# ntnu-yjyjames/nano-vectordb

Measured on AMD Instinct MI355X. Metric: QPS + effective HBM GB/s, flat-scan top-10 d=768, higher is better.
Workload: dtype f16

## Files before the change

nano-vectordb_amd/csrc/kernels_corpus.h:

```cpp
#pragma once
#include <hip/hip_runtime.h>

#include "kernels_exact.h"
#include "nvdb_common.h"

namespace nvdbhip {

template <int DT>
__global__ __launch_bounds__(256) void gen_rows_kernel(uint64_t seed, uint64_t row_base, uint64_t n, uint32_t dim,
                                                       void* __restrict__ rows, float* __restrict__ scales) {
  const int lane = threadIdx.x & 63;
  const uint64_t r = static_cast<uint64_t>(blockIdx.x) * 4 + (threadIdx.x >> 6);
  if (r >= n) return;
  const uint32_t key = synth_row_key(seed, row_base + r);
  unsigned long long ss = 0;
  for (uint32_t c = lane; c < dim; c += 64) { const long long v = synth_raw(key, c); ss += static_cast<unsigned long long>(v * v); }
  for (int o = 32; o > 0; o >>= 1) ss += __shfl_xor(ss, o);
  const double inv = synth_inv_norm(ss);
  if constexpr (DT == DT_F32) {
    float* out = static_cast<float*>(rows) + r * dim;
    for (uint32_t c = lane; c < dim; c += 64) out[c] = synth_elem(synth_raw(key, c), inv);
  } else if constexpr (DT == DT_F16) {
    _Float16* out = static_cast<_Float16*>(rows) + r * dim;
    for (uint32_t c = lane; c < dim; c += 64) out[c] = static_cast<_Float16>(synth_elem(synth_raw(key, c), inv));
  } else {
    float mx = 0.f;
    for (uint32_t c = lane; c < dim; c += 64) mx = fmaxf(mx, fabsf(synth_elem(synth_raw(key, c), inv)));
    for (int o = 32; o > 0; o >>= 1) mx = fmaxf(mx, __shfl_xor(mx, o));
    const float scale = mx > 0.f ? mx / 127.f : 1.f;
    const float is = 1.0f / scale;
    signed char* out = static_cast<signed char*>(rows) + r * dim;
    for (uint32_t c = lane; c < dim; c += 64) {
      float qv = rintf(synth_elem(synth_raw(key, c), inv) * is);
      qv = fminf(fmaxf(qv, -127.f), 127.f);
      out[c] = static_cast<signed char>(static_cast<int>(qv));
    }
    if (lane == 0) scales[r] = scale;
  }
}

template <typename SrcT>
__global__ __launch_bounds__(256) void shadow_f16_kernel(const SrcT* __restrict__ src, _Float16* __restrict__ dst, size_t n,
                                                         uint32_t dim, uint32_t sdim, uint32_t* __restrict__ maxabs_bits) {
  float mx = 0.f;
  const size_t count = n * sdim;
  for (size_t i = static_cast<size_t>(blockIdx.x) * 256 + threadIdx.x; i < count; i += static_cast<size_t>(gridDim.x) * 256) {
    const size_t r = i / sdim;
    const uint32_t c = static_cast<uint32_t>(i - r * sdim);
    const float v = c < dim ? static_cast<float>(src[r * dim + c]) : 0.f;
    dst[i] = static_cast<_Float16>(v);
    mx = fmaxf(mx, fabsf(v));
  }
  for (int o = 32; o > 0; o >>= 1) mx = fmaxf(mx, __shfl_xor(mx, o));
  if ((threadIdx.x & 63) == 0 && mx > 0.f) atomicMax(maxabs_bits, __builtin_bit_cast(uint32_t, mx));
}

static __global__ __launch_bounds__(256) void shadow_i8_kernel(const signed char* __restrict__ src, signed char* __restrict__ dst, size_t n,
                                                        uint32_t dim, uint32_t sdim) {
  const size_t count = n * sdim;
  for (size_t i = static_cast<size_t>(blockIdx.x) * 256 + threadIdx.x; i < count; i += static_cast<size_t>(gridDim.x) * 256) {
    const size_t r = i / sdim;
    const uint32_t c = static_cast<uint32_t>(i - r * sdim);
    dst[i] = c < dim ? src[r * dim + c] : static_cast<signed char>(0);
  }
}

template <typename SrcT>
__global__ __launch_bounds__(256) void shadow_q8_kernel(const SrcT* __restrict__ src, signed char* __restrict__ dst, float* __restrict__ dst_scales,
                                                        uint64_t n, uint32_t dim, uint32_t sdim, uint32_t* __restrict__ out_bits) {
  const int lane = threadIdx.x & 63;
  float wres = 0.f;
  bool bad = false;
  for (uint64_t r = static_cast<uint64_t>(blockIdx.x) * 4 + (threadIdx.x >> 6); r < n; r += static_cast<uint64_t>(gridDim.x) * 4) {
    const SrcT* row = src + r * dim;
    float mx = 0.f;
    for (uint32_t c = lane; c < dim; c += 64) mx = fmaxf(mx, fabsf(static_cast<float>(row[c])));
    for (int o = 32; o > 0; o >>= 1) mx = fmaxf(mx, __shfl_xor(mx, o));
    if (!(mx < 3.0e38f)) bad = true;
    const float scale = mx > 0.f ? mx / 127.f : 1.f;
    const float inv = 1.0f / scale;
    float ss = 0.f;
    signed char* out = dst + r * sdim;
    for (uint32_t c = lane; c < sdim; c += 64) {
      float qv = 0.f, x = 0.f;
      if (c < dim) { x = static_cast<float>(row[c]); qv = fminf(fmaxf(rintf(x * inv), -127.f), 127.f); }
      out[c] = static_cast<signed char>(static_cast<int>(qv));
      const float d = x - qv * scale;
      ss = __builtin_fmaf(d, d, ss);
    }
    for (int o = 32; o > 0; o >>= 1) ss += __shfl_xor(ss, o);
    if (!(ss == ss)) bad = true;
    if (lane == 0) dst_scales[r] = scale;
    wres = fmaxf(wres, sqrtf(ss) * 1.0001f);
  }
  if (lane == 0 && wres > 0.f) atomicMax(out_bits, __builtin_bit_cast(uint32_t, wres));
  if (lane == 0 && (bad || !(wres < 3.0e38f))) out_bits[1] = 1u;
}

template <int DT>
__global__ __launch_bounds__(256) void row_norm_max_kernel(const void* __restrict__ rows, const float* __restrict__ scales,
                                                           uint64_t n, uint32_t dim, uint32_t* __restrict__ out_bits) {
  const int lane = threadIdx.x & 63;
  float wmax = 0.f;
  for (uint64_t r = static_cast<uint64_t>(blockIdx.x) * 4 + (threadIdx.x >> 6); r < n; r += static_cast<uint64_t>(gridDim.x) * 4) {
    const void* rp = row_ptr<DT>(rows, r, dim);
    float ss = 0.f;
    for (uint32_t c = lane; c < dim; c += 64) { const float v = load1<DT>(rp, c); ss = __builtin_fmaf(v, v, ss); }
    for (int o = 32; o > 0; o >>= 1) ss += __shfl_xor(ss, o);
    float nrm = sqrtf(ss) * 1.0001f;
    if constexpr (DT == DT_I8) {
      const float sc = scales[r];
      nrm *= fabsf(sc);
      if (!(sc >= 0.f && sc < 1e30f) && lane == 0) out_bits[1] = 1u;
    }
    wmax = fmaxf(wmax, nrm);
  }
  if (lane == 0 && wmax > 0.f) atomicMax(out_bits, __builtin_bit_cast(uint32_t, wmax));
}

}
```

nano-vectordb_amd/csrc/kernels_filter.h:

```cpp
#pragma once
#include <hip/hip_runtime.h>

#include "kernels_exact.h"

namespace nvdbhip {

typedef _Float16 half8_t __attribute__((ext_vector_type(8)));
typedef float floatx16 __attribute__((ext_vector_type(16)));
typedef int intx16 __attribute__((ext_vector_type(16)));
typedef int int4_t __attribute__((ext_vector_type(4)));

#define NVDB_GPTR(p) ((const __attribute__((address_space(1))) void*)(p))
#define NVDB_LPTR(p) ((__attribute__((address_space(3))) void*)(p))

constexpr int FILTER_ROWS = 32;
constexpr int FILTER_STAGES = 3;
constexpr int FILTER_STAGES_I8 = 5;

struct PrepInit {
  uint32_t* cnt;
  float* thr;
  uint32_t* misc;
  uint32_t* prog;
  uint32_t prog_words;
  uint32_t* tickets;
  const float* q_src;
  float* q32_copy;
};
constexpr uint32_t FUSE_TICKETS = 1;

__device__ __forceinline__ const float* prep_init(const PrepInit& pi, const float* q32, uint32_t q, uint32_t tid, uint32_t nq, uint32_t dim, uint32_t* overflow) {
  if (pi.cnt != nullptr) {
    if (tid == 0) { pi.cnt[q] = 0; overflow[q] = 0; pi.thr[q] = NEG_INF; }
    if (q == 0 && tid < 8) pi.misc[tid] = 0;
    if (q == 0 && tid >= 64 && tid < 64 + FUSE_TICKETS) pi.tickets[tid - 64] = 0;
    for (uint32_t j = q * 256 + tid; j < pi.prog_words; j += gridDim.x * 256) pi.prog[j] = 0xFFFFFFFFu;
  }
  if (pi.q_src != nullptr && q < nq) {
    float* dst = pi.q32_copy + static_cast<uint64_t>(q) * dim;
    const float* srch = pi.q_src + static_cast<uint64_t>(q) * dim;
    for (uint32_t i = tid; i < dim; i += 256) dst[i] = srch[i];
    return dst;
  }
  return q32 + static_cast<uint64_t>(q) * dim;
}

static __global__ __launch_bounds__(256) void prep_q16_kernel(const float* __restrict__ q32, uint32_t nq, uint32_t dim, uint32_t sdim,
                                                       float max_row_norm, float rel, float abs_per_norm, uint32_t* __restrict__ overflow, _Float16* __restrict__ q16,
                                                       float* __restrict__ qscale, float* __restrict__ qinv,
                                                       float* __restrict__ ebound, float* __restrict__ slack, PrepInit pi) {
  __shared__ float red_max[4], red_ss[4];
  const uint32_t q = blockIdx.x, tid = threadIdx.x;
  const float* src = prep_init(pi, q32, q, tid, nq, dim, overflow);
  if (q >= nq) {
    for (uint32_t i = tid; i < sdim; i += 256) q16[static_cast<uint64_t>(q) * sdim + i] = static_cast<_Float16>(0.f);
    if (tid == 0) { qscale[q] = 1.f; qinv[q] = 1.f; ebound[q] = 0.f; slack[q] = 0.f; }
    return;
  }
  float mx = 0.f, ss = 0.f;
  for (uint32_t i = tid; i < dim; i += 256) { const float v = src[i]; mx = fmaxf(mx, fabsf(v)); ss = __builtin_fmaf(v, v, ss); }
  for (int o = 32; o > 0; o >>= 1) { mx = fmaxf(mx, __shfl_xor(mx, o)); ss += __shfl_xor(ss, o); }
  if ((tid & 63) == 0) { red_max[tid >> 6] = mx; red_ss[tid >> 6] = ss; }
  __syncthreads();
  mx = fmaxf(fmaxf(red_max[0], red_max[1]), fmaxf(red_max[2], red_max[3]));
  ss = (red_ss[0] + red_ss[1]) + (red_ss[2] + red_ss[3]);
  int e = 0;
  if (mx > 0.f && mx < 3.0e38f) {
    int ex; (void)frexpf(mx, &ex);
    e = 15 - ex;
    e = e > 100 ? 100 : (e < -100 ? -100 : e);
  }
  const float sc = ldexpf(1.f, e);
  for (uint32_t i = tid; i < sdim; i += 256) q16[static_cast<uint64_t>(q) * sdim + i] = static_cast<_Float16>(i < dim ? src[i] * sc : 0.f);
  if (tid == 0) {
    const float nrm = sqrtf(ss) * 1.0001f;
    const float eb = rel * nrm * max_row_norm + abs_per_norm * nrm + 1e-30f;
    qscale[q] = sc; qinv[q] = ldexpf(1.f, -e); ebound[q] = eb; slack[q] = 2.f * eb;
    if (!(ss < 3.0e38f)) { overflow[q] = 1u; ebound[q] = -1.f; }
  }
}

typedef float float4_t __attribute__((ext_vector_type(4)));
typedef float float2_t __attribute__((ext_vector_type(2)));

#define NVDB_MFMA_F16_ZERO_A(acc, a, b) asm volatile("v_mfma_f32_32x32x16_f16 %0, %1, %2, 0" : "=&v"(acc) : "v"(a), "a"(b))
#define NVDB_MFMA_F16_ZERO_V(acc, a, b) asm volatile("v_mfma_f32_32x32x16_f16 %0, %1, %2, 0" : "=&v"(acc) : "v"(a), "v"(b))
#define NVDB_MFMA_F16_ACC_A(acc, a, b) asm volatile("v_mfma_f32_32x32x16_f16 %0, %1, %2, %0" : "+v"(acc) : "v"(a), "a"(b))
#define NVDB_MFMA_F16_ACC_V(acc, a, b) asm volatile("v_mfma_f32_32x32x16_f16 %0, %1, %2, %0" : "+v"(acc) : "v"(a), "v"(b))

__device__ __forceinline__ void glds16(uint32_t voff, const void* sbase, uint32_t lds_off) {
  uint32_t keep;
  asm volatile("s_mov_b32 %0, m0\n\ts_mov_b32 m0, %2\n\ts_nop 0\n\tglobal_load_lds_dwordx4 %1, %3\n\ts_mov_b32 m0, %0"
               : "=&s"(keep) : "v"(voff), "s"(lds_off), "s"(sbase) : "memory");
}

__device__ __forceinline__ float vmax3(float a, float b, float c) {
  float r;
  asm("v_max3_f32 %0, %1, %2, %3" : "=v"(r) : "v"(a), "v"(b), "v"(c));
  return r;
}

struct Hit { float score; uint32_t row; uint32_t qid; uint32_t pad; };
constexpr uint32_t I8_HI_L1_MAX = 65500;
constexpr int I8_ACC_BIAS = 0x4B000000;
__device__ __forceinline__ int shl_i32(int v, uint32_t bits) { return static_cast<int>(static_cast<uint32_t>(v) << bits); }
constexpr uint32_t FILTER_LOGCAP = 4096;

struct ScatterArgs {
  Cand* cand;
  uint32_t* cnt;
  uint32_t* overflow;
  uint32_t* log_overflow;
  uint32_t cap;
  uint32_t n_rows;
  uint32_t perm_mul, perm_mask, perm_T;
  float* xcdw;
  uint32_t lo_bits;
};

__device__ __forceinline__ void stream_tile_range(uint32_t T, uint32_t S, uint32_t stream, bool xcd_map, const float* xcdw, uint32_t& lo, uint32_t& hi) {
  if (!xcd_map || xcdw == nullptr || (S & 7u) != 0) {
    lo = static_cast<uint32_t>(static_cast<uint64_t>(T) * stream / S);
    hi = static_cast<uint32_t>(static_cast<uint64_t>(T) * (stream + 1) / S);
    return;
  }
  double pre[9];
  pre[0] = 0.0;
#pragma unroll
  for (int x = 0; x < 8; ++x) pre[x + 1] = pre[x] + static_cast<double>(xcdw[x]);
  const double total = pre[8] * static_cast<double>(S >> 3);
  auto f = [&](uint32_t s) -> uint32_t {
    if (s >= S) return T;
    double part = 0.0;
#pragma unroll
    for (int x = 0; x < 8; ++x) part = (static_cast<uint32_t>(x) == (s & 7u)) ? pre[x] : part;
    const double cum = pre[8] * static_cast<double>(s >> 3) + part;
    const uint32_t v = static_cast<uint32_t>(static_cast<double>(T) * (cum / total));
    return v > T ? T : v;
  };
  lo = f(stream);
  hi = f(stream + 1);
}

__device__ __forceinline__ void record_xcd_speed(float* xcdw, bool xcd_map, uint32_t label, uint32_t ntiles, uint32_t ticks_100mhz) {
  if (xcdw == nullptr || !xcd_map || ntiles < 128) return;
  atomicAdd(xcdw + 8 + label, static_cast<float>(ticks_100mhz) * 0.01f);
  atomicAdd(xcdw + 16 + label, static_cast<float>(ntiles));
}

__host__ __device__ __forceinline__ uint32_t perm_tile_raw(uint32_t g, uint32_t mul, uint32_t mask, uint32_t T) {
  if (mask == 0) return g;
  uint32_t x = g;
  do { x = (x * mul + 0x9E3779B1u) & mask; } while (x >= T);
  return x;
}
__device__ __forceinline__ uint32_t perm_tile(uint32_t g, const ScatterArgs& a) { return perm_tile_raw(g, a.perm_mul, a.perm_mask, a.perm_T); }

__host__ __device__ __forceinline__ void perm_params(uint32_t T, uint32_t& mul, uint32_t& mask) {
  mul = 1u; mask = 0u;
  if (T < 64) return;
  uint32_t m = 1;
  while (m < T) m <<= 1;
  mask = m - 1;
  mul = (static_cast<uint32_t>(0.6180339887 * m) | 1u) & mask;
}

__device__ __forceinline__ void scatter_own_log(const Hit* mylog, uint32_t wcnt, const ScatterArgs& a, int lane) {
  asm volatile("s_waitcnt vmcnt(0)" ::: "memory");
  uint32_t n = wcnt;
  if (n > FILTER_LOGCAP) { if (lane == 0) *a.log_overflow = 1u; n = FILTER_LOGCAP; }
  for (uint32_t i = lane; i < n; i += 64) {
    const uint32_t* w = reinterpret_cast<const uint32_t*>(mylog + i);
    const uint32_t sbits = __hip_atomic_load(w + 0, __ATOMIC_RELAXED, __HIP_MEMORY_SCOPE_AGENT);
    const uint32_t row = __hip_atomic_load(w + 1, __ATOMIC_RELAXED, __HIP_MEMORY_SCOPE_AGENT);
    const uint32_t qid = __hip_atomic_load(w + 2, __ATOMIC_RELAXED, __HIP_MEMORY_SCOPE_AGENT);
    if (row >= a.n_rows) continue;
    const uint32_t slot = atomicAdd(&a.cnt[qid], 1u);
    if (slot < a.cap) a.cand[static_cast<uint64_t>(qid) * a.cap + slot] = Cand{__builtin_bit_cast(float, sbits), row};
    else a.overflow[qid] = 1u;
  }
}

__device__ __forceinline__ void glds16_v(const void* gptr, uint32_t lds_off) {
  uint32_t keep;
  asm volatile("s_mov_b32 %0, m0\n\ts_mov_b32 m0, %2\n\ts_nop 0\n\tglobal_load_lds_dwordx4 %1, off\n\ts_mov_b32 m0, %0"
               : "=&s"(keep) : "v"(gptr), "s"(lds_off) : "memory");
}

template <int DIM> constexpr size_t filter_f16_lds_bytes() { return static_cast<size_t>(FILTER_STAGES) * FILTER_ROWS * DIM * 2; }
// ... 504 lines not shown
  const char* gbase = reinterpret_cast<const char*>(rows);
  const uint32_t lds_base = static_cast<uint32_t>(reinterpret_cast<uintptr_t>(NVDB_LPTR(smem)));
  const uint32_t g_lo = row_lo / TROWS + t_lo;
  auto tile_phys = [&](uint32_t t_rel) -> uint32_t { return perm_tile(g_lo + (t_rel < NT ? t_rel : NT - 1), sa); };
  auto stage_ptr = [&](uint32_t t_rel, int kh) -> const char* {
    return gbase + static_cast<uint64_t>(tile_phys(t_rel)) * TROWS * ROW_BYTES + kh * SROW;
  };
  auto issue_piece = [&](const char* src, uint32_t buf, int i) {
    glds16(src_off[i], src, lds_base + buf * STAGE_BYTES + (wave * PPW + i) * 1024);
  };
#pragma unroll
  for (int i = 0; i < PPW; ++i) issue_piece(stage_ptr(0, 0), 0, i);
#pragma unroll
  for (int i = 0; i < PPW; ++i) issue_piece(stage_ptr(0, 1), 1, i);

  constexpr int PIECE_EVERY = KS / PPW;
  uint32_t wcnt = 0;
  Hit* mylog = hitlog + static_cast<uint64_t>(wave_gid) * FILTER_LOGCAP;
  uint32_t* myprog = prog + static_cast<uint64_t>(stream) * 8;
  uint32_t sync_strikes = 0;
  const uint32_t xw_t0 = static_cast<uint32_t>(__builtin_amdgcn_s_memrealtime());
  for (uint32_t t = 0; t < NT; ++t) {
    if constexpr (SYNC) {
      if (wave == 0 && (t & sync_mask) == 0) sibling_rendezvous(myprog, qt, t, sync_lead, sync_strikes, lane);
    }
    float4_t acc;
#pragma unroll
    for (int kh = 0; kh < 2; ++kh) {
      const uint32_t st = 2 * t + kh;
      asm volatile("s_waitcnt vmcnt(%0)" ::"n"(PPW) : "memory");
      __builtin_amdgcn_s_barrier();
      const char* next_src = stage_ptr(t + 1, kh);
      const uint32_t next_buf = (st + 2) % FILTER_STAGES;
      const char* stage = smem + (st % FILTER_STAGES) * STAGE_BYTES;
      if (!wave_has_queries) {
#pragma unroll
        for (int i = 0; i < PPW; ++i) issue_piece(next_src, next_buf, i);
        continue;
      }
      auto read_a = [&](int s) -> float4_t {
        return *reinterpret_cast<const float4_t*>(stage + (a16 ^ ((s & 3) << 6)) + (s >> 2) * 256);
      };
      float4_t ar[RING];
#pragma unroll
      for (int s = 0; s < RING - 1; ++s) ar[s] = read_a(s);
#pragma unroll
      for (int s = 0; s < KS; ++s) {
        if (s + RING - 1 < KS) ar[(s + RING - 1) % RING] = read_a(s + RING - 1);
        const float4_t a = ar[s % RING];
        const int f = kh * KS + s;
        if (f == 0) NVDB_MFMA16_ZERO_A(acc, a, bqa[0]);
        else if (f < NFRAG_A) NVDB_MFMA16_ACC_A(acc, a, bqa[f < NFRAG_A ? f : 0]);
        else NVDB_MFMA16_ACC_V(acc, a, bqv[f >= NFRAG_A ? f - NFRAG_A : 0]);
        if (s % PIECE_EVERY == PIECE_EVERY - 1) issue_piece(next_src, next_buf, s / PIECE_EVERY);
      }
    }
    if (!wave_has_queries) continue;
    asm volatile("s_nop 15\n\ts_nop 15" : "+v"(acc));
    const float m = vmax3(vmax3(acc[0], acc[1], acc[2]), acc[3], acc[3]);
    if (__builtin_amdgcn_ballot_w64(m - thr_s >= 0.f)) {
      const uint32_t row0 = tile_phys(t) * TROWS;
#pragma unroll
      for (int r = 0; r < 4; ++r) {
        const float v = acc[r];
        const bool hit = v >= thr_s;
        const unsigned long long mm = __builtin_amdgcn_ballot_w64(hit);
        if (mm) {
          const uint32_t idx = wcnt + static_cast<uint32_t>(__builtin_popcountll(mm & ((1ull << lane) - 1ull)));
          if (hit && idx < FILTER_LOGCAP) mylog[idx] = Hit{v * inv_s, row0 + 4 * g4 + r, qid, 0u};
          wcnt += static_cast<uint32_t>(__builtin_popcountll(mm));
        }
      }
    }
  }
  if constexpr (SYNC) { if (wave == 0 && lane == 0) __hip_atomic_store(myprog + qt, 0xFFFFFFFFu, __ATOMIC_RELAXED, __HIP_MEMORY_SCOPE_AGENT); }
  if (wave == 0 && lane == 0) record_xcd_speed(sa.xcdw, xcd_map, stream & 7u, NT, static_cast<uint32_t>(__builtin_amdgcn_s_memrealtime()) - xw_t0);
  scatter_own_log(mylog, wcnt, sa, lane);
}

static __global__ __launch_bounds__(256) void prep_q8_kernel(const float* __restrict__ q32, uint32_t nq, uint32_t dim, uint32_t sdim,
                                                      float max_row_norm, float corpus_resid, signed char* __restrict__ qhi,
                                                      signed char* __restrict__ qlo, float* __restrict__ qscale,
                                                      float* __restrict__ qinv, float* __restrict__ ebound,
                                                      float* __restrict__ slack, float* __restrict__ qdelta, uint32_t* __restrict__ overflow, uint32_t lo_bits, PrepInit pi) {
  __shared__ float red_max[4], red_ss[4];
  __shared__ uint32_t red_lo[4];
  const uint32_t q = blockIdx.x, tid = threadIdx.x;
  const float* src = prep_init(pi, q32, q, tid, nq, dim, overflow);
  if (q >= nq) {
    for (uint32_t i = tid; i < sdim; i += 256) { qhi[static_cast<uint64_t>(q) * sdim + i] = 0; qlo[static_cast<uint64_t>(q) * sdim + i] = 0; }
    if (tid == 0) { qscale[q] = 1.f; qinv[q] = 1.f; ebound[q] = 0.f; slack[q] = 0.f; qdelta[q] = 0.f; }
    return;
  }
  float mx = 0.f, ss = 0.f;
  for (uint32_t i = tid; i < dim; i += 256) { const float v = src[i]; mx = fmaxf(mx, fabsf(v)); ss = __builtin_fmaf(v, v, ss); }
  for (int o = 32; o > 0; o >>= 1) { mx = fmaxf(mx, __shfl_xor(mx, o)); ss += __shfl_xor(ss, o); }
  if ((tid & 63) == 0) { red_max[tid >> 6] = mx; red_ss[tid >> 6] = ss; }
  __syncthreads();
  mx = fmaxf(fmaxf(red_max[0], red_max[1]), fmaxf(red_max[2], red_max[3]));
  ss = (red_ss[0] + red_ss[1]) + (red_ss[2] + red_ss[3]);
  const int tmax = 127 << lo_bits, half = 1 << (lo_bits - 1);
  const float sq0 = (mx > 0.f && mx < 3.0e38f) ? mx / static_cast<float>(tmax) : 1.f;
  const float isq0 = 1.0f / sq0;
  float sq_adj = 1.f;
  if (static_cast<uint64_t>(dim) * 127u > I8_HI_L1_MAX) {
    __shared__ uint32_t red_l1[4];
    uint32_t l1 = 0;
    for (uint32_t i = tid; i < dim; i += 256) {
      int t = static_cast<int>(rintf(src[i] * isq0));
      t = t > tmax ? tmax : (t < -tmax ? -tmax : t);
      const int hi = (t + half) >> lo_bits;
      l1 += static_cast<uint32_t>(hi < 0 ? -hi : hi);
    }
    for (int o = 32; o > 0; o >>= 1) l1 += __shfl_xor(l1, o);
    if ((tid & 63) == 0) red_l1[tid >> 6] = l1;
    __syncthreads();
    l1 = (red_l1[0] + red_l1[1]) + (red_l1[2] + red_l1[3]);
    if (l1 > I8_HI_L1_MAX - dim) {
      const float shrink = static_cast<float>(l1) / static_cast<float>(I8_HI_L1_MAX - dim) * 1.001f;
      sq_adj = shrink;
    }
  }
  const float sq = sq0 * sq_adj;
  const float isq = 1.0f / sq;
  uint32_t lo2 = 0;
  for (uint32_t i = tid; i < dim; i += 256) {
    int t = static_cast<int>(rintf(src[i] * isq));
    t = t > tmax ? tmax : (t < -tmax ? -tmax : t);
    const int hi = (t + half) >> lo_bits;
    const int lo = t - (hi << lo_bits);
    qhi[static_cast<uint64_t>(q) * sdim + i] = static_cast<signed char>(hi);
    qlo[static_cast<uint64_t>(q) * sdim + i] = static_cast<signed char>(lo);
    lo2 += static_cast<uint32_t>(lo * lo);
  }
  for (uint32_t i = dim + tid; i < sdim; i += 256) { qhi[static_cast<uint64_t>(q) * sdim + i] = 0; qlo[static_cast<uint64_t>(q) * sdim + i] = 0; }
  for (int o = 32; o > 0; o >>= 1) lo2 += __shfl_xor(lo2, o);
  if ((tid & 63) == 0) red_lo[tid >> 6] = lo2;
  __syncthreads();
  if (tid == 0) {
    qdelta[q] = sqrtf(static_cast<float>(red_lo[0] + red_lo[1] + red_lo[2] + red_lo[3])) * max_row_norm * 1.0001f;

    const float nrm = sqrtf(ss) * 1.0001f;
    const float eb = (0.5005f * sqrtf(static_cast<float>(dim)) * sq + 1.0e-5f * nrm) * max_row_norm * 1.001f + nrm * corpus_resid * 1.001f + 1e-30f;
    qscale[q] = isq; qinv[q] = sq; ebound[q] = eb; slack[q] = 2.f * eb;
    if (!(ss < 3.0e38f)) { overflow[q] = 1u; ebound[q] = -1.f; }
  }
}

template <int ROW_BYTES> __device__ constexpr bool swz16() { return (ROW_BYTES / 16) % 16 == 0; }
template <int ROW_BYTES> __device__ inline uint32_t swz_chunk(uint32_t c, uint32_t r) {
  static_assert(ROW_BYTES % 128 == 0, "int8 row stride: a multiple of 128 bytes");
  return swz16<ROW_BYTES>() ? c ^ (r & 15u) : c ^ ((r >> 1) & 7u);
}
template <int ROW_BYTES> __device__ inline uint32_t a_base_i8(uint32_t r31, uint32_t hsel) { return r31 * ROW_BYTES + (swz_chunk<ROW_BYTES>(hsel, r31) << 4); }
template <int ROW_BYTES> __device__ inline uint32_t a_addr_i8(uint32_t a_base, int s) {
  return swz16<ROW_BYTES>() ? (a_base ^ ((s & 7) << 5)) + (s >> 3) * 256 : (a_base ^ ((s & 3) << 5)) + (s >> 2) * 128;
}

#define NVDB_MFMA_I8_ZERO(acc, a, b) asm volatile("v_mfma_i32_32x32x32_i8 %0, %1, %2, 0" : "=&v"(acc) : "v"(a), "a"(b))
#define NVDB_MFMA_I8_ACC(acc, a, b) asm volatile("v_mfma_i32_32x32x32_i8 %0, %1, %2, %0" : "+v"(acc) : "v"(a), "a"(b))
#define NVDB_MFMA_I8_FROM(acc, a, b, c0) asm volatile("v_mfma_i32_32x32x32_i8 %0, %1, %2, %3" : "=&v"(acc) : "v"(a), "a"(b), "v"(c0))

template <int DIM> constexpr size_t filter_i8_lds_bytes() { return static_cast<size_t>(FILTER_STAGES_I8) * (FILTER_ROWS * DIM + 4 * 1024); }
template <int DIM, bool BOOT = false, int RING = 6, bool SYNC = false>
__global__ __launch_bounds__(256, 1) void filter_i8_kernel(
    const signed char* __restrict__ rows, const float* __restrict__ scales, uint32_t row_lo, uint32_t row_hi,
    const signed char* __restrict__ qhi, const signed char* __restrict__ qlo, uint32_t nq, uint32_t QT,
    const float* __restrict__ thr, const float* __restrict__ qscale, const float* __restrict__ qinv,
    Hit* __restrict__ hitlog, ScatterArgs sa, uint32_t aux, uint32_t* __restrict__ prog, uint32_t sync_mask, uint32_t sync_lead) {
  constexpr int KSTEPS = DIM / 32;
  constexpr int ROW_BYTES = DIM;
  constexpr int DATA_BYTES = FILTER_ROWS * ROW_BYTES;
  constexpr int STAGE_BYTES = DATA_BYTES + 4 * 1024;
  constexpr int PIECES = DATA_BYTES / 1024;
  constexpr int PPW = PIECES / 4;
  constexpr int CHUNKS_PER_ROW = ROW_BYTES / 16;
  static_assert(DIM % 128 == 0, "int8 row stride: a multiple of 128 bytes (swz_chunk)");
  static_assert(PIECES % 4 == 0 && KSTEPS % PPW == 0 && 2 * KSTEPS <= 64, "shape");
  static_assert(FILTER_STAGES_I8 * STAGE_BYTES == filter_i8_lds_bytes<DIM>(), "the launchers size the dynamic LDS with filter_i8_lds_bytes");

  extern __shared__ __attribute__((aligned(16))) char smem[];
  const int tid = threadIdx.x, lane = tid & 63, wave = __builtin_amdgcn_readfirstlane(tid >> 6);
  const int r31 = lane & 31, hsel = lane >> 5;
  const uint32_t wave_gid = blockIdx.x * 4 + wave;

  const uint32_t nwg = gridDim.x, b = blockIdx.x;
  const uint32_t S = nwg / QT;
  uint32_t stream, qt;
  if ((nwg & 7u) == 0 && ((nwg >> 3) % QT) == 0) { const uint32_t xcd = b & 7u, i = b >> 3; qt = i % QT; stream = (i / QT) * 8u + xcd; }
  else { qt = b % QT; stream = b / QT; }
  const uint32_t tiles_total = (row_hi - row_lo) / FILTER_ROWS;
  const bool xcd_map = (nwg & 7u) == 0 && ((nwg >> 3) % QT) == 0;
  uint32_t t_lo, t_hi;
  stream_tile_range(tiles_total, S, stream, xcd_map, sa.xcdw, t_lo, t_hi);
  const uint32_t NT = t_hi - t_lo;
  if (NT == 0) return;

  const uint32_t qbase = qt * 128u + wave * 32u;
  float4_t bq[2 * KSTEPS];
#pragma unroll
  for (int f = 0; f < 2 * KSTEPS; ++f) {
    const signed char* plane = (f < KSTEPS) ? qhi : qlo;
    const int s = f % KSTEPS;
    bq[f] = *reinterpret_cast<const float4_t*>(plane + static_cast<uint64_t>(qbase + r31) * DIM + 32 * s + 16 * hsel);
  }
#pragma unroll
  for (int f = 0; f < 2 * KSTEPS; ++f) asm volatile("" ::"a"(bq[f]));
  const uint32_t qid = qbase + r31;
  const bool real = qid < nq;
  float thr_s = real ? thr[qid] * qscale[qid] : __builtin_huge_valf();
  float inv_s = real ? qinv[qid] : 0.f;
  asm volatile("" ::"v"(thr_s), "v"(inv_s));
  const bool wave_has_queries = qbase < nq;

  uint32_t src_off[PPW];
#pragma unroll
  for (int i = 0; i < PPW; ++i) {
    const uint32_t P = static_cast<uint32_t>((wave * PPW + i) * 64 + lane);
    const uint32_t r = P / CHUNKS_PER_ROW, cpos = P % CHUNKS_PER_ROW;
    src_off[i] = r * ROW_BYTES + (swz_chunk<ROW_BYTES>(cpos, r) << 4);
  }
  const uint32_t sc_off = (lane & 7) * 16;
  const uint32_t a_base = a_base_i8<ROW_BYTES>(static_cast<uint32_t>(r31), static_cast<uint32_t>(hsel));

  const char* gbase = reinterpret_cast<const char*>(rows);
  const uint32_t lds_base = static_cast<uint32_t>(reinterpret_cast<uintptr_t>(NVDB_LPTR(smem)));
  const uint32_t g_lo = row_lo / FILTER_ROWS + t_lo;
  auto tile_row0 = [&](uint32_t t_rel) -> uint32_t { return perm_tile(g_lo + (t_rel < NT ? t_rel : NT - 1), sa) * FILTER_ROWS; };
// ... 324 lines not shown
    if constexpr (VAR == 1) continue;
    const uint32_t row0 = tile_row0(t);
    if constexpr (DEFER) {
      uint32_t nflag = 0;
#pragma unroll
      for (int mb = 0; mb < MB; ++mb)
#pragma unroll
        for (int nb = 0; nb < NB; ++nb) {
          if (!__builtin_amdgcn_ballot_w64(d1[mb][nb] >= 0.f)) continue;
#pragma unroll
          for (int r = 0; r < 16; ++r) {
            const unsigned long long m = __builtin_amdgcn_ballot_w64(static_cast<float>(acc[mb][nb][r]) * scv[mb][r] >= t1q[nb]);
            if (m) {
              nflag += static_cast<uint32_t>(__builtin_popcountll(m));
              const int L = __builtin_ctzll(m);
              pend_H = __builtin_amdgcn_readlane(acc[mb][nb][r], L);
              pend_scale = readlane_f(scv[mb][r], L);
              pend_thr = readlane_f(thr_s[nb], L);
              pend_inv = readlane_f(inv_s[nb], L);
              pend_qid = readlane_u(qid[nb], L);
              pend_row = 32u * mb + (r & 3) + 8u * (r >> 2) + 4u * (static_cast<uint32_t>(L) >> 5);
            }
          }
        }
      if (nflag == 1) {
        if (lane < DIM / 16) pend_x = *reinterpret_cast<const uint4*>(stage + pend_row * ROW_BYTES + (swz_chunk<ROW_BYTES>(static_cast<uint32_t>(lane), pend_row) << 4));
        if (lane < DIM / 16) glds16(static_cast<uint32_t>(lane) * 16u, qlo + static_cast<uint64_t>(pend_qid) * DIM, lds_scratch);
        pend_row += row0;
        pend = true;
        continue;
      }
    }
#pragma unroll
    for (int mb = 0; mb < MB; ++mb)
#pragma unroll
      for (int nb = 0; nb < NB; ++nb) {
        if (!__builtin_amdgcn_ballot_w64(d1[mb][nb] >= 0.f)) continue;
        ++n_stage2;
        const signed char* ql = qlo + static_cast<uint64_t>(qbase + nb * 32 + r31) * DIM + 16 * hsel;
        intx16 lo;
        constexpr int HALF = KSTEPS / 2;
#pragma unroll
        for (int h = 0; h < 2; ++h) {
          float4_t bl[HALF];
#pragma unroll
          for (int s = 0; s < HALF; ++s) bl[s] = *reinterpret_cast<const float4_t*>(ql + 32 * (h * HALF + s));
#pragma unroll
          for (int s = 0; s < RING - 1; ++s) ar[s] = read_a(MB * (h * HALF + s) + mb);
#pragma unroll
          for (int s = 0; s < HALF; ++s) {
            if (s + RING - 1 < HALF) ar[(s + RING - 1) % RING] = read_a(MB * (h * HALF + s + RING - 1) + mb);
            const float4_t a = ar[s % RING];
            if (h == 0 && s == 0) NVDB_MFMA_I8_ZERO_V(lo, a, bl[s]); else NVDB_MFMA_I8_ACC_V(lo, a, bl[s]);
          }
        }
        asm volatile("s_nop 15\n\ts_nop 15" : "+v"(lo));
#pragma unroll
        for (int r = 0; r < 16; ++r) {
          const float fv = static_cast<float>(shl_i32(acc[mb][nb][r], sa.lo_bits) + lo[r]) * scv[mb][r];
          const bool hit = fv >= thr_s[nb];
          const unsigned long long m = __builtin_amdgcn_ballot_w64(hit);
          if (m) {
            const uint32_t idx = wcnt + static_cast<uint32_t>(__builtin_popcountll(m & ((1ull << lane) - 1ull)));
            if (hit && idx < FILTER_LOGCAP) mylog[idx] = Hit{fv * inv_s[nb], row0 + 32 * mb + (r & 3) + 8 * (r >> 2) + 4 * hsel, qid[nb], 0u};
            wcnt += static_cast<uint32_t>(__builtin_popcountll(m));
          }
        }
      }
  }
  if constexpr (DEFER) { if (pend) consume_pending(0); }
  if constexpr (STAMP) {
    const uint64_t dc = __builtin_amdgcn_s_memtime() - stamp_c, dr = __builtin_amdgcn_s_memrealtime() - stamp_r;
    if (wave == 0 && lane == 0) {
      uint64_t* out = reinterpret_cast<uint64_t*>(prog + static_cast<uint64_t>(gridDim.x) * 8) + static_cast<uint64_t>(blockIdx.x) * 2;
      out[0] = dc; out[1] = dr;
    }
  }
  if constexpr (SYNC) { if (wave == 0 && lane == 0) __hip_atomic_store(prog + static_cast<uint64_t>(stream) * 8 + qt, 0xFFFFFFFFu, __ATOMIC_RELAXED, __HIP_MEMORY_SCOPE_AGENT); }
  if (stage_counts && lane == 0 && (n_stage1 | n_stage2)) { atomicAdd(stage_counts, n_stage1); atomicAdd(stage_counts + 1, n_stage2); }
  if (wave == 0 && lane == 0) record_xcd_speed(sa.xcdw, xcd_map, stream & 7u, NT, static_cast<uint32_t>(__builtin_amdgcn_s_memrealtime()) - xw_t0);
  scatter_own_log(mylog, wcnt, sa, lane);
}

template <int DIM>
__device__ __forceinline__ void verify_and_scatter_i8(const Hit* mylog, uint32_t wcnt, const ScatterArgs& a, int lane, const signed char* __restrict__ rows,
                                                      const signed char* __restrict__ qlo, const float* __restrict__ thr, const float* __restrict__ qscale,
                                                      const float* __restrict__ qinv) {
  asm volatile("s_waitcnt vmcnt(0)" ::: "memory");
  uint32_t n = wcnt;
  if (n > FILTER_LOGCAP) { if (lane == 0) *a.log_overflow = 1u; n = FILTER_LOGCAP; }
  constexpr int CPL = DIM / 64;
  constexpr int NE = 2;
  const int part4 = lane & 3;
  for (uint32_t base = 0; base < n; base += 16 * NE) {
    uint32_t sbits[NE], row[NE], qid[NE];
    int H[NE], part[NE];
    bool valid[NE];
#pragma unroll
    for (int j = 0; j < NE; ++j) {
      const uint32_t e = base + 16u * j + (static_cast<uint32_t>(lane) >> 2);
      valid[j] = e < n;
      const uint32_t* w = reinterpret_cast<const uint32_t*>(mylog + (valid[j] ? e : 0u));
      sbits[j] = __hip_atomic_load(w + 0, __ATOMIC_RELAXED, __HIP_MEMORY_SCOPE_AGENT);
      row[j] = __hip_atomic_load(w + 1, __ATOMIC_RELAXED, __HIP_MEMORY_SCOPE_AGENT);
      qid[j] = __hip_atomic_load(w + 2, __ATOMIC_RELAXED, __HIP_MEMORY_SCOPE_AGENT);
      H[j] = static_cast<int>(__hip_atomic_load(w + 3, __ATOMIC_RELAXED, __HIP_MEMORY_SCOPE_AGENT));
    }
    uint4 x[NE][CPL], y[NE][CPL];
#pragma unroll
    for (int j = 0; j < NE; ++j) {
      valid[j] = valid[j] && row[j] < a.n_rows;
      const uint4* xr = reinterpret_cast<const uint4*>(rows + static_cast<uint64_t>(valid[j] ? row[j] : 0u) * DIM);
      const uint4* qr = reinterpret_cast<const uint4*>(qlo + static_cast<uint64_t>(valid[j] ? qid[j] : 0u) * DIM);
#pragma unroll
      for (int c = 0; c < CPL; ++c) { x[j][c] = xr[part4 + 4 * c]; y[j][c] = qr[part4 + 4 * c]; }
    }
#pragma unroll
    for (int j = 0; j < NE; ++j) {
      part[j] = 0;
#pragma unroll
      for (int c = 0; c < CPL; ++c) {
        part[j] = __builtin_amdgcn_sdot4(static_cast<int>(x[j][c].x), static_cast<int>(y[j][c].x), part[j], false);
        part[j] = __builtin_amdgcn_sdot4(static_cast<int>(x[j][c].y), static_cast<int>(y[j][c].y), part[j], false);
        part[j] = __builtin_amdgcn_sdot4(static_cast<int>(x[j][c].z), static_cast<int>(y[j][c].z), part[j], false);
        part[j] = __builtin_amdgcn_sdot4(static_cast<int>(x[j][c].w), static_cast<int>(y[j][c].w), part[j], false);
      }
      part[j] += __builtin_amdgcn_update_dpp(0, part[j], 0xB1, 0xF, 0xF, true);
      part[j] += __builtin_amdgcn_update_dpp(0, part[j], 0x4E, 0xF, 0xF, true);
      if (valid[j] && part4 == 0) {
        const float fv = static_cast<float>(shl_i32(H[j], a.lo_bits) + part[j]) * __builtin_bit_cast(float, sbits[j]);
        if (fv >= thr[qid[j]] * qscale[qid[j]]) {
          const uint32_t slot = atomicAdd(&a.cnt[qid[j]], 1u);
          if (slot < a.cap) a.cand[static_cast<uint64_t>(qid[j]) * a.cap + slot] = Cand{fv * qinv[qid[j]], row[j]};
          else a.overflow[qid[j]] = 1u;
        }
      }
    }
  }
}

template <int DIM, int WPB = 4, bool DEFER = true> constexpr size_t filter_i8p_lds_bytes() {
  return static_cast<size_t>(3) * (2 * FILTER_ROWS * DIM + (WPB == 4 ? 4 : 1) * 256) + (DEFER ? WPB * (16 / WPB) * DIM : 0);
}
template <int DIM, bool SYNC = false, bool STAMP = false, int RING = 6, int VAR = 0, int WPB = 4, bool DEFER = true>
__global__ __launch_bounds__(64 * WPB, 1) void filter_i8p_kernel(
    const signed char* __restrict__ rows, const float* __restrict__ scales, uint32_t row_lo, uint32_t row_hi,
    const signed char* __restrict__ qhi, const signed char* __restrict__ qlo, uint32_t nq, uint32_t QT,
    const float* __restrict__ thr, const float* __restrict__ qscale, const float* __restrict__ qinv,
    const float* __restrict__ qdelta, Hit* __restrict__ hitlog, ScatterArgs sa, uint32_t* __restrict__ prog,
    uint32_t sync_mask, uint32_t sync_lead, uint32_t* __restrict__ stage_counts) {
  static_assert(WPB == 4 || WPB == 8, "4 waves x 64 queries or 8 waves x 32 queries");
  constexpr int NB = 8 / WPB, MB = 2;
  constexpr int NV = 16 * NB;
  constexpr int KSTEPS = DIM / 32;
  constexpr int ROW_BYTES = DIM;
  constexpr int TROWS = FILTER_ROWS * MB;
  constexpr int NSTAGE = 3;
  constexpr int DATA_BYTES = TROWS * ROW_BYTES;
  constexpr int SC_COPIES = WPB == 4 ? 4 : 1;
  constexpr int STAGE_BYTES = DATA_BYTES + SC_COPIES * 256;
  constexpr int NSLOT_DEFER = 16 / WPB, SCRATCH_BYTES = DEFER ? NSLOT_DEFER * DIM : 0;
  constexpr int PIECES = DATA_BYTES / 1024;
  constexpr int PPW = PIECES / WPB;
  constexpr int CHUNKS_PER_ROW = ROW_BYTES / 16;
  static_assert(DIM % 128 == 0 && DIM <= 768, "row stride multiple of 128 bytes (swz_chunk); int32 range of 128*H + L");
  static_assert(PIECES % WPB == 0 && KSTEPS % PPW == 0 && KSTEPS % 2 == 0 && KSTEPS >= 8, "shape");
  static_assert(NSTAGE * STAGE_BYTES + WPB * SCRATCH_BYTES <= 160 * 1024 && PPW + 1 < 64 && DIM % 16 == 0 && DIM / 16 <= 64, "LDS / vmcnt range");
  static_assert(NSTAGE * STAGE_BYTES + WPB * SCRATCH_BYTES == filter_i8p_lds_bytes<DIM, WPB, DEFER>(), "the launchers size the dynamic LDS with filter_i8p_lds_bytes");

  extern __shared__ __attribute__((aligned(16))) char smem[];
  const int tid = threadIdx.x, lane = tid & 63, wave = __builtin_amdgcn_readfirstlane(tid >> 6);
  const int r31 = lane & 31, hsel = lane >> 5;
  const uint32_t wave_gid = blockIdx.x * WPB + wave;

  const uint32_t nwg = gridDim.x, b = blockIdx.x;
  const uint32_t S = nwg / QT;
  uint32_t stream, qt;
  if ((nwg & 7u) == 0 && ((nwg >> 3) % QT) == 0) { const uint32_t xcd = b & 7u, i = b >> 3; qt = i % QT; stream = (i / QT) * 8u + xcd; }
  else { qt = b % QT; stream = b / QT; }
  const uint32_t tiles_total = (row_hi - row_lo) / TROWS;
  const bool xcd_map = (nwg & 7u) == 0 && ((nwg >> 3) % QT) == 0;
  uint32_t t_lo, t_hi;
  stream_tile_range(tiles_total, S, stream, xcd_map, sa.xcdw, t_lo, t_hi);
  const uint32_t NT = t_hi - t_lo;
  if (NT == 0) return;

  const uint32_t qbase = qt * 256u + wave * (32u * NB);
  float4_t bq[NB * KSTEPS];
#pragma unroll
  for (int f = 0; f < NB * KSTEPS; ++f) {
    const int nb = f / KSTEPS, s = f % KSTEPS;
    bq[f] = *reinterpret_cast<const float4_t*>(qhi + static_cast<uint64_t>(qbase + nb * 32 + r31) * DIM + 32 * s + 16 * hsel);
  }
#pragma unroll
  for (int f = 0; f < NB * KSTEPS; ++f) asm volatile("" ::"a"(bq[f]));
  constexpr bool BIASED = !DEFER;
  intx16 bias0;
#pragma unroll
  for (int r = 0; r < 16; ++r) bias0[r] = I8_ACC_BIAS;
  if constexpr (BIASED) asm volatile("" : "+v"(bias0));
  auto hval = [&](int bits) -> int { return BIASED ? bits - I8_ACC_BIAS : bits; };
  uint32_t qid[NB];
  float thr_s[NB], t1q[NB], inv_s[NB];
  const float lo_unit = __builtin_bit_cast(float, (127u - sa.lo_bits) << 23);
#pragma unroll
  for (int nb = 0; nb < NB; ++nb) {
    qid[nb] = qbase + nb * 32 + r31;
    const bool real = qid[nb] < nq;
    thr_s[nb] = real ? thr[qid[nb]] * qscale[qid[nb]] : __builtin_huge_valf();
    inv_s[nb] = real ? qinv[qid[nb]] : 0.f;
    const float T = thr_s[nb];
    t1q[nb] = real ? (T - (1.001f * qdelta[qid[nb]] + 2e-6f * fabsf(T) + 1e-5f)) * lo_unit : __builtin_huge_valf();
    asm volatile("" ::"v"(thr_s[nb]), "v"(inv_s[nb]), "v"(t1q[nb]));
  }
// ... 392 lines not shown
```

nano-vectordb_amd/csrc/kernels_filter_i8s.h:

```cpp
#pragma once
#include "kernels_filter.h"

namespace nvdbhip {

typedef int intx4_t __attribute__((ext_vector_type(4)));

#define NVDB_MFMA_I8S_FROM(acc, a, b, c0) asm volatile("v_mfma_i32_16x16x64_i8 %0, %1, %2, %3" : "=&v"(acc) : "v"(a), "a"(b), "v"(c0))
#define NVDB_MFMA_I8S_ACC(acc, a, b) asm volatile("v_mfma_i32_16x16x64_i8 %0, %1, %2, %0" : "+v"(acc) : "v"(a), "a"(b))

template <int DIM, int WPB = 4> constexpr size_t filter_i8s_lds_bytes() { return static_cast<size_t>(3) * (2 * FILTER_ROWS * DIM + WPB * 256); }
template <int DIM, bool SYNC = false, bool STAMP = false, int RING = 6, int VAR = 0, int WPB = 4>
__global__ __launch_bounds__(64 * WPB, 1) void filter_i8s_kernel(
    const signed char* __restrict__ rows, const float* __restrict__ scales, uint32_t row_lo, uint32_t row_hi,
    const signed char* __restrict__ qhi, const signed char* __restrict__ qlo, uint32_t nq, uint32_t QT,
    const float* __restrict__ thr, const float* __restrict__ qscale, const float* __restrict__ qinv,
    const float* __restrict__ qdelta, Hit* __restrict__ hitlog, ScatterArgs sa, uint32_t* __restrict__ prog,
    uint32_t sync_mask, uint32_t sync_lead, uint32_t* __restrict__ stage_counts) {
  static_assert(WPB == 4 || WPB == 8, "4 waves x 64 queries or 8 waves x 32 queries");
  constexpr bool NOTEST = VAR == 1 || VAR == 3 || VAR == 4;
  constexpr int NB = 16 / WPB, MB = 2;
  constexpr int NV = 8 * NB;
  constexpr int KS = DIM / 64;
  constexpr int ROW_BYTES = DIM;
  constexpr int TROWS = FILTER_ROWS * MB;
  constexpr int NSTAGE = 3;
  constexpr int DATA_BYTES = TROWS * ROW_BYTES;
  constexpr int STAGE_BYTES = DATA_BYTES + WPB * 256;
  constexpr int PIECES = DATA_BYTES / 1024, PPW = PIECES / WPB;
  constexpr int CHUNKS_PER_ROW = ROW_BYTES / 16;
  constexpr int NSLOT = 2 * NB * KS;
  constexpr int NFRAG = 2 * KS;
  static_assert(DIM % 128 == 0 && DIM <= 768, "row stride multiple of 128 bytes (swz_chunk); 64 queries x DIM bytes = 192 AGPRs at most");
  static_assert(PIECES % WPB == 0 && PPW % 2 == 0 && NSTAGE * STAGE_BYTES <= 160 * 1024 && PPW + 1 < 64 && NFRAG >= RING, "shape / LDS / vmcnt range");
  static_assert(NSTAGE * STAGE_BYTES == filter_i8s_lds_bytes<DIM, WPB>(), "the launchers size the dynamic LDS with filter_i8s_lds_bytes");

  extern __shared__ __attribute__((aligned(16))) char smem[];
  const int tid = threadIdx.x, lane = tid & 63, wave = __builtin_amdgcn_readfirstlane(tid >> 6);
  const int x15 = lane & 15, g4 = lane >> 4;
  const uint32_t wave_gid = blockIdx.x * WPB + wave;

  const uint32_t nwg = gridDim.x, b = blockIdx.x;
  const uint32_t S = nwg / QT;
  uint32_t stream, qt;
  if ((nwg & 7u) == 0 && ((nwg >> 3) % QT) == 0) { const uint32_t xcd = b & 7u, i = b >> 3; qt = i % QT; stream = (i / QT) * 8u + xcd; }
  else { qt = b % QT; stream = b / QT; }
  const uint32_t tiles_total = (row_hi - row_lo) / TROWS;
  const bool xcd_map = (nwg & 7u) == 0 && ((nwg >> 3) % QT) == 0;
  uint32_t t_lo, t_hi;
  stream_tile_range(tiles_total, S, stream, xcd_map, sa.xcdw, t_lo, t_hi);
  const uint32_t NT = t_hi - t_lo;
  if (NT == 0) return;

  const uint32_t qbase = qt * 256u + wave * (16u * NB);
  float4_t bq[NB * KS];
#pragma unroll
  for (int f = 0; f < NB * KS; ++f) {
    const int nb = f / KS, s = f % KS;
    bq[f] = *reinterpret_cast<const float4_t*>(qhi + static_cast<uint64_t>(qbase + nb * 16 + x15) * DIM + 64 * s + 16 * g4);
  }
#pragma unroll
  for (int f = 0; f < NB * KS; ++f) asm volatile("" ::"a"(bq[f]));
  intx4_t bias0;
#pragma unroll
  for (int r = 0; r < 4; ++r) bias0[r] = I8_ACC_BIAS;
  asm volatile("" : "+v"(bias0));
  uint32_t qid[NB];
  float t1q[NB];
  const float lo_unit = __builtin_bit_cast(float, (127u - sa.lo_bits) << 23);
#pragma unroll
  for (int nb = 0; nb < NB; ++nb) {
    qid[nb] = qbase + nb * 16 + x15;
    const bool real = qid[nb] < nq;
    const float T = real ? thr[qid[nb]] * qscale[qid[nb]] : __builtin_huge_valf();
    t1q[nb] = real ? (T - (1.001f * qdelta[qid[nb]] + 2e-6f * fabsf(T) + 1e-5f)) * lo_unit : __builtin_huge_valf();
    asm volatile("" ::"v"(t1q[nb]));
  }
  const bool wave_has_queries = qbase < nq;

  uint32_t src_off[PPW];
#pragma unroll
  for (int i = 0; i < PPW; ++i) {
    const uint32_t P = static_cast<uint32_t>((wave * PPW + i) * 64 + lane);
    const uint32_t r = P / CHUNKS_PER_ROW, cpos = P % CHUNKS_PER_ROW;
    src_off[i] = r * ROW_BYTES + (swz_chunk<ROW_BYTES>(cpos, r) << 4);
  }
  const uint32_t sc_off = (lane & (8 * MB - 1)) * 16;
  const uint32_t a16 = static_cast<uint32_t>(x15) * ROW_BYTES + (swz_chunk<ROW_BYTES>(static_cast<uint32_t>(g4), static_cast<uint32_t>(x15)) << 4);

  const char* gbase = reinterpret_cast<const char*>(rows);
  const uint32_t lds_base = static_cast<uint32_t>(reinterpret_cast<uintptr_t>(NVDB_LPTR(smem)));
  const uint32_t g_lo = row_lo / TROWS + t_lo;
  auto tile_row0 = [&](uint32_t t_rel) -> uint32_t { return perm_tile(g_lo + (t_rel < NT ? t_rel : NT - 1), sa) * TROWS; };
  auto issue_piece = [&](uint32_t row0, uint32_t buf, int i) {
    glds16(src_off[i], gbase + static_cast<uint64_t>(row0) * ROW_BYTES, lds_base + buf * STAGE_BYTES + (wave * PPW + i) * 1024);
  };
  auto issue_scales = [&](uint32_t row0, uint32_t buf) {
    if (lane < 8 * MB) glds16(sc_off, reinterpret_cast<const char*>(scales + row0), lds_base + buf * STAGE_BYTES + DATA_BYTES + wave * 256);
  };
  auto loop_piece = [&](uint32_t row0, uint32_t buf, int i) { if constexpr (VAR != 3) issue_piece(row0, buf, i); };
  auto loop_scales = [&](uint32_t row0, uint32_t buf) { if constexpr (VAR != 3) issue_scales(row0, buf); };
#pragma unroll
  for (int st = 0; st < NSTAGE - 1; ++st) {
#pragma unroll
    for (int i = 0; i < PPW; ++i) issue_piece(tile_row0(st), st, i);
    issue_scales(tile_row0(st), st);
  }

  uint32_t wcnt = 0, n_stage1 = 0;
  Hit* mylog = hitlog + static_cast<uint64_t>(wave_gid) * FILTER_LOGCAP;

  intx4_t acc0[2][NB], acc1[2][NB];
  float scv[2][8], scc[2][8];
#pragma unroll
  for (int i = 0; i < 8; ++i) { scv[0][i] = scv[1][i] = 0.f; scc[0][i] = scc[1][i] = 0.f; }
#pragma unroll
  for (int h = 0; h < 2; ++h)
#pragma unroll
    for (int nb = 0; nb < NB; ++nb) acc1[h][nb] = bias0;
  float mx[NB][2];
  float4_t ar[RING];

  auto read_a = [&](const char* stage, int u, int mb) -> float4_t {
    const int s = u >> 1, h = u & 1;
    if constexpr (VAR == 4) { float4_t z = {0.f, 1.f, 2.f, 3.f}; asm volatile("" : "+v"(z)); return z; }
    const uint32_t off = swz16<ROW_BYTES>() ? (a16 ^ ((s & 3) << 6)) + (s >> 2) * 256 : (a16 ^ ((s & 1) << 6)) + (s >> 1) * 128;
    return *reinterpret_cast<const float4_t*>(stage + off + (2 * mb + h) * 16 * ROW_BYTES);
  };
  constexpr int SW0 = NSLOT >= 64 ? 8 : 4;
  auto scale_step = [&](const char* stage, int mb, int set, int w) {
    if constexpr (NOTEST) return;
    if (w == 0) {
      const float* sc_lds = reinterpret_cast<const float*>(stage + DATA_BYTES + wave * 256);
#pragma unroll
      for (int h = 0; h < 2; ++h) {
        const float4 v = *reinterpret_cast<const float4*>(sc_lds + 32 * mb + 16 * h + 4 * g4);
        scv[set][4 * h] = v.x; scv[set][4 * h + 1] = v.y; scv[set][4 * h + 2] = v.z; scv[set][4 * h + 3] = v.w;
      }
    }
    const int i = w - SW0;
    if (i >= 0 && i < 8) scc[set][i] = scv[set][i] * -8388608.f;
  };
  float tm[NV];
  constexpr int W0 = SW0 + 10;
  constexpr int SPU = (NSLOT - W0 - 4) / NV >= 2 ? 2 : 1;
  static_assert(W0 + NV * SPU + 2 <= NSLOT, "the test ends before the half's last MFMA");
  auto test_step = [&](const intx4_t (&a)[2][NB], const float (&sc)[8], const float (&sccs)[8], int w) {
    if constexpr (NOTEST) return;
    const int rel = w - W0;
    if (rel < 0 || rel % SPU != 0) return;
    const int v = rel / SPU;
    if (v < NV) {
      const int nb = v >> 3, h = (v >> 2) & 1, j = v & 3;
      const int b0 = a[h][nb][j];
      tm[v] = __builtin_fmaf(__builtin_bit_cast(float, b0), sc[4 * h + j], sccs[4 * h + j]);
    }
    const int p = v - 1;
    if (p >= 0 && p < NV && (p & 1)) mx[p >> 3][(p >> 2) & 1] = vmax3(mx[p >> 3][(p >> 2) & 1], tm[p - 1], tm[p]);
  };
  auto reset_max = [&]() {
#pragma unroll
    for (int nb = 0; nb < NB; ++nb) { mx[nb][0] = -__builtin_huge_valf(); mx[nb][1] = -__builtin_huge_valf(); }
  };
  float flagv = -1.f;
  auto combine_flags = [&]() {
    if constexpr (NOTEST) return;
    float m[NB];
#pragma unroll
    for (int nb = 0; nb < NB; ++nb) m[nb] = vmax3(mx[nb][0], mx[nb][1], mx[nb][1]) - t1q[nb];
    flagv = NB == 4 ? vmax3(vmax3(m[0], m[1], m[NB / 2]), m[NB - 1], m[NB - 1]) : vmax3(m[0], m[NB - 1], m[NB - 1]);
  };
  auto any_flag = [&]() -> bool { return __builtin_amdgcn_ballot_w64(flagv >= 0.f) != 0; };
  auto rare_log = [&](const intx4_t (&a)[2][NB], const float (&sc)[8], uint32_t row0, int mb) {
    ++n_stage1;
#pragma unroll
    for (int nb = 0; nb < NB; ++nb)
#pragma unroll
      for (int h = 0; h < 2; ++h) {
        if (!__builtin_amdgcn_ballot_w64(mx[nb][h] >= t1q[nb])) continue;
#pragma unroll
        for (int j = 0; j < 4; ++j) {
          const int H = a[h][nb][j] - I8_ACC_BIAS;
          const bool hit = static_cast<float>(H) * sc[4 * h + j] >= t1q[nb];
          const unsigned long long m = __builtin_amdgcn_ballot_w64(hit);
          if (m) {
            const uint32_t idx = wcnt + static_cast<uint32_t>(__builtin_popcountll(m & ((1ull << lane) - 1ull)));
            if (hit && idx < FILTER_LOGCAP)
              mylog[idx] = Hit{sc[4 * h + j], row0 + 32u * mb + 16u * h + 4u * g4 + j, qid[nb], static_cast<uint32_t>(H)};
            wcnt += static_cast<uint32_t>(__builtin_popcountll(m));
          }
        }
      }
  };

  uint32_t sync_strikes = 0;
  uint64_t stamp_c = 0, stamp_r = 0;
  if constexpr (STAMP) { stamp_c = __builtin_amdgcn_s_memtime(); stamp_r = __builtin_amdgcn_s_memrealtime(); }
  const uint32_t xw_t0 = static_cast<uint32_t>(__builtin_amdgcn_s_memrealtime());
  constexpr int HP = PPW / 2, HP0 = HP < 3 ? HP : 3;
  constexpr int D1 = (HP - HP0) > 0 ? (HP - HP0) : 1;
  constexpr int EV1 = NFRAG / D1, EV2 = NFRAG / (PPW - HP);
  static_assert((HP == HP0 || NFRAG % (HP - HP0) == 0) && NFRAG % (PPW - HP) == 0, "pieces spread evenly over the A fragments of both halves");
  for (uint32_t t = 0; t < NT; ++t) {
    if constexpr (SYNC) {
      if (wave == 0 && (t & sync_mask) == 0) sibling_rendezvous(prog + static_cast<uint64_t>(stream) * 8, qt, t, sync_lead, sync_strikes, lane);
    }
    asm volatile("s_waitcnt vmcnt(%0)" ::"n"(PPW + 1) : "memory");
    __builtin_amdgcn_s_barrier();
    const uint32_t next_row0 = tile_row0(t + 2), next_buf = (t + 2) % NSTAGE;
    const char* stage = smem + (t % NSTAGE) * STAGE_BYTES;
    if (!wave_has_queries) {
#pragma unroll
      for (int i = 0; i < PPW; ++i) issue_piece(next_row0, next_buf, i);
      issue_scales(next_row0, next_buf);
      continue;
    }
    reset_max();
#pragma unroll
    for (int u = 0; u < RING - 1; ++u) ar[u] = read_a(stage, u, 0);
#pragma unroll
    for (int i = 0; i < HP0; ++i) loop_piece(next_row0, next_buf, i);
    __builtin_amdgcn_sched_barrier(0);
#pragma unroll
    for (int u = 0; u < NFRAG; ++u) {
      if (u + RING - 1 < NFRAG) ar[(u + RING - 1) % RING] = read_a(stage, u + RING - 1, 0);
      else ar[(u + RING - 1) % RING] = read_a(stage, u + RING - 1 - NFRAG, 1);
      const float4_t av = ar[u % RING];
      const int s = u >> 1, h = u & 1;
#pragma unroll
      for (int nb = 0; nb < NB; ++nb) {
        if (s == 0) NVDB_MFMA_I8S_FROM(acc0[h][nb], av, bq[nb * KS], bias0);
        else NVDB_MFMA_I8S_ACC(acc0[h][nb], av, bq[nb * KS + s]);
        const int w = NB * u + nb;
        scale_step(stage, 0, 0, w);
        test_step(acc1, scv[1], scc[1], w);
        if (w == NSLOT - 1) combine_flags();
        __builtin_amdgcn_sched_barrier(0);
      }
      if constexpr (HP > HP0) {
        if (u % EV1 == EV1 - 1) loop_piece(next_row0, next_buf, HP0 + u / EV1);
        __builtin_amdgcn_sched_barrier(0);
      }
    }
    if (VAR == 0 && t > 0 && any_flag()) rare_log(acc1, scv[1], tile_row0(t - 1), 1);
    if constexpr (VAR != 0) { asm volatile("" ::"v"(flagv)); }
    reset_max();
    constexpr int R0 = NFRAG % RING;
#pragma unroll
    for (int u = 0; u < NFRAG; ++u) {
      if (u + RING - 1 < NFRAG) ar[(R0 + u + RING - 1) % RING] = read_a(stage, u + RING - 1, 1);
      const float4_t av = ar[(R0 + u) % RING];
      const int s = u >> 1, h = u & 1;
#pragma unroll
      for (int nb = 0; nb < NB; ++nb) {
        if (s == 0) NVDB_MFMA_I8S_FROM(acc1[h][nb], av, bq[nb * KS], bias0);
        else NVDB_MFMA_I8S_ACC(acc1[h][nb], av, bq[nb * KS + s]);
        const int w = NB * u + nb;
        scale_step(stage, 1, 1, w);
        test_step(acc0, scv[0], scc[0], w);
        if (w == NSLOT - 1) combine_flags();
        __builtin_amdgcn_sched_barrier(0);
      }
      if (u % EV2 == EV2 - 1) loop_piece(next_row0, next_buf, HP + u / EV2);
      if (u == 0) loop_scales(next_row0, next_buf);
      __builtin_amdgcn_sched_barrier(0);
    }
    if (VAR == 0 && any_flag()) rare_log(acc0, scv[0], tile_row0(t), 0);
    if constexpr (VAR != 0) { asm volatile("" ::"v"(flagv)); }
  }
  if (wave_has_queries) {
    asm volatile("s_nop 15\n\ts_nop 15" ::: "memory");
    reset_max();
#pragma unroll
    for (int w = W0; w < W0 + (NV + 1) * SPU; ++w) test_step(acc1, scv[1], scc[1], w);
    combine_flags();
    if (VAR == 0 && any_flag()) rare_log(acc1, scv[1], tile_row0(NT - 1), 1);
  }
  if constexpr (STAMP) {
    const uint64_t dc = __builtin_amdgcn_s_memtime() - stamp_c, dr = __builtin_amdgcn_s_memrealtime() - stamp_r;
    if (wave == 0 && lane == 0) {
      uint64_t* out = reinterpret_cast<uint64_t*>(prog + static_cast<uint64_t>(gridDim.x) * 8) + static_cast<uint64_t>(blockIdx.x) * 2;
      out[0] = dc; out[1] = dr;
    }
  }
  if constexpr (SYNC) { if (wave == 0 && lane == 0) __hip_atomic_store(prog + static_cast<uint64_t>(stream) * 8 + qt, 0xFFFFFFFFu, __ATOMIC_RELAXED, __HIP_MEMORY_SCOPE_AGENT); }
  if (stage_counts && lane == 0 && n_stage1) atomicAdd(stage_counts, n_stage1);
  if (wave == 0 && lane == 0) record_xcd_speed(sa.xcdw, xcd_map, stream & 7u, NT, static_cast<uint32_t>(__builtin_amdgcn_s_memrealtime()) - xw_t0);
  verify_and_scatter_i8<DIM>(mylog, wcnt, sa, lane, rows, qlo, thr, qscale, qinv);
}

}
```

nano-vectordb_amd/csrc/nvdb_corpus.cpp:

```cpp
#include "nvdb_ctx.h"
#include "kernels_corpus.h"

namespace {

std::string g_create_err;

void free_corpus(nvdb_hip_ctx* c) {
  if (c->owned) {
    if (c->rows) (void)hipFree(c->rows);
    if (c->scales) (void)hipFree(c->scales);
  }
  if (c->shadow16) { (void)hipFree(c->shadow16); c->shadow16 = nullptr; }
  if (c->shadow8) { (void)hipFree(c->shadow8); c->shadow8 = nullptr; }
  if (c->shadow8_scales) { (void)hipFree(c->shadow8_scales); c->shadow8_scales = nullptr; }
  c->rows = nullptr; c->scales = nullptr; c->owned = false; c->n = 0; c->dim = 0; c->fdim = 0; c->dtype = 0; c->max_norm = 0.f;
  c->cap_hint = 0;
  c->q8shadow = false; c->resid_max = 0.f; c->filter_max_norm = 0.f;
  c->shadow_demoted = false; c->last_filter_kind = 0;
  c->range_valid = false; c->range_total = 0;
  parts_drop(c);
  c->nmasks = 0;
}

nvdb_status compute_max_norm(nvdb_hip_ctx* c) {
  nvdb_status st = ensure(c, c->misc, 64);
  if (st) return st;
  HIPCHK(c, hipMemsetAsync(c->misc.p, 0, 64, c->stream));
  uint32_t* bits = static_cast<uint32_t*>(c->misc.p) + 8;
  const unsigned grid = static_cast<unsigned>(std::min<uint64_t>((c->n + 3) / 4, 4096));
  if (c->dtype == NVDB_DTYPE_F32) row_norm_max_kernel<DT_F32><<<grid, 256, 0, c->stream>>>(c->rows, c->scales, c->n, c->dim, bits);
  else if (c->dtype == NVDB_DTYPE_F16) row_norm_max_kernel<DT_F16><<<grid, 256, 0, c->stream>>>(c->rows, c->scales, c->n, c->dim, bits);
  else row_norm_max_kernel<DT_I8><<<grid, 256, 0, c->stream>>>(c->rows, c->scales, c->n, c->dim, bits);
  HIPCHK(c, hipGetLastError());
  uint32_t h = 0, hb[2] = {0, 0};
  HIPCHK(c, hipMemcpyAsync(hb, bits, 8, hipMemcpyDeviceToHost, c->stream));
  HIPCHK(c, hipStreamSynchronize(c->stream));
  h = hb[0];
  std::memcpy(&c->max_norm, &h, 4);
  c->i8_scales_signed = hb[1] != 0;
  c->fdim = c->dim;
  c->filter_max_norm = c->max_norm;
  c->q8shadow = false; c->resid_max = 0.f;
  size_t free_hbm = 0, total_hbm = 0;
  const bool automatic = c->opt_q8_shadow < 0;
  if (automatic && hipMemGetInfo(&free_hbm, &total_hbm) != hipSuccess) { (void)hipGetLastError(); free_hbm = 0; }
  if (q8_shadow_wanted(c, free_hbm)) {
    const uint32_t sdim = c->dim;
    const size_t count = static_cast<size_t>(c->n) * sdim, pad = static_cast<size_t>(PAD_ROWS) * sdim + 4096;
    const size_t n_pad = (static_cast<size_t>(c->n) + PAD_ROWS - 1) / PAD_ROWS * PAD_ROWS + PAD_ROWS;
    hipError_t e = hipMalloc(reinterpret_cast<void**>(&c->shadow8), count + pad);
    if (e == hipSuccess) e = hipMalloc(reinterpret_cast<void**>(&c->shadow8_scales), n_pad * 4);
    if (e != hipSuccess) {
      if (c->shadow8) (void)hipFree(c->shadow8);
      c->shadow8 = nullptr; c->shadow8_scales = nullptr;
      (void)hipGetLastError();
      if (!automatic) return fail(c, NVDB_ERR_HIP, std::string("q8_shadow allocation: ") + hipGetErrorString(e));
    }
  }
  if (c->shadow8) {
    const uint32_t sdim = c->dim;
    const size_t count = static_cast<size_t>(c->n) * sdim, pad = static_cast<size_t>(PAD_ROWS) * sdim + 4096;
    const size_t n_pad = (static_cast<size_t>(c->n) + PAD_ROWS - 1) / PAD_ROWS * PAD_ROWS + PAD_ROWS;
    HIPCHK(c, hipMemsetAsync(c->shadow8 + count, 0, pad, c->stream));
    HIPCHK(c, hipMemsetAsync(c->shadow8_scales, 0, n_pad * 4, c->stream));
    HIPCHK(c, hipMemsetAsync(bits, 0, 8, c->stream));
    if (c->dtype == NVDB_DTYPE_F32) shadow_q8_kernel<float><<<grid, 256, 0, c->stream>>>(static_cast<const float*>(c->rows), c->shadow8, c->shadow8_scales, c->n, c->dim, sdim, bits);
    else shadow_q8_kernel<_Float16><<<grid, 256, 0, c->stream>>>(static_cast<const _Float16*>(c->rows), c->shadow8, c->shadow8_scales, c->n, c->dim, sdim, bits);
    HIPCHK(c, hipGetLastError());
    HIPCHK(c, hipMemcpyAsync(hb, bits, 8, hipMemcpyDeviceToHost, c->stream));
    HIPCHK(c, hipStreamSynchronize(c->stream));
    if (hb[1] == 0) {
      std::memcpy(&c->resid_max, &hb[0], 4);
      HIPCHK(c, hipMemsetAsync(bits, 0, 8, c->stream));
      row_norm_max_kernel<DT_I8><<<grid, 256, 0, c->stream>>>(c->shadow8, c->shadow8_scales, c->n, sdim, bits);
      HIPCHK(c, hipGetLastError());
      HIPCHK(c, hipMemcpyAsync(hb, bits, 8, hipMemcpyDeviceToHost, c->stream));
      HIPCHK(c, hipStreamSynchronize(c->stream));
      std::memcpy(&c->filter_max_norm, &hb[0], 4);
      c->q8shadow = true;
      c->i8_scales_signed = false;
      return NVDB_OK;
    }
    (void)hipFree(c->shadow8); c->shadow8 = nullptr;
    (void)hipFree(c->shadow8_scales); c->shadow8_scales = nullptr;
  }
  if (c->dtype != NVDB_DTYPE_I8 && c->dim <= F16_FILTER_MAX_DIM && !(c->dtype == NVDB_DTYPE_F16 && f16_filter_dim(c->dim)) && c->opt_f32_shadow) {
    uint32_t sdim = 128;
    while (!f16_filter_dim(sdim) || sdim < c->dim) sdim += 128;
    const size_t count = static_cast<size_t>(c->n) * sdim;
    const size_t pad = static_cast<size_t>(PAD_ROWS) * sdim * 2 + 4096;
    HIPCHK(c, hipMalloc(reinterpret_cast<void**>(&c->shadow16), count * 2 + pad));
    HIPCHK(c, hipMemsetAsync(reinterpret_cast<char*>(c->shadow16) + count * 2, 0, pad, c->stream));
    HIPCHK(c, hipMemsetAsync(bits, 0, 4, c->stream));
    if (c->dtype == NVDB_DTYPE_F32) shadow_f16_kernel<float><<<4096, 256, 0, c->stream>>>(static_cast<const float*>(c->rows), c->shadow16, c->n, c->dim, sdim, bits);
    else shadow_f16_kernel<_Float16><<<4096, 256, 0, c->stream>>>(static_cast<const _Float16*>(c->rows), c->shadow16, c->n, c->dim, sdim, bits);
    HIPCHK(c, hipGetLastError());
    HIPCHK(c, hipMemcpyAsync(&h, bits, 4, hipMemcpyDeviceToHost, c->stream));
    HIPCHK(c, hipStreamSynchronize(c->stream));
    float maxabs; std::memcpy(&maxabs, &h, 4);
    if (!(maxabs < 60000.f)) { (void)hipFree(c->shadow16); c->shadow16 = nullptr; }
    else c->fdim = sdim;
  }
  if (c->dtype == NVDB_DTYPE_I8 && c->dim <= I8_FILTER_MAX_DIM && !i8_filter_dim(c->dim) && c->opt_f32_shadow) {
    uint32_t sdim = 256;
    while (!i8_filter_dim(sdim) || sdim < c->dim) sdim += 128;
    const size_t count = static_cast<size_t>(c->n) * sdim, pad = static_cast<size_t>(PAD_ROWS) * sdim + 4096;
    const size_t n_pad = (static_cast<size_t>(c->n) + PAD_ROWS - 1) / PAD_ROWS * PAD_ROWS + PAD_ROWS;
    HIPCHK(c, hipMalloc(reinterpret_cast<void**>(&c->shadow8), count + pad));
    HIPCHK(c, hipMalloc(reinterpret_cast<void**>(&c->shadow8_scales), n_pad * 4));
    HIPCHK(c, hipMemsetAsync(c->shadow8 + count, 0, pad, c->stream));
    HIPCHK(c, hipMemsetAsync(c->shadow8_scales, 0, n_pad * 4, c->stream));
    HIPCHK(c, hipMemcpyAsync(c->shadow8_scales, c->scales, static_cast<size_t>(c->n) * 4, hipMemcpyDeviceToDevice, c->stream));
    shadow_i8_kernel<<<4096, 256, 0, c->stream>>>(static_cast<const signed char*>(c->rows), c->shadow8, c->n, c->dim, sdim);
    HIPCHK(c, hipGetLastError());
    HIPCHK(c, hipStreamSynchronize(c->stream));
    c->fdim = sdim;
  }
  return NVDB_OK;
}

nvdb_status upload_rows(nvdb_hip_ctx* c, void* dst, const void* src, size_t bytes) {
  unsigned T = std::min(6u, std::max(2u, std::thread::hardware_concurrency() / 2));
  if (const char* e = std::getenv("NVDB_UPLOAD_THREADS")) T = static_cast<unsigned>(std::max(1, std::atoi(e)));
  constexpr size_t CH = size_t(8) << 20;
  const size_t nch = (bytes + CH - 1) / CH;
  if (T <= 1 || nch < 4 * static_cast<size_t>(T)) {
    const size_t chunk = size_t(256) << 20;
    for (size_t off = 0; off < bytes; off += chunk) {
      const size_t take = std::min(chunk, bytes - off);
      HIPCHK(c, hipMemcpy(static_cast<char*>(dst) + off, static_cast<const char*>(src) + off, take, hipMemcpyHostToDevice));
    }
    return NVDB_OK;
  }
  std::vector<std::string> errs(T);
  std::atomic<size_t> next{0};
  auto worker = [&](unsigned t) {
    hipStream_t st = nullptr;
    void* pin[2] = {nullptr, nullptr};
    hipEvent_t ev[2] = {nullptr, nullptr};
    bool used[2] = {false, false};
    auto chk = [&](hipError_t e, const char* what) { if (e != hipSuccess && errs[t].empty()) errs[t] = std::string(what) + ": " + hipGetErrorString(e); return e == hipSuccess; };
    bool ok = chk(hipSetDevice(c->device), "hipSetDevice") && chk(hipStreamCreateWithFlags(&st, hipStreamNonBlocking), "hipStreamCreate");
    const auto tp0 = std::chrono::steady_clock::now();
    for (int b = 0; b < 2 && ok; ++b)
      ok = chk(hipHostMalloc(&pin[b], CH, hipHostMallocDefault), "hipHostMalloc") && chk(hipEventCreateWithFlags(&ev[b], hipEventDisableTiming), "hipEventCreate");
    if (t == 0 && std::getenv("NVDB_UPLOAD_DEBUG")) std::fprintf(stderr, "[nvdb upload] thread 0: stream + 2 pinned buffers of %zu MB in %.1f ms\n", CH >> 20, std::chrono::duration<double, std::milli>(std::chrono::steady_clock::now() - tp0).count());
    for (int b = 0; ok; b ^= 1) {
      const size_t i = next.fetch_add(1);
      if (i >= nch) break;
      const size_t off = i * CH, take = std::min(CH, bytes - off);
      if (used[b]) ok = chk(hipEventSynchronize(ev[b]), "hipEventSynchronize");
      if (!ok) break;
      std::memcpy(pin[b], static_cast<const char*>(src) + off, take);
      ok = chk(hipMemcpyAsync(static_cast<char*>(dst) + off, pin[b], take, hipMemcpyHostToDevice, st), "hipMemcpyAsync") && chk(hipEventRecord(ev[b], st), "hipEventRecord");
      used[b] = true;
    }
    if (st) (void)hipStreamSynchronize(st);
    for (int b = 0; b < 2; ++b) { if (ev[b]) (void)hipEventDestroy(ev[b]); if (pin[b]) (void)hipHostFree(pin[b]); }
    if (st) (void)hipStreamDestroy(st);
  };
  std::vector<std::thread> th;
  for (unsigned t = 0; t < T; ++t) th.emplace_back(worker, t);
  for (auto& x : th) x.join();
  for (const auto& e : errs) if (!e.empty()) return fail(c, NVDB_ERR_HIP, "upload: " + e);
  return NVDB_OK;
}

// ... 15 lines not shown
  const size_t pad = static_cast<size_t>(PAD_ROWS) * dim * bpe_of(dtype) + 4096;
  HIPCHK(c, hipMalloc(rows, bytes + pad));
  hipError_t e = hipMemset(static_cast<char*>(*rows) + bytes, 0, pad);
  if (e == hipSuccess && dtype == NVDB_DTYPE_I8) {
    e = hipMalloc(reinterpret_cast<void**>(scales), (n + PAD_ROWS) * sizeof(float));
    if (e == hipSuccess) e = hipMemset(*scales + n, 0, PAD_ROWS * sizeof(float));
  }
  if (e != hipSuccess) {
    (void)hipFree(*rows); *rows = nullptr;
    if (*scales) { (void)hipFree(*scales); *scales = nullptr; }
    return fail(c, NVDB_ERR_HIP, std::string("corpus allocation: ") + hipGetErrorString(e));
  }
  return NVDB_OK;
}

nvdb_status corpus_take_ownership(nvdb_hip_ctx* c, void* dev_rows, float* dev_scales, uint64_t n, uint32_t dim, uint32_t dtype,
                                  uint64_t global_row_base) {
  free_corpus(c);
  c->rows = dev_rows; c->scales = dev_scales; c->owned = true;
  nvdb_status st = check_corpus_args(c, n, dim, dtype);
  if (!st && (!dev_rows || (dtype == NVDB_DTYPE_I8 && !dev_scales))) st = fail(c, NVDB_ERR_INVALID, "take_ownership: null buffer");
  if (st) { free_corpus(c); return st; }
  HIPCHK(c, hipSetDevice(c->device));
  c->n = n; c->dim = dim; c->dtype = dtype; c->row_base = global_row_base;
  return compute_max_norm(c);
}

}

extern "C" {

int nvdb_hip_abi_version(void) { return NVDB_HIP_ABI_VERSION; }

int nvdb_hip_device_count(void) {
  int n = 0;
  if (hipGetDeviceCount(&n) != hipSuccess) return -1;
  return n;
}

nvdb_status nvdb_hip_create(int device_ordinal, nvdb_hip_ctx** out_ctx) {
  if (!out_ctx) return NVDB_ERR_INVALID;
  *out_ctx = nullptr;
  int ndev = 0;
  hipError_t e = hipGetDeviceCount(&ndev);
  if (e != hipSuccess || ndev <= 0) {
    g_create_err = std::string("no HIP device available: ") + (e != hipSuccess ? hipGetErrorString(e) : "device count is 0");
    return NVDB_ERR_HIP;
  }
  if (device_ordinal < 0 || device_ordinal >= ndev) { g_create_err = "device ordinal out of range"; return NVDB_ERR_INVALID; }
  if ((e = hipSetDevice(device_ordinal)) != hipSuccess) { g_create_err = hipGetErrorString(e); return NVDB_ERR_HIP; }
  auto* c = new nvdb_hip_ctx();
  c->device = device_ordinal;
  hipDeviceProp_t prop;
  if (hipGetDeviceProperties(&prop, device_ordinal) == hipSuccess) c->num_cu = prop.multiProcessorCount;
  if ((e = hipStreamCreateWithFlags(&c->stream, hipStreamNonBlocking)) != hipSuccess) {
    g_create_err = hipGetErrorString(e);
    delete c;
    return NVDB_ERR_HIP;
  }
  {
    float w0[24];
    for (int i = 0; i < 24; ++i) w0[i] = i < 8 ? 1.f : 0.f;
    if ((e = hipMalloc(&c->xcdw.p, sizeof(w0))) != hipSuccess || (e = hipMemcpy(c->xcdw.p, w0, sizeof(w0), hipMemcpyHostToDevice)) != hipSuccess) {
      g_create_err = hipGetErrorString(e);
      if (c->xcdw.p) (void)hipFree(c->xcdw.p);
      (void)hipStreamDestroy(c->stream);
      delete c;
      return NVDB_ERR_HIP;
    }
    c->xcdw.bytes = sizeof(w0);
  }
  *out_ctx = c;
  return NVDB_OK;
}

void nvdb_hip_destroy(nvdb_hip_ctx* c) {
  if (!c) return;
  (void)hipSetDevice(c->device);
  (void)hipStreamSynchronize(c->stream);
  free_corpus(c);
  parts_destroy(c);
  if (c->hostblock.p) c->misc.p = nullptr;
  for (DevBuf* b : {&c->q32, &c->q16, &c->qscale, &c->qinv, &c->ebound, &c->slack, &c->thr, &c->cnt, &c->overflow, &c->cand,
                    &c->out_ids, &c->out_scores, &c->misc, &c->hostblock, &c->hitlog, &c->prog, &c->qdelta, &c->rq, &c->rcand, &c->rout_ids, &c->rout_dist, &c->rdbg, &c->lk_scores, &c->lk_sel, &c->lk_hist, &c->lk_state, &c->xcdw, &c->tickets,
                    &c->rg_radius, &c->rg_kept, &c->rg_off, &c->rg_idx, &c->rg_q, &c->rg_desc, &c->rg_taken, &c->rg_slab, &c->rg_pcnt, &c->rg_maskof, &c->rg_ids, &c->rg_scores, &c->row_masks, &c->mask_rows})
    if (b->p) (void)hipFree(b->p);
  for (hipEvent_t e : c->ev_pool) (void)hipEventDestroy(e);
  for (auto& k : c->klaunch) { (void)hipEventDestroy(k.e0); (void)hipEventDestroy(k.e1); }
  for (hipEvent_t e : c->kl_pool) (void)hipEventDestroy(e);
  if (c->pinned) (void)hipHostFree(c->pinned);
  if (c->rpinned) (void)hipHostFree(c->rpinned);
  (void)hipStreamDestroy(c->stream);
  delete c;
}

const char* nvdb_hip_last_error(const nvdb_hip_ctx* c) { return c ? c->err.c_str() : g_create_err.c_str(); }

nvdb_status nvdb_hip_upload_corpus(nvdb_hip_ctx* c, const void* rows, const float* scales, uint64_t n, uint32_t dim,
                                   uint32_t dtype, uint64_t global_row_base) {
  nvdb_status st = check_corpus_args(c, n, dim, dtype);
  if (st) return st;
  if (!rows) return fail(c, NVDB_ERR_INVALID, "upload_corpus: null rows");
  if (dtype == NVDB_DTYPE_I8 && !scales) return fail(c, NVDB_ERR_INVALID, "upload_corpus: int8 corpus needs per-row scales");
  HIPCHK(c, hipSetDevice(c->device));
  free_corpus(c);
  const size_t bytes = static_cast<size_t>(n) * dim * bpe_of(dtype);
  const bool dbg = std::getenv("NVDB_UPLOAD_DEBUG") != nullptr;
  const auto t0 = std::chrono::steady_clock::now();
  auto since = [&]() { return std::chrono::duration<double, std::milli>(std::chrono::steady_clock::now() - t0).count(); };
  if ((st = corpus_alloc_padded(c, n, dim, dtype, &c->rows, &c->scales))) return st;
  c->owned = true;
  const double t_alloc = since();
  if ((st = upload_rows(c, c->rows, rows, bytes))) return st;
  const double t_rows = since();
  if (dtype == NVDB_DTYPE_I8) HIPCHK(c, hipMemcpy(c->scales, scales, n * sizeof(float), hipMemcpyHostToDevice));
  c->n = n; c->dim = dim; c->dtype = dtype; c->row_base = global_row_base;
  st = compute_max_norm(c);
  if (dbg) std::fprintf(stderr, "[nvdb upload] %.2f GB: device allocation %.1f ms, rows %.1f ms (%.1f GB/s), scales + row-norm pass (+ shadow copy) %.1f ms\n",
                        bytes / 1e9, t_alloc, t_rows - t_alloc, bytes / 1e6 / (t_rows - t_alloc), since() - t_rows);
  return st;
}

nvdb_status nvdb_hip_adopt_corpus(nvdb_hip_ctx* c, void* dev_rows, float* dev_scales, uint64_t n, uint32_t dim, uint32_t dtype,
                                  uint64_t global_row_base) {
  nvdb_status st = check_corpus_args(c, n, dim, dtype);
  if (st) return st;
  if (!dev_rows) return fail(c, NVDB_ERR_INVALID, "adopt_corpus: null rows");
  if (dtype == NVDB_DTYPE_I8 && !dev_scales) return fail(c, NVDB_ERR_INVALID, "adopt_corpus: int8 corpus needs per-row scales");
  HIPCHK(c, hipSetDevice(c->device));
  free_corpus(c);
  c->rows = dev_rows; c->scales = dev_scales; c->owned = false;
  c->n = n; c->dim = dim; c->dtype = dtype; c->row_base = global_row_base;
  return compute_max_norm(c);
}

nvdb_status nvdb_hip_generate_corpus(nvdb_hip_ctx* c, uint64_t seed, uint64_t n, uint32_t dim, uint32_t dtype,
                                     uint64_t global_row_base) {
  nvdb_status st = check_corpus_args(c, n, dim, dtype);
  if (st) return st;
  HIPCHK(c, hipSetDevice(c->device));
  free_corpus(c);
  if ((st = corpus_alloc_padded(c, n, dim, dtype, &c->rows, &c->scales))) return st;
  c->owned = true;
  c->n = n; c->dim = dim; c->dtype = dtype; c->row_base = global_row_base;
  const uint64_t slab = 1ull << 24;
  for (uint64_t r0 = 0; r0 < n; r0 += slab) {
    const uint64_t cntr = std::min(slab, n - r0);
    const unsigned grid = static_cast<unsigned>((cntr + 3) / 4);
    char* rp = static_cast<char*>(c->rows) + r0 * dim * bpe_of(dtype);
    if (dtype == NVDB_DTYPE_F32) gen_rows_kernel<DT_F32><<<grid, 256, 0, c->stream>>>(seed, global_row_base + r0, cntr, dim, rp, nullptr);
    else if (dtype == NVDB_DTYPE_F16) gen_rows_kernel<DT_F16><<<grid, 256, 0, c->stream>>>(seed, global_row_base + r0, cntr, dim, rp, nullptr);
    else gen_rows_kernel<DT_I8><<<grid, 256, 0, c->stream>>>(seed, global_row_base + r0, cntr, dim, rp, c->scales + r0);
    HIPCHK(c, hipGetLastError());
  }
  return compute_max_norm(c);
}

nvdb_status nvdb_hip_corpus_info(const nvdb_hip_ctx* c, uint64_t* n, uint32_t* dim, uint32_t* dtype, uint64_t* base, float* mx) {
  if (!c) return NVDB_ERR_INVALID;
  if (n) *n = c->n;
  if (dim) *dim = c->dim;
  if (dtype) *dtype = c->dtype;
  if (base) *base = c->row_base;
  if (mx) *mx = c->max_norm;
  return c->rows ? NVDB_OK : NVDB_ERR_NO_CORPUS;
}

nvdb_status nvdb_hip_download_rows(nvdb_hip_ctx* c, uint64_t row0, uint64_t nrows, void* rows_out, float* scales_out) {
  if (!c) return NVDB_ERR_INVALID;
  if (!c->rows) return fail(c, NVDB_ERR_NO_CORPUS, "Empty base");
  if (row0 + nrows > c->n || !rows_out) return fail(c, NVDB_ERR_INVALID, "download_rows: range out of bounds");
  HIPCHK(c, hipSetDevice(c->device));
  HIPCHK(c, hipStreamSynchronize(c->stream));
  const size_t rb = static_cast<size_t>(c->dim) * bpe_of(c->dtype);
  HIPCHK(c, hipMemcpy(rows_out, static_cast<const char*>(c->rows) + row0 * rb, nrows * rb, hipMemcpyDeviceToHost));
  if (scales_out && c->scales) HIPCHK(c, hipMemcpy(scales_out, c->scales + row0, nrows * sizeof(float), hipMemcpyDeviceToHost));
  return NVDB_OK;
}

nvdb_status nvdb_hip_set_option(nvdb_hip_ctx* c, const char* key, int64_t value) {
  if (!c || !key) return NVDB_ERR_INVALID;
  const std::string k(key);
  if (k == "path") { if (value < 0 || value > 2) return fail(c, NVDB_ERR_INVALID, "path must be 0,1,2"); c->opt_path = value; }
  else if (k == "chunk0_rows") { if (value < 256) return fail(c, NVDB_ERR_INVALID, "chunk0_rows must be >= 256"); c->opt_chunk0 = value; }
  else if (k == "cand_cap") { if (value < 0 || value > SELECT_MAX_CAP) return fail(c, NVDB_ERR_INVALID, "cand_cap out of range"); c->opt_cap = value; }
  else if (k == "time_kernels") { c->opt_time_kernels = value ? 1 : 0; }
  else if (k == "sync_every") { if (value < 1 || (value & (value - 1))) return fail(c, NVDB_ERR_INVALID, "sync_every must be a power of two"); c->opt_sync_every = value; }
  else if (k == "sync_lead") { if (value < 1) return fail(c, NVDB_ERR_INVALID, "sync_lead must be >= 1"); c->opt_sync_lead = value; }
  else if (k == "sibling_sync") { c->opt_sibling_sync = value ? 1 : 0; }
  else if (k == "f32_shadow") { c->opt_f32_shadow = value ? 1 : 0; }
  else if (k == "q8_shadow") { c->opt_q8_shadow = value < 0 ? -1 : value ? 1 : 0; }
  else if (k == "q8_auto_min_rows") { if (value < 1) return fail(c, NVDB_ERR_INVALID, "q8_auto_min_rows must be >= 1"); c->opt_q8_auto_min_rows = value; }
  else if (k == "q8_auto_max_mb") { if (value < 0 || value > (int64_t(1) << 30)) return fail(c, NVDB_ERR_INVALID, "q8_auto_max_mb out of range"); c->opt_q8_auto_max_mb = value; }
#ifdef NVDB_HIP_DEV
  else if (k == "mfma16") { c->opt_mfma16 = value ? 1 : 0; }
  else if (k == "i8_wide") { c->opt_i8_wide = value ? 1 : 0; }
  else if (k == "i8_pipe") { c->opt_i8_pipe = value ? 1 : 0; }
  else if (k == "i8_waves8") { c->opt_i8_waves8 = value ? 1 : 0; }
  else if (k == "i8_mfma16") { c->opt_i8_mfma16 = value ? 1 : 0; }
  else if (k == "i8_small8") { c->opt_i8_small8 = value ? 1 : 0; }
#else
  else if (k == "mfma16" || k == "i8_wide" || k == "i8_pipe" || k == "i8_mfma16" || k == "i8_small8") { if (!value) return fail(c, NVDB_ERR_UNSUPPORTED, k + " = 0 selects a developer-build kernel variant (libnvdb_hip_dev.so)"); }
  else if (k == "i8_waves8") { if (value) return fail(c, NVDB_ERR_UNSUPPORTED, "i8_waves8 = 1 selects a developer-build kernel variant (libnvdb_hip_dev.so)"); }
#endif

  else if (k == "i8_defer") { c->opt_i8_defer = value ? 1 : 0; }
  else if (k == "xcd_balance") { c->opt_xcd_balance = value ? 1 : 0; }
  else if (k == "i8_lo_bits") { if (value < 2 || value > 7) return fail(c, NVDB_ERR_INVALID, "i8_lo_bits must be in [2,7]"); c->opt_i8_lo_bits = value; }
  else if (k == "boot_tiles") { if (value < 0 || value > SELECT_MAX_CAP) return fail(c, NVDB_ERR_INVALID, "boot_tiles out of range"); c->opt_boot_tiles = value; }
#ifdef NVDB_HIP_DEV
  else if (k == "debug_rows") { c->dbg_rows = value < 0 ? 0 : value; }
#endif
  else if (k == "waves8") { c->opt_waves8 = value ? 1 : 0; }
  else if (k == "fuse") { c->opt_fuse = value ? 1 : 0; }
  else if (k == "zero_copy") { c->opt_zero_copy = value ? 1 : 0; }
  else if (k == "shadow_exact_thr") { c->opt_shadow_exact_thr = value ? 1 : 0; }
  else if (k == "exact_mfma") { c->opt_exact_mfma = value ? 1 : 0; }
  else if (k == "exact_img") { c->opt_exact_img = value ? 1 : 0; }
  else if (k == "exact_prescan") { c->opt_exact_prescan = value ? 1 : 0; }
  else if (k == "exact_wgs") { if (value < 1 || value > 16) return fail(c, NVDB_ERR_INVALID, "exact_wgs must be in [1,16]"); c->opt_exact_wgs = value; }
  else if (k == "exact_lds") { if (value < 0 || value > 2) return fail(c, NVDB_ERR_INVALID, "exact_lds must be 0, 1 or 2"); c->opt_exact_lds = value; }
  else if (k == "time_launches") { c->opt_time_launches = value ? 1 : 0; }
  else if (k == "tile_permute") { c->opt_tile_permute = value ? 1 : 0; }
  else if (k == "rescore8") { c->opt_rescore8 = value < 0 ? 0 : (value > 2 ? 2 : value); }
  else if (k == "mfma_boot") { c->opt_mfma_boot = value ? 1 : 0; }
  else if (k == "refine_v2") { c->opt_refine_v2 = value < 0 ? 0 : (value > 2 ? 2 : value); }
  else if (k == "refine_pinned") { c->opt_refine_pinned = value ? 1 : 0; }
  else if (k == "refine_dbg_q") { if (value < 0) return fail(c, NVDB_ERR_INVALID, "refine_dbg_q must be >= 0"); c->opt_refine_dbg_q = value; }
  else if (k == "largek_budget_mb") { if (value < 1) return fail(c, NVDB_ERR_INVALID, "largek_budget_mb must be >= 1"); c->opt_largek_budget_mb = value; }
  else if (k == "range_max_mb") { if (value < 1) return fail(c, NVDB_ERR_INVALID, "range_max_mb must be >= 1"); c->opt_range_max_mb = value; }
  else if (k == "chunk_growth") { if (value != 0 && (value < 2 || value > 64)) return fail(c, NVDB_ERR_INVALID, "chunk_growth must be 0 (automatic) or in [2,64]"); c->opt_growth = value; }
  else if (k == "min_filter_batch") { if (value < 1) return fail(c, NVDB_ERR_INVALID, "min_filter_batch must be >= 1"); c->opt_min_filter_batch = value; }
  else return fail(c, NVDB_ERR_INVALID, "unknown option: " + k);
  return NVDB_OK;
}

nvdb_status nvdb_hip_shadow_info(const nvdb_hip_ctx* c, uint64_t* out4) {
  if (!c || !out4) return NVDB_ERR_INVALID;
  out4[0] = c->q8shadow ? 1u : 0u;
  out4[1] = c->q8shadow ? q8_shadow_bytes(c->n, c->dim) : 0u;
  out4[2] = c->shadow_demoted ? 1u : 0u;
  out4[3] = c->last_filter_kind;
  return NVDB_OK;
}

nvdb_status nvdb_hip_get_stats(nvdb_hip_ctx* c, nvdb_hip_scan_stats* stats) {
  if (!c || !stats) return NVDB_ERR_INVALID;
  if (c->stats_lazy) {
    c->stats_lazy = false;
    unsigned long long tot = 0;
    HIPCHK(c, hipSetDevice(c->device));
    if (nvdb_status st = sum_candidates(c, &tot)) return st;
    c->stats.candidates = tot;
  }
  *stats = c->stats;
  return NVDB_OK;
}

#ifdef NVDB_HIP_DEV
uint32_t nvdb_permuted_tile(uint32_t g, uint32_t n_tiles) {
  uint32_t mul, mask;
  perm_params(n_tiles, mul, mask);
  return perm_tile_raw(g, mul, mask, n_tiles);
}
#endif

void nvdb_synth_rows_f32(uint64_t seed, uint64_t row0, uint64_t nrows, uint32_t dim, float* out) {
  std::vector<int32_t> raw(dim);
  for (uint64_t r = 0; r < nrows; ++r) {
    const uint32_t key = synth_row_key(seed, row0 + r);
    uint64_t ss = 0;
    for (uint32_t c = 0; c < dim; ++c) { raw[c] = synth_raw(key, c); ss += static_cast<uint64_t>(static_cast<int64_t>(raw[c]) * raw[c]); }
    const double inv = synth_inv_norm(ss);
    for (uint32_t c = 0; c < dim; ++c) out[r * dim + c] = synth_elem(raw[c], inv);
  }
}

void nvdb_f32_to_f16(const float* src, uint16_t* dst, uint64_t n) {
  for (uint64_t i = 0; i < n; ++i) dst[i] = f32_to_f16_rne(src[i]);
}

void nvdb_quantize_i8_rows(const float* rows, uint64_t nrows, uint32_t dim, int8_t* out, float* scales) {
  for (uint64_t r = 0; r < nrows; ++r) scales[r] = quantize_i8_row(rows + r * dim, dim, out + r * dim);
}

}
```

nano-vectordb_amd/csrc/nvdb_ctx.h:

```cpp
#pragma once
#pragma GCC visibility push(default)
#include "../../include/nvdb_hip.h"
#ifdef NVDB_HIP_DEV
#include "../../include/nvdb_hip_dev.h"
#endif
#pragma GCC visibility pop

#include <hip/hip_runtime.h>
#include <hip/hip_ext.h>

#include <algorithm>
#include <atomic>
#include <chrono>
#include <cmath>
#include <cstdio>
#include <cstdlib>
#include <cstring>
#include <set>
#include <string>
#include <thread>
#include <type_traits>
#include <vector>

#include "kernels_exact.h"
#include "kernels_filter.h"
#include "nvdb_common.h"

using namespace nvdbhip;

namespace nvdbhip {

constexpr uint32_t SELECT_MAX_CAP = 8192;
constexpr uint32_t WAVE_KMAX = 64;
constexpr uint32_t FILTER_KMAX = 1024;
constexpr float FILTER_REL_F16 = 7.5e-4f;
constexpr uint32_t PROG_SLOTS = 16;
constexpr uint32_t F16_FILTER_MAX_DIM = 3072;
constexpr uint32_t I8W_TILE_ROWS = 64;
constexpr uint32_t PAD_ROWS = 64;
constexpr uint32_t I8_FILTER_MAX_DIM = 1536;

struct DevBuf {
  void* p = nullptr;
  size_t bytes = 0;
};

struct PartState;

}

struct nvdb_hip_ctx {
  int device = 0;
  int num_cu = 256;
  hipStream_t stream = nullptr;
  std::string err;

  void* rows = nullptr;
  float* scales = nullptr;
  bool owned = false;
  uint64_t n = 0;
  uint32_t dim = 0, dtype = 0;
  uint64_t row_base = 0;
  float max_norm = 0.f;
  bool i8_scales_signed = false;
  signed char* shadow8 = nullptr;
  bool q8shadow = false;
  bool use_shadow = true;
  bool shadow_demoted = false;
  uint32_t last_filter_kind = 0;
  float filter_max_norm = 0.f;
  float resid_max = 0.f;
  int64_t opt_q8_shadow = -1;
  int64_t opt_q8_auto_min_rows = 1 << 20;
  int64_t opt_q8_auto_max_mb = 16384;
  float* shadow8_scales = nullptr;
  _Float16* shadow16 = nullptr;
  uint32_t fdim = 0;
  DevBuf qdelta;
  int64_t opt_i8_wide = 1;
  int64_t opt_i8_waves8 = 0;
  int64_t opt_i8_defer = 0;
  int64_t opt_i8_mfma16 = 1;
  int64_t opt_i8_pipe = 1;
  int64_t opt_waves8 = 1;
  void* pinned = nullptr;
  void* pinned_dev = nullptr;
  size_t pinned_bytes = 0;
  bool perm_on = false;
  int64_t opt_tile_permute = 1;
  uint32_t cap_hint = 0;
  bool stats_lazy = false;
  hipEvent_t launch_e0 = nullptr, launch_e1 = nullptr;
  std::vector<hipEvent_t> kl_pool;
  uint32_t prog_slot = 0;
  int64_t opt_time_launches = 0;
  int64_t opt_exact_lds = 1;
  int64_t opt_exact_img = 1;
  int64_t opt_exact_wgs = 1;
  int64_t opt_exact_prescan = 1;
  int64_t opt_exact_mfma = 1;
  int64_t opt_rescore8 = 2;

  DevBuf q32, q16, qscale, qinv, ebound, slack, thr, cnt, overflow, cand, out_ids, out_scores, misc, hitlog, prog;
  DevBuf hostblock;
  DevBuf tickets;
  int64_t opt_fuse = 1;
  int64_t opt_shadow_exact_thr = 1;
  int64_t opt_zero_copy = 1;
  bool status_by_kernel = false;
  size_t q32_dirty = 0;
  DevBuf rq, rcand, rout_ids, rout_dist;
  DevBuf rdbg;
  DevBuf xcdw;
  int64_t opt_xcd_balance = 1;
  int64_t opt_i8_lo_bits = 7;
  int64_t opt_boot_tiles = 0;
  int64_t opt_i8_small8 = 1;
  int64_t dbg_rows = 0;
  DevBuf lk_scores, lk_sel, lk_hist, lk_state;
  int64_t opt_refine_pinned = 0;
  int64_t opt_refine_dbg_q = 0;
  void* rpinned = nullptr;
  size_t rpinned_bytes = 0;
  int64_t opt_largek_budget_mb = 8192;
  DevBuf rg_radius, rg_kept, rg_off, rg_idx, rg_q, rg_desc, rg_taken, rg_slab;
  DevBuf rg_pcnt, rg_maskof;
  DevBuf rg_ids, rg_scores;
  uint64_t range_total = 0;
  bool range_valid = false;
  int64_t opt_range_max_mb = 4096;

  int64_t opt_path = 0, opt_chunk0 = 512, opt_cap = 0, opt_min_filter_batch = 1, opt_growth = 0;

  nvdb_hip_scan_stats stats{};
  uint32_t last_nq = 0, last_cap = 0;
  bool last_filter = false;
  std::vector<hipEvent_t> ev_pool;
  std::vector<std::pair<int, int>> ev_filter;
  struct KLaunch { hipEvent_t e0, e1; double flops, bytes; };
  std::vector<KLaunch> klaunch;
  int64_t opt_time_kernels = 0;
  int64_t opt_sync_every = 4, opt_sync_lead = 4;
  int64_t opt_sibling_sync = 1;
  int64_t opt_f32_shadow = 1;
  int64_t opt_mfma_boot = 1;
  int64_t opt_refine_v2 = 2;
  int64_t opt_mfma16 = 1;
  std::set<const void*> lds_attr_set;
  nvdbhip::PartState* parts = nullptr;
  DevBuf row_masks, mask_rows;
  uint32_t nmasks = 0;
};

#define HIPCHK(ctx, call)                                                                        \
  do {                                                                                           \
    hipError_t e_ = (call);                                                                      \
    if (e_ != hipSuccess) {                                                                      \
      (ctx)->err = std::string(#call) + ": " + hipGetErrorString(e_);                            \
      return NVDB_ERR_HIP;                                                                       \
    }                                                                                            \
  } while (0)

namespace nvdbhip {

inline nvdb_status fail(nvdb_hip_ctx* c, nvdb_status s, const std::string& msg) {
  c->err = msg;
  return s;
}

inline nvdb_status ensure(nvdb_hip_ctx* c, DevBuf& b, size_t bytes) {
  if (b.bytes >= bytes && b.p) return NVDB_OK;
  if (b.p) { HIPCHK(c, hipFree(b.p)); b.p = nullptr; b.bytes = 0; }
  size_t want = std::max<size_t>(bytes, 256);
  HIPCHK(c, hipMalloc(&b.p, want));
  b.bytes = want;
  return NVDB_OK;
}

inline size_t bpe_of(uint32_t dtype) { return dtype == NVDB_DTYPE_F32 ? 4 : (dtype == NVDB_DTYPE_F16 ? 2 : (dtype == NVDB_DTYPE_I8 ? 1 : 0)); }

inline bool aligned_rows(uint32_t dtype, uint32_t dim) {
  if (dtype == NVDB_DTYPE_F32) return dim % 4 == 0;
  return dim % 8 == 0;
}

template <int... D> struct DimList {};
using F16Dims = DimList<768, 640, 512, 384, 256, 128>;
using F16Dims16 = DimList<896, 1024, 1152, 1280, 1408, 1536>;
using F16DimsK2 = DimList<2048, 2560, 3072>;
using I8Dims = DimList<768, 640, 512, 384, 256>;
using I8DimsBig = DimList<896, 1024, 1152, 1280, 1408, 1536>;

template <int... D, typename F>
bool dispatch_dim(DimList<D...>, uint32_t dim, nvdb_status& st, F&& f) {
  return ((dim == static_cast<uint32_t>(D) && ((st = f(std::integral_constant<int, D>{})), true)) || ...);
}
template <int... D> bool has_dim(DimList<D...>, uint32_t dim) { return ((dim == static_cast<uint32_t>(D)) || ...); }

inline bool f16_filter_dim(uint32_t dim) { return has_dim(F16Dims{}, dim) || has_dim(F16Dims16{}, dim) || has_dim(F16DimsK2{}, dim); }
inline bool i8_filter_dim(uint32_t dim) { return has_dim(I8Dims{}, dim) || has_dim(I8DimsBig{}, dim); }
inline bool refine3_dim(uint32_t dim) { return dim == 768 || dim == 512 || dim == 384 || dim == 256; }

inline const signed char* filter_rows_i8(const nvdb_hip_ctx* c) { return c->shadow8 ? c->shadow8 : static_cast<const signed char*>(c->rows); }
inline const float* filter_scales_i8(const nvdb_hip_ctx* c) { return c->shadow8 ? c->shadow8_scales : c->scales; }
inline const _Float16* filter_rows_f16(const nvdb_hip_ctx* c) {
  return c->shadow16 ? c->shadow16 : static_cast<const _Float16*>(c->rows);
}

inline bool filter_is_i8(const nvdb_hip_ctx* c) { return c->dtype == NVDB_DTYPE_I8 || (c->q8shadow && c->use_shadow); }
inline bool f16_beside_shadow(const nvdb_hip_ctx* c) { return c->q8shadow && c->dtype == NVDB_DTYPE_F16 && f16_filter_dim(c->dim); }
inline bool shadow_preferred(const nvdb_hip_ctx* c) { return c->q8shadow && !(f16_beside_shadow(c) && (c->opt_q8_shadow == 0 || c->shadow_demoted)); }
inline uint64_t q8_shadow_bytes(uint64_t n, uint32_t dim) { return n * (static_cast<uint64_t>(dim) + 4u); }
inline bool q8_shadow_wanted(const nvdb_hip_ctx* c, uint64_t free_hbm) {
  if (c->opt_q8_shadow == 0 || c->dtype == NVDB_DTYPE_I8 || !i8_filter_dim(c->dim)) return false;
  if (c->opt_q8_shadow > 0) return true;
  const uint64_t bytes = q8_shadow_bytes(c->n, c->dim);
  return c->dtype == NVDB_DTYPE_F16 && f16_filter_dim(c->dim) && c->n >= static_cast<uint64_t>(c->opt_q8_auto_min_rows) &&
         bytes <= (static_cast<uint64_t>(c->opt_q8_auto_max_mb) << 20) && bytes <= free_hbm / 4;
}
inline bool filter_supported(const nvdb_hip_ctx* c) {
  if (c->q8shadow) return true;
  if (c->dtype == NVDB_DTYPE_F16) return f16_filter_dim(c->dim) || c->shadow16 != nullptr;
  if (c->dtype == NVDB_DTYPE_F32) return c->shadow16 != nullptr;
  if (c->dtype == NVDB_DTYPE_I8) return i8_filter_dim(c->dim) || c->shadow8 != nullptr;
  return false;
}

inline bool i8_two_stage(const nvdb_hip_ctx* c) { return filter_is_i8(c) && c->opt_i8_wide; }

inline uint32_t filter_nb(const nvdb_hip_ctx* c, uint32_t nq) {
  if (filter_is_i8(c) && (!i8_two_stage(c) || c->fdim > 768)) return 1u;
  if (!filter_is_i8(c) && c->fdim > 768) return 1u;
  return nq <= 128 ? 1u : 2u;
}

inline bool corpus_padded(const nvdb_hip_ctx* c) { return c->owned || c->shadow16 != nullptr || (c->shadow8 != nullptr && filter_is_i8(c)); }
inline bool f16_m16_build(const nvdb_hip_ctx* c, uint32_t nb) { return nb == 2 && c->opt_mfma16; }
constexpr uint32_t f16_m16_tile_rows(uint32_t dim) { return dim <= 384 ? 64u : 32u; }
constexpr uint32_t i8w_tile_rows(uint32_t dim) { return dim <= 768 ? I8W_TILE_ROWS : FILTER_ROWS; }
inline uint32_t filter_tile_rows(const nvdb_hip_ctx* c, uint32_t nq) {
  if (filter_is_i8(c)) return i8_two_stage(c) ? i8w_tile_rows(c->fdim) : FILTER_ROWS;
  return (c->fdim <= 768 && f16_m16_build(c, filter_nb(c, nq))) ? f16_m16_tile_rows(c->fdim) : FILTER_ROWS;
}
constexpr uint32_t f16_filter_qpb(uint32_t dim, uint32_t nb) { return dim > 1536 ? 64u : dim > 768 ? 128u : 128u * nb; }
constexpr uint32_t f16_m16_qpb(uint32_t nqb, uint32_t wpb) { return 16u * nqb * wpb; }
inline uint32_t filter_qpb(const nvdb_hip_ctx* c, uint32_t nq) { return filter_is_i8(c) ? 128u * filter_nb(c, nq) : f16_filter_qpb(c->fdim, filter_nb(c, nq)); }
inline bool i8_pipelined(const nvdb_hip_ctx* c, uint32_t nb) { return nb == 2 && c->opt_i8_pipe; }
inline bool i8_stage2_in_loop(const nvdb_hip_ctx* c) { return c->opt_i8_defer != 0 || c->i8_scales_signed; }
inline bool i8_logs_survivors(const nvdb_hip_ctx* c, uint32_t nb) { return i8_pipelined(c, nb) && !i8_stage2_in_loop(c); }

inline hipEvent_t get_event(nvdb_hip_ctx* c, size_t idx) {
  while (c->ev_pool.size() <= idx) { hipEvent_t e; (void)hipEventCreate(&e); c->ev_pool.push_back(e); }
  return c->ev_pool[idx];
}

nvdb_status launch_init_search(nvdb_hip_ctx* c, hipStream_t s, uint32_t nq_pad, uint32_t prog_words);
nvdb_status launch_scan_exact(nvdb_hip_ctx* c, hipStream_t s, uint32_t row_lo, uint32_t row_hi, const float* q32, uint32_t nq, uint32_t k,
                              const float* thr, uint32_t cap, uint32_t reserve);
nvdb_status launch_select(nvdb_hip_ctx* c, hipStream_t s, uint32_t nq, uint32_t cap, uint32_t k, const float* slack, int mode, uint64_t* out_ids,
                          float* out_scores, uint32_t out_k, const float* q32 = nullptr);
nvdb_status launch_rescore(nvdb_hip_ctx* c, hipStream_t s, const float* q32, uint32_t nq, uint32_t cap, FinalSelect fs = FinalSelect{}, bool* fused = nullptr);
nvdb_status search_largek(nvdb_hip_ctx* c, hipStream_t s, const float* dev_q, uint32_t nq, uint32_t k, uint64_t* dev_out_ids, float* dev_out_scores,
                          uint32_t n_rows = 0, Cand* seed_cand = nullptr, uint32_t* seed_cnt = nullptr, uint32_t seed_cap = 0);
nvdb_status score_matrix_batch(nvdb_hip_ctx* c, uint32_t nq, size_t per_query_bytes, size_t held_bytes, uint32_t& QB, uint32_t& QG);
nvdb_status launch_score_matrix(nvdb_hip_ctx* c, hipStream_t s, const float* q32, uint32_t nq, float* scores, uint64_t ld, uint32_t n, uint32_t QG, bool mfma_ok);
nvdb_status launch_sort_keys(nvdb_hip_ctx* c, hipStream_t s, unsigned long long* keys, uint32_t K2, uint32_t lists);
nvdb_status launch_prep_q16(nvdb_hip_ctx* c, hipStream_t s, const float* dev_q, uint32_t nq, uint32_t nq_pad, const PrepInit& pinit);
nvdb_status launch_prep_q8(nvdb_hip_ctx* c, hipStream_t s, const float* dev_q, uint32_t nq, uint32_t nq_pad, const PrepInit& pinit);
nvdb_status launch_filter_f16(nvdb_hip_ctx* c, hipStream_t s, uint32_t row_lo, uint32_t row_hi, uint32_t nq, uint32_t QT, uint32_t cap);
nvdb_status launch_filter_i8(nvdb_hip_ctx* c, hipStream_t s, uint32_t row_lo, uint32_t row_hi, uint32_t nq, uint32_t QT, uint32_t cap);
nvdb_status launch_boot_f16(nvdb_hip_ctx* c, hipStream_t s, uint32_t n0, uint32_t nq, uint32_t QT, uint32_t cap, uint32_t nb);
nvdb_status launch_boot_i8(nvdb_hip_ctx* c, hipStream_t s, uint32_t n0, uint32_t nq, uint32_t QT, uint32_t cap);
nvdb_status corpus_alloc_padded(nvdb_hip_ctx* c, uint64_t n, uint32_t dim, uint32_t dtype, void** rows, float** scales);
nvdb_status corpus_take_ownership(nvdb_hip_ctx* c, void* dev_rows, float* dev_scales, uint64_t n, uint32_t dim, uint32_t dtype, uint64_t global_row_base);
void parts_drop(nvdb_hip_ctx* c);
void parts_destroy(nvdb_hip_ctx* c);
nvdb_status ensure_q32(nvdb_hip_ctx* c, hipStream_t s, size_t qbytes);
nvdb_status zero_q32_pad(nvdb_hip_ctx* c, hipStream_t s, size_t qbytes);
nvdb_status next_prog_region(nvdb_hip_ctx* c, hipStream_t s, uint32_t nwg, uint32_t** out);
ScatterArgs scatter_args(nvdb_hip_ctx* c, uint32_t cap, uint32_t trows = 0);
float filter_events_ms(const nvdb_hip_ctx* c);
nvdb_status sum_candidates(nvdb_hip_ctx* c, unsigned long long* total);

inline nvdb_status raise_lds_limit(nvdb_hip_ctx* c, const void* fn, size_t bytes) {
  if (c->lds_attr_set.count(fn)) return NVDB_OK;
  HIPCHK(c, hipFuncSetAttribute(fn, hipFuncAttributeMaxDynamicSharedMemorySize, static_cast<int>(bytes)));
  c->lds_attr_set.insert(fn);
  return NVDB_OK;
}

inline uint32_t filter_grid(const nvdb_hip_ctx* c, uint32_t QT) {
  const uint32_t nwg = (static_cast<uint32_t>(c->num_cu) / QT) * QT;
  return nwg ? nwg : QT;
}

inline bool xcd_aware_grid(uint32_t QT, uint32_t nwg) { return (nwg & 7u) == 0 && ((nwg >> 3) % QT) == 0; }
inline bool sibling_sync_grid(const nvdb_hip_ctx* c, uint32_t QT, uint32_t nwg) { return c->opt_sibling_sync && QT > 1 && QT <= 8 && xcd_aware_grid(QT, nwg); }

struct SyncArgs { uint32_t* prog = nullptr; uint32_t mask = 0, lead = 0; };
inline nvdb_status sibling_sync_args(nvdb_hip_ctx* c, hipStream_t s, uint32_t QT, uint32_t nwg, SyncArgs& out) {
  out = SyncArgs{};
  if (!sibling_sync_grid(c, QT, nwg)) return NVDB_OK;
  out.mask = static_cast<uint32_t>(c->opt_sync_every - 1);
  out.lead = static_cast<uint32_t>(c->opt_sync_lead);
  return next_prog_region(c, s, nwg, &out.prog);
}

struct FilterCall { hipStream_t s; uint32_t row_lo, row_hi, nq, QT, cap; const float* thr; };
struct FilterGeom { uint32_t block; size_t lds; uint32_t log_waves; bool timed; };

template <typename T> inline T launch_arg(T a) { return a; }
inline Hit* launch_arg(DevBuf* b) { return static_cast<Hit*>(b->p); }

template <typename... KA, typename... A>
nvdb_status launch_filter_kernel(nvdb_hip_ctx* c, hipStream_t s, void (*kern)(KA...), uint32_t nwg, const FilterGeom& g, A... args) {
  nvdb_status st;
  if ((st = raise_lds_limit(c, reinterpret_cast<const void*>(kern), g.lds))) return st;
  if (g.log_waves && (st = ensure(c, c->hitlog, static_cast<size_t>(nwg) * g.log_waves * FILTER_LOGCAP * sizeof(Hit)))) return st;
  if (g.timed) hipExtLaunchKernelGGL(kern, dim3(nwg), dim3(g.block), g.lds, s, c->launch_e0, c->launch_e1, 0, launch_arg(args)...);
  else kern<<<nwg, g.block, g.lds, s>>>(launch_arg(args)...);
  HIPCHK(c, hipGetLastError());
  return NVDB_OK;
}

template <typename... KA, typename... Rest>
nvdb_status launch_filter_f16_kernel(nvdb_hip_ctx* c, const FilterCall& f, void (*kern)(KA...), uint32_t nwg, const FilterGeom& g, DevBuf* log,
                                     uint32_t trows, Rest... rest) {
  if (trows && (f.row_hi - f.row_lo) % trows) return fail(c, NVDB_ERR_INTERNAL, "fp16 filter kernel: row range is not a multiple of its tile");
  return launch_filter_kernel(c, f.s, kern, nwg, g, filter_rows_f16(c), f.row_lo, f.row_hi, static_cast<const _Float16*>(c->q16.p), f.nq, f.QT, f.thr,
                              static_cast<const float*>(c->qscale.p), static_cast<const float*>(c->qinv.p), log, scatter_args(c, f.cap, trows), rest...);
}

template <typename... KA, typename... Rest>
nvdb_status launch_filter_i8_kernel(nvdb_hip_ctx* c, const FilterCall& f, void (*kern)(KA...), uint32_t nwg, const FilterGeom& g, size_t qlo_off, Rest... rest) {
  const signed char* qhi = static_cast<const signed char*>(c->q16.p);
  return launch_filter_kernel(c, f.s, kern, nwg, g, filter_rows_i8(c), filter_scales_i8(c), f.row_lo, f.row_hi, qhi, qhi + qlo_off, f.nq, f.QT, f.thr,
                              static_cast<const float*>(c->qscale.p), static_cast<const float*>(c->qinv.p), rest...);
}
template <typename... KA>
nvdb_status launch_filter_i8w_kernel(nvdb_hip_ctx* c, const FilterCall& f, void (*kern)(KA...), uint32_t nwg, const FilterGeom& g, size_t qlo_off,
                                     uint32_t trows, const SyncArgs& sy) {
  return launch_filter_i8_kernel(c, f, kern, nwg, g, qlo_off, static_cast<const float*>(c->qdelta.p), &c->hitlog, scatter_args(c, f.cap, trows), sy.prog,
                                 sy.mask, sy.lead, static_cast<uint32_t*>(c->misc.p) + 4);
}

}
```

nano-vectordb_amd/csrc/nvdb_launch_i8.cpp:

```cpp
#include "nvdb_ctx.h"
#include "kernels_filter_i8s.h"

namespace nvdbhip {

nvdb_status launch_prep_q8(nvdb_hip_ctx* c, hipStream_t s, const float* dev_q, uint32_t nq, uint32_t nq_pad, const PrepInit& pinit) {
  prep_q8_kernel<<<nq_pad, 256, 0, s>>>(dev_q, nq, c->dim, c->fdim, c->filter_max_norm, c->q8shadow ? c->resid_max : 0.f, static_cast<signed char*>(c->q16.p),
                                        static_cast<signed char*>(c->q16.p) + static_cast<size_t>(nq_pad) * c->fdim,
                                        static_cast<float*>(c->qscale.p), static_cast<float*>(c->qinv.p),
                                        static_cast<float*>(c->ebound.p), static_cast<float*>(c->slack.p), static_cast<float*>(c->qdelta.p),
                                        static_cast<uint32_t*>(c->overflow.p), static_cast<uint32_t>(c->opt_i8_lo_bits), pinit);
  HIPCHK(c, hipGetLastError());
  return NVDB_OK;
}

#ifdef NVDB_HIP_DEV
template <int DIM>
nvdb_status launch_filter_i8_dim(nvdb_hip_ctx* c, const FilterCall& f, uint32_t nq_pad) {
  const uint32_t nwg = filter_grid(c, f.QT);
  nvdb_status st;
  SyncArgs sy;
  if ((st = sibling_sync_args(c, f.s, f.QT, nwg, sy))) return st;
  return launch_filter_i8_kernel(c, f, sy.prog ? filter_i8_kernel<DIM, false, 6, true> : filter_i8_kernel<DIM>, nwg, FilterGeom{256, filter_i8_lds_bytes<DIM>(), 4, true},
                                 static_cast<size_t>(nq_pad) * DIM, &c->hitlog, scatter_args(c, f.cap, FILTER_ROWS), 0u, sy.prog, sy.mask, sy.lead);
}
#endif

template <int DIM, int NB, int MB> auto i8w_build(bool sync) { return sync ? filter_i8w_kernel<DIM, NB, 6, true, MB> : filter_i8w_kernel<DIM, NB, 6, false, MB>; }
template <int DIM, int WPB, bool DEFER> auto i8p_build(bool sync) { return sync ? filter_i8p_kernel<DIM, true, false, 6, 0, WPB, DEFER> : filter_i8p_kernel<DIM, false, false, 6, 0, WPB, DEFER>; }
template <int DIM, int WPB> auto i8s_build(bool sync) { return sync ? filter_i8s_kernel<DIM, true, false, 6, 0, WPB> : filter_i8s_kernel<DIM, false, false, 6, 0, WPB>; }

template <int DIM, int NB>
nvdb_status launch_filter_i8w_dim(nvdb_hip_ctx* c, const FilterCall& f, uint32_t nq_pad) {
  constexpr uint32_t TROWS = i8w_tile_rows(DIM);
  static_assert(TROWS == I8W_TILE_ROWS, "the builds of dims <= 768 stream two 32-row blocks per tile");
  if ((f.row_hi - f.row_lo) % TROWS) return fail(c, NVDB_ERR_INTERNAL, "int8 two-stage kernel: row range is not a multiple of its 64-row tile");
  const bool pipe = i8_pipelined(c, NB);
  const bool defer = i8_stage2_in_loop(c), logs = i8_logs_survivors(c, NB);
#ifdef NVDB_HIP_DEV
  const bool w8 = pipe && c->opt_i8_waves8 && DIM != 384;
  constexpr bool HAS_I8W = true, HAS_I8P32 = true;
#else
  constexpr bool w8 = false;
  constexpr bool HAS_I8W = (NB == 1);
  constexpr bool HAS_I8P32 = (DIM < 384);
#endif
  const uint32_t nwg = filter_grid(c, f.QT);
  nvdb_status st;
  SyncArgs sy;
  if ((st = sibling_sync_args(c, f.s, f.QT, nwg, sy))) return st;
  const bool sync = sy.prog != nullptr;
  auto launch = [&](auto kern, uint32_t waves, size_t lds) {
    return launch_filter_i8w_kernel(c, f, kern, nwg, FilterGeom{64 * waves, lds, 8, true}, static_cast<size_t>(nq_pad) * DIM, TROWS, sy);
  };
  if constexpr (NB == 1 && (DIM == 768 || DIM == 512))
    if (c->opt_i8_small8 && !defer && f.QT == 1 && f.nq > 8)
      return launch(filter_i8s_kernel<DIM, false, false, 6, 0, 8>, 8, filter_i8s_lds_bytes<DIM, 8>());
  if constexpr (NB == 1 && DIM == 384)
    if (c->opt_i8_small8 && !defer && f.QT == 1 && f.nq > 64)
      return launch(filter_i8s_kernel<DIM, false, false, 6, 0, 4>, 4, filter_i8s_lds_bytes<DIM, 4>());
  if (logs && c->opt_i8_mfma16) {
#ifdef NVDB_HIP_DEV
    if constexpr (DIM == 768 || DIM == 512)
      if (w8 && DIM == 768) return launch(i8s_build<DIM, 8>(sync), 8, filter_i8s_lds_bytes<DIM, 8>());
#endif
    if constexpr (DIM >= 384)
      if (!w8) return launch(i8s_build<DIM, 4>(sync), 4, filter_i8s_lds_bytes<DIM, 4>());
  }
#ifdef NVDB_HIP_DEV
  if constexpr (DIM != 384)
    if (w8) return launch(i8p_build<DIM, 8, true>(sync), 8, filter_i8p_lds_bytes<DIM, 8, true>());
#endif
  if (pipe && defer) return launch(i8p_build<DIM, 4, true>(sync), 4, filter_i8p_lds_bytes<DIM, 4, true>());
  if constexpr (HAS_I8P32)
    if (pipe) return launch(i8p_build<DIM, 4, false>(sync), 4, filter_i8p_lds_bytes<DIM, 4, false>());
  if constexpr (HAS_I8W)
    if (!pipe) return launch(i8w_build<DIM, NB, 2>(sync), 4, filter_i8w_lds_bytes<DIM, 2>());
  return fail(c, NVDB_ERR_INTERNAL, "int8 two-stage kernel: no build for this batch");
}

template <int DIM>
nvdb_status launch_filter_i8w_big_dim(nvdb_hip_ctx* c, const FilterCall& f, uint32_t nq_pad) {
  constexpr uint32_t TROWS = i8w_tile_rows(DIM);
  static_assert(TROWS == FILTER_ROWS, "the builds of dims > 768 stream one 32-row block per tile");
  if ((f.row_hi - f.row_lo) % TROWS) return fail(c, NVDB_ERR_INTERNAL, "int8 kernel: row range is not a multiple of its 32-row tile");
  const uint32_t nwg = filter_grid(c, f.QT);
  nvdb_status st;
  SyncArgs sy;
  if ((st = sibling_sync_args(c, f.s, f.QT, nwg, sy))) return st;
  return launch_filter_i8w_kernel(c, f, i8w_build<DIM, 1, 1>(sy.prog != nullptr), nwg, FilterGeom{256, filter_i8w_lds_bytes<DIM, 1>(), 4, true},
                                  static_cast<size_t>(nq_pad) * DIM, TROWS, sy);
}

template <int DIM>
nvdb_status launch_boot_i8_dim(nvdb_hip_ctx* c, const FilterCall& f) {
  return launch_filter_i8_kernel(c, f, filter_i8_kernel<DIM, true>, filter_grid(c, f.QT), FilterGeom{256, filter_i8_lds_bytes<DIM>(), 0, false},
                                 static_cast<size_t>(f.QT) * 128u * DIM, &c->cand, scatter_args(c, f.cap, FILTER_ROWS), f.cap, static_cast<uint32_t*>(nullptr), 0u, 0u);
}

nvdb_status launch_boot_i8(nvdb_hip_ctx* c, hipStream_t s, uint32_t n0, uint32_t nq, uint32_t QT, uint32_t cap) {
  const FilterCall f{s, 0, n0, nq, QT, cap, static_cast<const float*>(c->thr.p)};
  nvdb_status st;
  if (dispatch_dim(I8Dims{}, c->fdim, st, [&](auto D) { return launch_boot_i8_dim<decltype(D)::value>(c, f); })) return st;
  return fail(c, NVDB_ERR_UNSUPPORTED, "int8 boot kernel: unsupported dim");
}

nvdb_status launch_filter_i8(nvdb_hip_ctx* c, hipStream_t s, uint32_t row_lo, uint32_t row_hi, uint32_t nq, uint32_t QT, uint32_t cap) {
  const uint32_t nb = filter_nb(c, nq);
  const uint32_t nq_pad = QT * filter_qpb(c, nq);
  const FilterCall f{s, row_lo, row_hi, nq, QT, cap, static_cast<const float*>(c->thr.p)};
  nvdb_status st;
  if (dispatch_dim(I8DimsBig{}, c->fdim, st, [&](auto D) { return launch_filter_i8w_big_dim<decltype(D)::value>(c, f, nq_pad); })) return st;
  if (i8_two_stage(c) && dispatch_dim(I8Dims{}, c->fdim, st, [&](auto D) {
        return nb == 2 ? launch_filter_i8w_dim<decltype(D)::value, 2>(c, f, nq_pad) : launch_filter_i8w_dim<decltype(D)::value, 1>(c, f, nq_pad);
      })) return st;
#ifdef NVDB_HIP_DEV
  if (dispatch_dim(I8Dims{}, c->fdim, st, [&](auto D) { return launch_filter_i8_dim<decltype(D)::value>(c, f, nq_pad); })) return st;
#endif
  return fail(c, NVDB_ERR_UNSUPPORTED, "int8 filter kernel: unsupported dim");
}

}
```

nano-vectordb_amd/csrc/nvdb_search.cpp:

```cpp
#include "nvdb_plan.h"

namespace nvdbhip {

nvdb_status ensure_hostblock(nvdb_hip_ctx* c, size_t out_bytes) {
  const size_t need = 64 + out_bytes;
  if (c->hostblock.p && c->hostblock.bytes >= need) return NVDB_OK;
  HIPCHK(c, hipDeviceSynchronize());
  void* np = nullptr;
  const size_t want = std::max<size_t>(need + need / 2, static_cast<size_t>(1) << 20);
  HIPCHK(c, hipMalloc(&np, want));
  if (c->misc.p) HIPCHK(c, hipMemcpy(np, c->misc.p, 64, hipMemcpyDeviceToDevice));
  else HIPCHK(c, hipMemset(np, 0, 64));
  if (c->hostblock.p) HIPCHK(c, hipFree(c->hostblock.p));
  else if (c->misc.p) HIPCHK(c, hipFree(c->misc.p));
  c->hostblock.p = np; c->hostblock.bytes = want;
  c->misc.p = np; c->misc.bytes = 64;
  return NVDB_OK;
}

nvdb_status ensure_q32(nvdb_hip_ctx* c, hipStream_t s, size_t qbytes) {
  const size_t before = c->q32.p ? c->q32.bytes : 0;
  if (nvdb_status st = ensure(c, c->q32, qbytes + 8 * static_cast<size_t>(c->dim) * 4)) return st;
  if (c->q32.bytes != before) { HIPCHK(c, hipMemsetAsync(c->q32.p, 0, c->q32.bytes, s)); c->q32_dirty = 0; }
  return NVDB_OK;
}
nvdb_status zero_q32_pad(nvdb_hip_ctx* c, hipStream_t s, size_t qbytes) {
  const size_t pad_bytes = 8 * static_cast<size_t>(c->dim) * 4;
  if (c->q32_dirty > qbytes) HIPCHK(c, hipMemsetAsync(static_cast<char*>(c->q32.p) + qbytes, 0, std::min(pad_bytes, c->q32_dirty - qbytes), s));
  c->q32_dirty = std::max(c->q32_dirty, qbytes);
  return NVDB_OK;
}

nvdb_status next_prog_region(nvdb_hip_ctx* c, hipStream_t s, uint32_t nwg, uint32_t** out) {
  const size_t region_words = static_cast<size_t>(c->num_cu) * 8;
  if (nwg * 8u > region_words) return fail(c, NVDB_ERR_INTERNAL, "rendezvous region too small for this grid");
  uint32_t* base = static_cast<uint32_t*>(c->prog.p) + static_cast<size_t>(c->prog_slot % PROG_SLOTS) * region_words;
  if (c->prog_slot >= PROG_SLOTS) HIPCHK(c, hipMemsetAsync(base, 0xFF, region_words * 4, s));
  ++c->prog_slot;
  *out = base;
  return NVDB_OK;
}

ScatterArgs scatter_args(nvdb_hip_ctx* c, uint32_t cap, uint32_t trows) {
  ScatterArgs a{static_cast<Cand*>(c->cand.p), static_cast<uint32_t*>(c->cnt.p), static_cast<uint32_t*>(c->overflow.p),
                static_cast<uint32_t*>(c->misc.p) + 1, cap, static_cast<uint32_t>(c->n), 1u, 0u, 0u,
                c->opt_xcd_balance ? static_cast<float*>(c->xcdw.p) : nullptr, static_cast<uint32_t>(c->opt_i8_lo_bits)};
  if (trows && c->perm_on) {
    const uint32_t n = static_cast<uint32_t>(c->n);
    a.perm_T = corpus_padded(c) ? (n + trows - 1) / trows : n / trows;
    perm_params(a.perm_T, a.perm_mul, a.perm_mask);
  }
  return a;
}

nvdb_status launch_boot(nvdb_hip_ctx* c, hipStream_t s, uint32_t n0, uint32_t nq, uint32_t QT, uint32_t cap, uint32_t nb) {
  return filter_is_i8(c) ? launch_boot_i8(c, s, n0, nq, QT * nb, cap) : launch_boot_f16(c, s, n0, nq, QT, cap, nb);
}

nvdb_status launch_filter(nvdb_hip_ctx* c, hipStream_t s, uint32_t row_lo, uint32_t row_hi, uint32_t nq, uint32_t QT, uint32_t cap) {
  return filter_is_i8(c) ? launch_filter_i8(c, s, row_lo, row_hi, nq, QT, cap) : launch_filter_f16(c, s, row_lo, row_hi, nq, QT, cap);
}

nvdb_status search_core(nvdb_hip_ctx* c, hipStream_t s, const float* dev_q, uint32_t nq, uint32_t k, uint64_t* dev_out_ids,
                        float* dev_out_scores, int force_path, bool time_filter, uint32_t cap_override = 0, bool sticky = true,
                        const float* host_q = nullptr, uint32_t* status_out = nullptr) {
  c->status_by_kernel = false;
  SearchPlan p;
  nvdb_status st = plan_search(*c, nq, k, force_path, cap_override, p);
  if (st) return fail(c, st, p.error);
  const int final_mode = sticky ? 1 : 3;
  const uint32_t n = static_cast<uint32_t>(c->n), k_eff = p.k_eff, cap = p.cap, QT = p.QT;
  const size_t per_q = static_cast<size_t>(p.nq_pad) * 4;
  const struct { DevBuf& buf; size_t bytes; bool filter_flow; } workspace[] = {
      {c->thr, per_q, false}, {c->cnt, per_q, false}, {c->overflow, per_q, false}, {c->cand, static_cast<size_t>(nq) * cap * sizeof(Cand), false},
      {c->misc, 64, false}, {c->prog, static_cast<size_t>(p.prog_words) * 4, false}, {c->tickets, FUSE_TICKETS * 4, false},
      {c->q16, static_cast<size_t>(p.nq_pad) * c->fdim * 2, true}, {c->qscale, per_q, true}, {c->qinv, per_q, true},
      {c->ebound, per_q, true}, {c->slack, per_q, true}, {c->qdelta, per_q, true}};
  for (const auto& w : workspace)
    if ((p.prep || !w.filter_flow) && (st = ensure(c, w.buf, w.bytes))) return st;
  c->stats = nvdb_hip_scan_stats{};
  c->stats.path = p.route;
  c->last_nq = nq; c->last_cap = cap; c->last_filter = p.route == ROUTE_FILTER;
  c->ev_filter.clear();
  c->prog_slot = 0;
  if (p.route == ROUTE_FILTER) c->perm_on = p.perm_on;
  c->last_filter_kind = p.route != ROUTE_FILTER ? 0u : p.shadow ? 2u : c->dtype == NVDB_DTYPE_I8 ? 3u : 1u;

  if (host_q && !p.prep_inits) { HIPCHK(c, hipMemcpyAsync(const_cast<float*>(dev_q), host_q, static_cast<size_t>(nq) * c->dim * 4, hipMemcpyDefault, s)); host_q = nullptr; }
  if (!p.prep_inits && (st = launch_init_search(c, s, p.nq_pad, QT > 1 ? p.prog_words : 0u))) return st;
  const PrepInit pinit = p.prep_inits ? PrepInit{static_cast<uint32_t*>(c->cnt.p), static_cast<float*>(c->thr.p), static_cast<uint32_t*>(c->misc.p),
                                                 static_cast<uint32_t*>(c->prog.p), QT > 1 ? p.prog_words : 0u, static_cast<uint32_t*>(c->tickets.p), host_q, const_cast<float*>(dev_q)}
                                      : PrepInit{nullptr, nullptr, nullptr, nullptr, 0u, nullptr, nullptr, nullptr};
  if (p.prep && (st = filter_is_i8(c) ? launch_prep_q8(c, s, dev_q, nq, p.nq_pad, pinit) : launch_prep_q16(c, s, dev_q, nq, p.nq_pad, pinit))) return st;
  const float* thr = static_cast<const float*>(c->thr.p);
  const float* slack = static_cast<const float*>(c->slack.p);

  if (p.route == ROUTE_ANYK) return search_largek(c, s, dev_q, nq, k, dev_out_ids, dev_out_scores);
  if (p.route == ROUTE_EXACT) {
    if (p.head && (st = launch_scan_exact(c, s, 0, p.head, dev_q, nq, k_eff, nullptr, cap, 0))) return st;
    if (p.head && (st = launch_select(c, s, nq, cap, k_eff, nullptr, 0, nullptr, nullptr, 0))) return st;
    if ((st = launch_scan_exact(c, s, p.head, n, dev_q, nq, k_eff, p.head ? thr : nullptr, cap, p.head ? k_eff : 0))) return st;
    c->stats.chunks = p.head ? 2 : 1;
    c->stats.rows_scanned = c->n;
    return launch_select(c, s, nq, cap, k_eff, nullptr, final_mode, dev_out_ids, dev_out_scores, k);
  }

  if (p.boot == BOOT_MFMA) st = launch_boot(c, s, p.boot_rows, nq, QT, cap, filter_nb(c, nq));
  else if (p.boot == BOOT_ANYK_SEEDED) st = search_largek(c, s, dev_q, nq, k_eff, nullptr, nullptr, p.r0, static_cast<Cand*>(c->cand.p), static_cast<uint32_t*>(c->cnt.p), cap);
  else st = launch_scan_exact(c, s, 0, p.r0, dev_q, nq, k_eff, nullptr, cap, 0);
  if (st) return st;
  const float* xthr_q = (p.shadow && k_eff <= WAVE_KMAX && c->opt_shadow_exact_thr) ? dev_q : nullptr;
  if ((st = launch_select(c, s, nq, cap, k_eff, slack, p.boot == BOOT_MFMA ? 2 : 0, nullptr, nullptr, p.boot == BOOT_MFMA ? p.boot_tiles : 0, xthr_q))) return st;
  size_t ev = 0;
  for (uint32_t r = p.r0; r < p.n_al;) {
    const uint32_t hi = chunk_end(p, r);
    nvdb_hip_ctx::KLaunch kl{nullptr, nullptr, 0.0, 0.0};
    const bool acct = c->opt_time_kernels && c->klaunch.size() < 8192;
    if (acct) {
      for (hipEvent_t* e : {&kl.e0, &kl.e1}) {
        if (!c->kl_pool.empty()) { *e = c->kl_pool.back(); c->kl_pool.pop_back(); }
        else HIPCHK(c, hipEventCreate(e));
      }
      kl.flops = 2.0 * nq * static_cast<double>(std::min(hi, n) - r) * c->dim;
      kl.bytes = static_cast<double>(std::min(hi, n) - r) * (filter_is_i8(c) ? c->fdim + 4.0 : c->fdim * 2.0);
      c->launch_e0 = kl.e0; c->launch_e1 = kl.e1;
    } else if (time_filter) {
      c->launch_e0 = get_event(c, ev); c->launch_e1 = get_event(c, ev + 1);
    }
    if (time_filter && acct) { HIPCHK(c, hipEventRecord(get_event(c, ev), s)); }
    st = launch_filter(c, s, r, hi, nq, QT, cap);
    c->launch_e0 = nullptr; c->launch_e1 = nullptr;
    if (st) return st;
    if (time_filter && acct) { HIPCHK(c, hipEventRecord(get_event(c, ev + 1), s)); }
    if (time_filter) { c->ev_filter.emplace_back(ev, ev + 1); ev += 2; }
    if (acct) c->klaunch.push_back(kl);
    if ((st = launch_select(c, s, nq, cap, k_eff, slack, 0, nullptr, nullptr, 0, xthr_q))) return st;
    c->stats.chunks++;
    c->stats.rows_scanned += static_cast<uint64_t>(hi - r) * QT;
    r = hi;
  }
  if (p.tail_exact && (st = launch_scan_exact(c, s, p.n_al, n, dev_q, nq, std::min(k_eff, WAVE_KMAX), thr, cap, 0))) return st;
  if (p.tail_exact) c->stats.rows_scanned += static_cast<uint64_t>(n - p.n_al) * QT;
  FinalSelect fs{};
  if (c->opt_fuse)
    fs = FinalSelect{final_mode, k_eff, k, c->row_base, reinterpret_cast<unsigned long long*>(dev_out_ids), dev_out_scores, static_cast<float*>(c->thr.p),
                     static_cast<uint32_t*>(c->overflow.p), static_cast<uint32_t*>(c->misc.p) + 6,
                     p.prep_inits ? static_cast<uint32_t*>(c->tickets.p) + (FUSE_TICKETS - 1) : nullptr, p.prep_inits ? status_out : nullptr};
  if (fs.mode == 1 && fs.ticket == nullptr) fs.mode = 0;
  bool fused = false;
  if ((st = launch_rescore(c, s, dev_q, nq, cap, fs, &fused))) return st;
  if (fused) { c->status_by_kernel = fs.status_out != nullptr; return NVDB_OK; }
  return launch_select(c, s, nq, cap, k_eff, nullptr, final_mode, dev_out_ids, dev_out_scores, k);
}

float filter_events_ms(const nvdb_hip_ctx* c) {
  float total = 0.f;
  for (auto& pr : c->ev_filter) { float ms = 0.f; if (hipEventElapsedTime(&ms, c->ev_pool[pr.first], c->ev_pool[pr.second]) == hipSuccess) total += ms; }
  return total;
}

// ... 259 lines not shown
```

Baseline: 154,600.

## Add per-row residual credit to tighten int8 shadow filter verification

Stores per-row quantization scale and residual norm in an interleaved buffer next to the shadow scales, and records per-query norms during int8 query prep. A new CREDIT variant of the i8 shadow filter kernel uses the gap between the corpus-wide max residual and the row's own residual to tighten the keep test, so fewer candidates get scattered for exact rescoring. The kernel body moves into a shared include so both variants share code. In exchange the kernel reads an extra per-row buffer and doubles the per-stage side-channel LDS, and the tighter bound carries some risk to correctness.

```diff
diff --git a/nano-vectordb_amd/csrc/kernels_corpus.h b/nano-vectordb_amd/csrc/kernels_corpus.h
--- a/nano-vectordb_amd/csrc/kernels_corpus.h
+++ b/nano-vectordb_amd/csrc/kernels_corpus.h
@@ -67,9 +67,10 @@
 
 template <typename SrcT>
 __global__ __launch_bounds__(256) void shadow_q8_kernel(const SrcT* __restrict__ src, signed char* __restrict__ dst, float* __restrict__ dst_scales,
-                                                        uint64_t n, uint32_t dim, uint32_t sdim, uint32_t* __restrict__ out_bits) {
+                                                        uint64_t n, uint32_t dim, uint32_t sdim, uint32_t* __restrict__ out_bits,
+                                                        float* __restrict__ dst_resid = nullptr) {
   const int lane = threadIdx.x & 63;
-  float wres = 0.f;
+  float wres = 0.f, wscale = 0.f;
   bool bad = false;
   for (uint64_t r = static_cast<uint64_t>(blockIdx.x) * 4 + (threadIdx.x >> 6); r < n; r += static_cast<uint64_t>(gridDim.x) * 4) {
     const SrcT* row = src + r * dim;
@@ -91,9 +92,13 @@
     for (int o = 32; o > 0; o >>= 1) ss += __shfl_xor(ss, o);
     if (!(ss == ss)) bad = true;
     if (lane == 0) dst_scales[r] = scale;
-    wres = fmaxf(wres, sqrtf(ss) * 1.0001f);
+    const float res = sqrtf(ss) * 1.0001f;
+    if (lane == 0 && dst_resid) { dst_resid[row_credit_index(r) - 64] = scale; dst_resid[row_credit_index(r)] = res; }
+    wres = fmaxf(wres, res);
+    wscale = fmaxf(wscale, scale);
   }
   if (lane == 0 && wres > 0.f) atomicMax(out_bits, __builtin_bit_cast(uint32_t, wres));
+  if (lane == 0 && wscale > 0.f) atomicMax(out_bits + 2, __builtin_bit_cast(uint32_t, wscale));
   if (lane == 0 && (bad || !(wres < 3.0e38f))) out_bits[1] = 1u;
 }
 
diff --git a/nano-vectordb_amd/csrc/kernels_filter.h b/nano-vectordb_amd/csrc/kernels_filter.h
--- a/nano-vectordb_amd/csrc/kernels_filter.h
+++ b/nano-vectordb_amd/csrc/kernels_filter.h
@@ -105,6 +105,9 @@
 constexpr int I8_ACC_BIAS = 0x4B000000;
 __device__ __forceinline__ int shl_i32(int v, uint32_t bits) { return static_cast<int>(static_cast<uint32_t>(v) << bits); }
 constexpr uint32_t FILTER_LOGCAP = 4096;
+
+struct RowCredit { const float* resid; const float* qn; float resid_max; float scale_max; };
+__host__ __device__ inline uint64_t row_credit_index(uint64_t row) { return (row >> 6) * 128u + 64u + (row & 63u); }
 
 struct ScatterArgs {
   Cand* cand;
@@ -775,14 +778,15 @@
                                                       float max_row_norm, float corpus_resid, signed char* __restrict__ qhi,
                                                       signed char* __restrict__ qlo, float* __restrict__ qscale,
                                                       float* __restrict__ qinv, float* __restrict__ ebound,
-                                                      float* __restrict__ slack, float* __restrict__ qdelta, uint32_t* __restrict__ overflow, uint32_t lo_bits, PrepInit pi) {
+                                                      float* __restrict__ slack, float* __restrict__ qdelta, uint32_t* __restrict__ overflow, uint32_t lo_bits, PrepInit pi,
+                                                      float* __restrict__ qn = nullptr) {
   __shared__ float red_max[4], red_ss[4];
   __shared__ uint32_t red_lo[4];
   const uint32_t q = blockIdx.x, tid = threadIdx.x;
   const float* src = prep_init(pi, q32, q, tid, nq, dim, overflow);
   if (q >= nq) {
     for (uint32_t i = tid; i < sdim; i += 256) { qhi[static_cast<uint64_t>(q) * sdim + i] = 0; qlo[static_cast<uint64_t>(q) * sdim + i] = 0; }
-    if (tid == 0) { qscale[q] = 1.f; qinv[q] = 1.f; ebound[q] = 0.f; slack[q] = 0.f; qdelta[q] = 0.f; }
+    if (tid == 0) { qscale[q] = 1.f; qinv[q] = 1.f; ebound[q] = 0.f; slack[q] = 0.f; qdelta[q] = 0.f; if (qn) qn[q] = 0.f; }
     return;
   }
   float mx = 0.f, ss = 0.f;
@@ -837,6 +841,7 @@
     const float eb = (0.5005f * sqrtf(static_cast<float>(dim)) * sq + 1.0e-5f * nrm) * max_row_norm * 1.001f + nrm * corpus_resid * 1.001f + 1e-30f;
     qscale[q] = isq; qinv[q] = sq; ebound[q] = eb; slack[q] = 2.f * eb;
     if (!(ss < 3.0e38f)) { overflow[q] = 1u; ebound[q] = -1.f; }
+    if (qn) qn[q] = (ss < 3.0e38f) ? nrm * 1.001f : 0.f;
   }
 }
 
@@ -1327,10 +1332,10 @@
   scatter_own_log(mylog, wcnt, sa, lane);
 }
 
-template <int DIM>
+template <int DIM, bool CREDIT = false>
 __device__ __forceinline__ void verify_and_scatter_i8(const Hit* mylog, uint32_t wcnt, const ScatterArgs& a, int lane, const signed char* __restrict__ rows,
                                                       const signed char* __restrict__ qlo, const float* __restrict__ thr, const float* __restrict__ qscale,
-                                                      const float* __restrict__ qinv) {
+                                                      const float* __restrict__ qinv, const RowCredit& rc = RowCredit{}) {
   asm volatile("s_waitcnt vmcnt(0)" ::: "memory");
   uint32_t n = wcnt;
   if (n > FILTER_LOGCAP) { if (lane == 0) *a.log_overflow = 1u; n = FILTER_LOGCAP; }
@@ -1374,7 +1379,14 @@
       part[j] += __builtin_amdgcn_update_dpp(0, part[j], 0x4E, 0xF, 0xF, true);
       if (valid[j] && part4 == 0) {
         const float fv = static_cast<float>(shl_i32(H[j], a.lo_bits) + part[j]) * __builtin_bit_cast(float, sbits[j]);
-        if (fv >= thr[qid[j]] * qscale[qid[j]]) {
+        bool keep = fv >= thr[qid[j]] * qscale[qid[j]];
+        if constexpr (CREDIT) {
+          if (keep) {
+            const float credit = rc.qn[qid[j]] * qscale[qid[j]] * 0.99999f * (rc.resid_max - rc.resid[row_credit_index(row[j])]);
+            keep = !(credit > 0.f) || fv - credit >= thr[qid[j]] * qscale[qid[j]];
+          }
+        }
+        if (keep) {
           const uint32_t slot = atomicAdd(&a.cnt[qid[j]], 1u);
           if (slot < a.cap) a.cand[static_cast<uint64_t>(qid[j]) * a.cap + slot] = Cand{fv * qinv[qid[j]], row[j]};
           else a.overflow[qid[j]] = 1u;
diff --git a/nano-vectordb_amd/csrc/kernels_filter_i8s.h b/nano-vectordb_amd/csrc/kernels_filter_i8s.h
--- a/nano-vectordb_amd/csrc/kernels_filter_i8s.h
+++ b/nano-vectordb_amd/csrc/kernels_filter_i8s.h
@@ -8,7 +8,8 @@
 #define NVDB_MFMA_I8S_FROM(acc, a, b, c0) asm volatile("v_mfma_i32_16x16x64_i8 %0, %1, %2, %3" : "=&v"(acc) : "v"(a), "a"(b), "v"(c0))
 #define NVDB_MFMA_I8S_ACC(acc, a, b) asm volatile("v_mfma_i32_16x16x64_i8 %0, %1, %2, %0" : "+v"(acc) : "v"(a), "a"(b))
 
-template <int DIM, int WPB = 4> constexpr size_t filter_i8s_lds_bytes() { return static_cast<size_t>(3) * (2 * FILTER_ROWS * DIM + WPB * 256); }
+template <int DIM, int WPB = 4, bool CREDIT = false> constexpr size_t filter_i8s_lds_bytes() { return static_cast<size_t>(3) * (2 * FILTER_ROWS * DIM + WPB * 256 * (CREDIT ? 2 : 1)); }
+
 template <int DIM, bool SYNC = false, bool STAMP = false, int RING = 6, int VAR = 0, int WPB = 4>
 __global__ __launch_bounds__(64 * WPB, 1) void filter_i8s_kernel(
     const signed char* __restrict__ rows, const float* __restrict__ scales, uint32_t row_lo, uint32_t row_hi,
@@ -16,276 +17,21 @@
     const float* __restrict__ thr, const float* __restrict__ qscale, const float* __restrict__ qinv,
     const float* __restrict__ qdelta, Hit* __restrict__ hitlog, ScatterArgs sa, uint32_t* __restrict__ prog,
     uint32_t sync_mask, uint32_t sync_lead, uint32_t* __restrict__ stage_counts) {
-  static_assert(WPB == 4 || WPB == 8, "4 waves x 64 queries or 8 waves x 32 queries");
-  constexpr bool NOTEST = VAR == 1 || VAR == 3 || VAR == 4;
-  constexpr int NB = 16 / WPB, MB = 2;
-  constexpr int NV = 8 * NB;
-  constexpr int KS = DIM / 64;
-  constexpr int ROW_BYTES = DIM;
-  constexpr int TROWS = FILTER_ROWS * MB;
-  constexpr int NSTAGE = 3;
-  constexpr int DATA_BYTES = TROWS * ROW_BYTES;
-  constexpr int STAGE_BYTES = DATA_BYTES + WPB * 256;
-  constexpr int PIECES = DATA_BYTES / 1024, PPW = PIECES / WPB;
-  constexpr int CHUNKS_PER_ROW = ROW_BYTES / 16;
-  constexpr int NSLOT = 2 * NB * KS;
-  constexpr int NFRAG = 2 * KS;
-  static_assert(DIM % 128 == 0 && DIM <= 768, "row stride multiple of 128 bytes (swz_chunk); 64 queries x DIM bytes = 192 AGPRs at most");
-  static_assert(PIECES % WPB == 0 && PPW % 2 == 0 && NSTAGE * STAGE_BYTES <= 160 * 1024 && PPW + 1 < 64 && NFRAG >= RING, "shape / LDS / vmcnt range");
-  static_assert(NSTAGE * STAGE_BYTES == filter_i8s_lds_bytes<DIM, WPB>(), "the launchers size the dynamic LDS with filter_i8s_lds_bytes");
+  constexpr bool CREDIT = false;
+  const RowCredit rc{};
+#include "kernels_filter_i8s_body.h"
+}
 
-  extern __shared__ __attribute__((aligned(16))) char smem[];
-  const int tid = threadIdx.x, lane = tid & 63, wave = __builtin_amdgcn_readfirstlane(tid >> 6);
-  const int x15 = lane & 15, g4 = lane >> 4;
-  const uint32_t wave_gid = blockIdx.x * WPB + wave;
-
-  const uint32_t nwg = gridDim.x, b = blockIdx.x;
-  const uint32_t S = nwg / QT;
-  uint32_t stream, qt;
-  if ((nwg & 7u) == 0 && ((nwg >> 3) % QT) == 0) { const uint32_t xcd = b & 7u, i = b >> 3; qt = i % QT; stream = (i / QT) * 8u + xcd; }
-  else { qt = b % QT; stream = b / QT; }
-  const uint32_t tiles_total = (row_hi - row_lo) / TROWS;
-  const bool xcd_map = (nwg & 7u) == 0 && ((nwg >> 3) % QT) == 0;
-  uint32_t t_lo, t_hi;
-  stream_tile_range(tiles_total, S, stream, xcd_map, sa.xcdw, t_lo, t_hi);
-  const uint32_t NT = t_hi - t_lo;
-  if (NT == 0) return;
-
-  const uint32_t qbase = qt * 256u + wave * (16u * NB);
-  float4_t bq[NB * KS];
-#pragma unroll
-  for (int f = 0; f < NB * KS; ++f) {
-    const int nb = f / KS, s = f % KS;
-    bq[f] = *reinterpret_cast<const float4_t*>(qhi + static_cast<uint64_t>(qbase + nb * 16 + x15) * DIM + 64 * s + 16 * g4);
-  }
-#pragma unroll
-  for (int f = 0; f < NB * KS; ++f) asm volatile("" ::"a"(bq[f]));
-  intx4_t bias0;
-#pragma unroll
-  for (int r = 0; r < 4; ++r) bias0[r] = I8_ACC_BIAS;
-  asm volatile("" : "+v"(bias0));
-  uint32_t qid[NB];
-  float t1q[NB];
-  const float lo_unit = __builtin_bit_cast(float, (127u - sa.lo_bits) << 23);
-#pragma unroll
-  for (int nb = 0; nb < NB; ++nb) {
-    qid[nb] = qbase + nb * 16 + x15;
-    const bool real = qid[nb] < nq;
-    const float T = real ? thr[qid[nb]] * qscale[qid[nb]] : __builtin_huge_valf();
-    t1q[nb] = real ? (T - (1.001f * qdelta[qid[nb]] + 2e-6f * fabsf(T) + 1e-5f)) * lo_unit : __builtin_huge_valf();
-    asm volatile("" ::"v"(t1q[nb]));
-  }
-  const bool wave_has_queries = qbase < nq;
-
-  uint32_t src_off[PPW];
-#pragma unroll
-  for (int i = 0; i < PPW; ++i) {
-    const uint32_t P = static_cast<uint32_t>((wave * PPW + i) * 64 + lane);
-    const uint32_t r = P / CHUNKS_PER_ROW, cpos = P % CHUNKS_PER_ROW;
-    src_off[i] = r * ROW_BYTES + (swz_chunk<ROW_BYTES>(cpos, r) << 4);
-  }
-  const uint32_t sc_off = (lane & (8 * MB - 1)) * 16;
-  const uint32_t a16 = static_cast<uint32_t>(x15) * ROW_BYTES + (swz_chunk<ROW_BYTES>(static_cast<uint32_t>(g4), static_cast<uint32_t>(x15)) << 4);
-
-  const char* gbase = reinterpret_cast<const char*>(rows);
-  const uint32_t lds_base = static_cast<uint32_t>(reinterpret_cast<uintptr_t>(NVDB_LPTR(smem)));
-  const uint32_t g_lo = row_lo / TROWS + t_lo;
-  auto tile_row0 = [&](uint32_t t_rel) -> uint32_t { return perm_tile(g_lo + (t_rel < NT ? t_rel : NT - 1), sa) * TROWS; };
-  auto issue_piece = [&](uint32_t row0, uint32_t buf, int i) {
-    glds16(src_off[i], gbase + static_cast<uint64_t>(row0) * ROW_BYTES, lds_base + buf * STAGE_BYTES + (wave * PPW + i) * 1024);
-  };
-  auto issue_scales = [&](uint32_t row0, uint32_t buf) {
-    if (lane < 8 * MB) glds16(sc_off, reinterpret_cast<const char*>(scales + row0), lds_base + buf * STAGE_BYTES + DATA_BYTES + wave * 256);
-  };
-  auto loop_piece = [&](uint32_t row0, uint32_t buf, int i) { if constexpr (VAR != 3) issue_piece(row0, buf, i); };
-  auto loop_scales = [&](uint32_t row0, uint32_t buf) { if constexpr (VAR != 3) issue_scales(row0, buf); };
-#pragma unroll
-  for (int st = 0; st < NSTAGE - 1; ++st) {
-#pragma unroll
-    for (int i = 0; i < PPW; ++i) issue_piece(tile_row0(st), st, i);
-    issue_scales(tile_row0(st), st);
-  }
-
-  uint32_t wcnt = 0, n_stage1 = 0;
-  Hit* mylog = hitlog + static_cast<uint64_t>(wave_gid) * FILTER_LOGCAP;
-
-  intx4_t acc0[2][NB], acc1[2][NB];
-  float scv[2][8], scc[2][8];
-#pragma unroll
-  for (int i = 0; i < 8; ++i) { scv[0][i] = scv[1][i] = 0.f; scc[0][i] = scc[1][i] = 0.f; }
-#pragma unroll
-  for (int h = 0; h < 2; ++h)
-#pragma unroll
-    for (int nb = 0; nb < NB; ++nb) acc1[h][nb] = bias0;
-  float mx[NB][2];
-  float4_t ar[RING];
-
-  auto read_a = [&](const char* stage, int u, int mb) -> float4_t {
-    const int s = u >> 1, h = u & 1;
-    if constexpr (VAR == 4) { float4_t z = {0.f, 1.f, 2.f, 3.f}; asm volatile("" : "+v"(z)); return z; }
-    const uint32_t off = swz16<ROW_BYTES>() ? (a16 ^ ((s & 3) << 6)) + (s >> 2) * 256 : (a16 ^ ((s & 1) << 6)) + (s >> 1) * 128;
-    return *reinterpret_cast<const float4_t*>(stage + off + (2 * mb + h) * 16 * ROW_BYTES);
-  };
-  constexpr int SW0 = NSLOT >= 64 ? 8 : 4;
-  auto scale_step = [&](const char* stage, int mb, int set, int w) {
-    if constexpr (NOTEST) return;
-    if (w == 0) {
-      const float* sc_lds = reinterpret_cast<const float*>(stage + DATA_BYTES + wave * 256);
-#pragma unroll
-      for (int h = 0; h < 2; ++h) {
-        const float4 v = *reinterpret_cast<const float4*>(sc_lds + 32 * mb + 16 * h + 4 * g4);
-        scv[set][4 * h] = v.x; scv[set][4 * h + 1] = v.y; scv[set][4 * h + 2] = v.z; scv[set][4 * h + 3] = v.w;
-      }
-    }
-    const int i = w - SW0;
-    if (i >= 0 && i < 8) scc[set][i] = scv[set][i] * -8388608.f;
-  };
-  float tm[NV];
-  constexpr int W0 = SW0 + 10;
-  constexpr int SPU = (NSLOT - W0 - 4) / NV >= 2 ? 2 : 1;
-  static_assert(W0 + NV * SPU + 2 <= NSLOT, "the test ends before the half's last MFMA");
-  auto test_step = [&](const intx4_t (&a)[2][NB], const float (&sc)[8], const float (&sccs)[8], int w) {
-    if constexpr (NOTEST) return;
-    const int rel = w - W0;
-    if (rel < 0 || rel % SPU != 0) return;
-    const int v = rel / SPU;
-    if (v < NV) {
-      const int nb = v >> 3, h = (v >> 2) & 1, j = v & 3;
-      const int b0 = a[h][nb][j];
-      tm[v] = __builtin_fmaf(__builtin_bit_cast(float, b0), sc[4 * h + j], sccs[4 * h + j]);
-    }
-    const int p = v - 1;
-    if (p >= 0 && p < NV && (p & 1)) mx[p >> 3][(p >> 2) & 1] = vmax3(mx[p >> 3][(p >> 2) & 1], tm[p - 1], tm[p]);
-  };
-  auto reset_max = [&]() {
-#pragma unroll
-    for (int nb = 0; nb < NB; ++nb) { mx[nb][0] = -__builtin_huge_valf(); mx[nb][1] = -__builtin_huge_valf(); }
-  };
-  float flagv = -1.f;
-  auto combine_flags = [&]() {
-    if constexpr (NOTEST) return;
-    float m[NB];
-#pragma unroll
-    for (int nb = 0; nb < NB; ++nb) m[nb] = vmax3(mx[nb][0], mx[nb][1], mx[nb][1]) - t1q[nb];
-    flagv = NB == 4 ? vmax3(vmax3(m[0], m[1], m[NB / 2]), m[NB - 1], m[NB - 1]) : vmax3(m[0], m[NB - 1], m[NB - 1]);
-  };
-  auto any_flag = [&]() -> bool { return __builtin_amdgcn_ballot_w64(flagv >= 0.f) != 0; };
-  auto rare_log = [&](const intx4_t (&a)[2][NB], const float (&sc)[8], uint32_t row0, int mb) {
-    ++n_stage1;
-#pragma unroll
-    for (int nb = 0; nb < NB; ++nb)
-#pragma unroll
-      for (int h = 0; h < 2; ++h) {
-        if (!__builtin_amdgcn_ballot_w64(mx[nb][h] >= t1q[nb])) continue;
-#pragma unroll
-        for (int j = 0; j < 4; ++j) {
-          const int H = a[h][nb][j] - I8_ACC_BIAS;
-          const bool hit = static_cast<float>(H) * sc[4 * h + j] >= t1q[nb];
-          const unsigned long long m = __builtin_amdgcn_ballot_w64(hit);
-          if (m) {
-            const uint32_t idx = wcnt + static_cast<uint32_t>(__builtin_popcountll(m & ((1ull << lane) - 1ull)));
-            if (hit && idx < FILTER_LOGCAP)
-              mylog[idx] = Hit{sc[4 * h + j], row0 + 32u * mb + 16u * h + 4u * g4 + j, qid[nb], static_cast<uint32_t>(H)};
-            wcnt += static_cast<uint32_t>(__builtin_popcountll(m));
-          }
-        }
-      }
-  };
-
-  uint32_t sync_strikes = 0;
-  uint64_t stamp_c = 0, stamp_r = 0;
-  if constexpr (STAMP) { stamp_c = __builtin_amdgcn_s_memtime(); stamp_r = __builtin_amdgcn_s_memrealtime(); }
-  const uint32_t xw_t0 = static_cast<uint32_t>(__builtin_amdgcn_s_memrealtime());
-  constexpr int HP = PPW / 2, HP0 = HP < 3 ? HP : 3;
-  constexpr int D1 = (HP - HP0) > 0 ? (HP - HP0) : 1;
-  constexpr int EV1 = NFRAG / D1, EV2 = NFRAG / (PPW - HP);
-  static_assert((HP == HP0 || NFRAG % (HP - HP0) == 0) && NFRAG % (PPW - HP) == 0, "pieces spread evenly over the A fragments of both halves");
-  for (uint32_t t = 0; t < NT; ++t) {
-    if constexpr (SYNC) {
-      if (wave == 0 && (t & sync_mask) == 0) sibling_rendezvous(prog + static_cast<uint64_t>(stream) * 8, qt, t, sync_lead, sync_strikes, lane);
-    }
-    asm volatile("s_waitcnt vmcnt(%0)" ::"n"(PPW + 1) : "memory");
-    __builtin_amdgcn_s_barrier();
-    const uint32_t next_row0 = tile_row0(t + 2), next_buf = (t + 2) % NSTAGE;
-    const char* stage = smem + (t % NSTAGE) * STAGE_BYTES;
-    if (!wave_has_queries) {
-#pragma unroll
-      for (int i = 0; i < PPW; ++i) issue_piece(next_row0, next_buf, i);
-      issue_scales(next_row0, next_buf);
-      continue;
-    }
-    reset_max();
-#pragma unroll
-    for (int u = 0; u < RING - 1; ++u) ar[u] = read_a(stage, u, 0);
-#pragma unroll
-    for (int i = 0; i < HP0; ++i) loop_piece(next_row0, next_buf, i);
-    __builtin_amdgcn_sched_barrier(0);
-#pragma unroll
-    for (int u = 0; u < NFRAG; ++u) {
-      if (u + RING - 1 < NFRAG) ar[(u + RING - 1) % RING] = read_a(stage, u + RING - 1, 0);
-      else ar[(u + RING - 1) % RING] = read_a(stage, u + RING - 1 - NFRAG, 1);
-      const float4_t av = ar[u % RING];
-      const int s = u >> 1, h = u & 1;
-#pragma unroll
-      for (int nb = 0; nb < NB; ++nb) {
-        if (s == 0) NVDB_MFMA_I8S_FROM(acc0[h][nb], av, bq[nb * KS], bias0);
-        else NVDB_MFMA_I8S_ACC(acc0[h][nb], av, bq[nb * KS + s]);
-        const int w = NB * u + nb;
-        scale_step(stage, 0, 0, w);
-        test_step(acc1, scv[1], scc[1], w);
-        if (w == NSLOT - 1) combine_flags();
-        __builtin_amdgcn_sched_barrier(0);
-      }
-      if constexpr (HP > HP0) {
-        if (u % EV1 == EV1 - 1) loop_piece(next_row0, next_buf, HP0 + u / EV1);
-        __builtin_amdgcn_sched_barrier(0);
-      }
-    }
-    if (VAR == 0 && t > 0 && any_flag()) rare_log(acc1, scv[1], tile_row0(t - 1), 1);
-    if constexpr (VAR != 0) { asm volatile("" ::"v"(flagv)); }
-    reset_max();
-    constexpr int R0 = NFRAG % RING;
-#pragma unroll
-    for (int u = 0; u < NFRAG; ++u) {
-      if (u + RING - 1 < NFRAG) ar[(R0 + u + RING - 1) % RING] = read_a(stage, u + RING - 1, 1);
-      const float4_t av = ar[(R0 + u) % RING];
-      const int s = u >> 1, h = u & 1;
-#pragma unroll
-      for (int nb = 0; nb < NB; ++nb) {
-        if (s == 0) NVDB_MFMA_I8S_FROM(acc1[h][nb], av, bq[nb * KS], bias0);
-        else NVDB_MFMA_I8S_ACC(acc1[h][nb], av, bq[nb * KS + s]);
-        const int w = NB * u + nb;
-        scale_step(stage, 1, 1, w);
-        test_step(acc0, scv[0], scc[0], w);
-        if (w == NSLOT - 1) combine_flags();
-        __builtin_amdgcn_sched_barrier(0);
-      }
-      if (u % EV2 == EV2 - 1) loop_piece(next_row0, next_buf, HP + u / EV2);
-      if (u == 0) loop_scales(next_row0, next_buf);
-      __builtin_amdgcn_sched_barrier(0);
-    }
-    if (VAR == 0 && any_flag()) rare_log(acc0, scv[0], tile_row0(t), 0);
-    if constexpr (VAR != 0) { asm volatile("" ::"v"(flagv)); }
-  }
-  if (wave_has_queries) {
-    asm volatile("s_nop 15\n\ts_nop 15" ::: "memory");
-    reset_max();
-#pragma unroll
-    for (int w = W0; w < W0 + (NV + 1) * SPU; ++w) test_step(acc1, scv[1], scc[1], w);
-    combine_flags();
-    if (VAR == 0 && any_flag()) rare_log(acc1, scv[1], tile_row0(NT - 1), 1);
-  }
-  if constexpr (STAMP) {
-    const uint64_t dc = __builtin_amdgcn_s_memtime() - stamp_c, dr = __builtin_amdgcn_s_memrealtime() - stamp_r;
-    if (wave == 0 && lane == 0) {
-      uint64_t* out = reinterpret_cast<uint64_t*>(prog + static_cast<uint64_t>(gridDim.x) * 8) + static_cast<uint64_t>(blockIdx.x) * 2;
-      out[0] = dc; out[1] = dr;
-    }
-  }
-  if constexpr (SYNC) { if (wave == 0 && lane == 0) __hip_atomic_store(prog + static_cast<uint64_t>(stream) * 8 + qt, 0xFFFFFFFFu, __ATOMIC_RELAXED, __HIP_MEMORY_SCOPE_AGENT); }
-  if (stage_counts && lane == 0 && n_stage1) atomicAdd(stage_counts, n_stage1);
-  if (wave == 0 && lane == 0) record_xcd_speed(sa.xcdw, xcd_map, stream & 7u, NT, static_cast<uint32_t>(__builtin_amdgcn_s_memrealtime()) - xw_t0);
-  verify_and_scatter_i8<DIM>(mylog, wcnt, sa, lane, rows, qlo, thr, qscale, qinv);
+template <int DIM, bool SYNC = false>
+__global__ __launch_bounds__(256, 1) void shadow_i8s_kernel(
+    const signed char* __restrict__ rows, const float* __restrict__ scales, uint32_t row_lo, uint32_t row_hi,
+    const signed char* __restrict__ qhi, const signed char* __restrict__ qlo, uint32_t nq, uint32_t QT,
+    const float* __restrict__ thr, const float* __restrict__ qscale, const float* __restrict__ qinv,
+    const float* __restrict__ qdelta, Hit* __restrict__ hitlog, ScatterArgs sa, uint32_t* __restrict__ prog,
+    uint32_t sync_mask, uint32_t sync_lead, uint32_t* __restrict__ stage_counts, RowCredit rc) {
+  constexpr bool CREDIT = true, STAMP = false;
+  constexpr int RING = 6, VAR = 0, WPB = 4;
+#include "kernels_filter_i8s_body.h"
 }
 
 }
diff --git a/nano-vectordb_amd/csrc/kernels_filter_i8s_body.h b/nano-vectordb_amd/csrc/kernels_filter_i8s_body.h
--- /dev/null
+++ b/nano-vectordb_amd/csrc/kernels_filter_i8s_body.h
@@ -0,0 +1,301 @@
+  static_assert(WPB == 4 || WPB == 8, "4 waves x 64 queries or 8 waves x 32 queries");
+  constexpr bool NOTEST = VAR == 1 || VAR == 3 || VAR == 4;
+  constexpr int NB = 16 / WPB, MB = 2;
+  constexpr int NV = 8 * NB;
+  constexpr int KS = DIM / 64;
+  constexpr int ROW_BYTES = DIM;
+  constexpr int TROWS = FILTER_ROWS * MB;
+  constexpr int NSTAGE = 3;
+  constexpr int DATA_BYTES = TROWS * ROW_BYTES;
+  constexpr int STAGE_BYTES = DATA_BYTES + WPB * 256 * (CREDIT ? 2 : 1);
+  constexpr int PIECES = DATA_BYTES / 1024, PPW = PIECES / WPB;
+  constexpr int VMT = PPW + 1;
+  constexpr int SLOT = CREDIT ? 512 : 256;
+  constexpr int CHUNKS_PER_ROW = ROW_BYTES / 16;
+  constexpr int NSLOT = 2 * NB * KS;
+  constexpr int NFRAG = 2 * KS;
+  static_assert(DIM % 128 == 0 && DIM <= 768, "row stride multiple of 128 bytes (swz_chunk); 64 queries x DIM bytes = 192 AGPRs at most");
+  static_assert(PIECES % WPB == 0 && PPW % 2 == 0 && NSTAGE * STAGE_BYTES <= 160 * 1024 && VMT < 64 && NFRAG >= RING, "shape / LDS / vmcnt range");
+  static_assert(NSTAGE * STAGE_BYTES == filter_i8s_lds_bytes<DIM, WPB, CREDIT>(), "the launchers size the dynamic LDS with filter_i8s_lds_bytes");
+
+  extern __shared__ __attribute__((aligned(16))) char smem[];
+  const int tid = threadIdx.x, lane = tid & 63, wave = __builtin_amdgcn_readfirstlane(tid >> 6);
+  const int x15 = lane & 15, g4 = lane >> 4;
+  const uint32_t wave_gid = blockIdx.x * WPB + wave;
+
+  const uint32_t nwg = gridDim.x, b = blockIdx.x;
+  const uint32_t S = nwg / QT;
+  uint32_t stream, qt;
+  if ((nwg & 7u) == 0 && ((nwg >> 3) % QT) == 0) { const uint32_t xcd = b & 7u, i = b >> 3; qt = i % QT; stream = (i / QT) * 8u + xcd; }
+  else { qt = b % QT; stream = b / QT; }
+  const uint32_t tiles_total = (row_hi - row_lo) / TROWS;
+  const bool xcd_map = (nwg & 7u) == 0 && ((nwg >> 3) % QT) == 0;
+  uint32_t t_lo, t_hi;
+  stream_tile_range(tiles_total, S, stream, xcd_map, sa.xcdw, t_lo, t_hi);
+  const uint32_t NT = t_hi - t_lo;
+  if (NT == 0) return;
+
+  const uint32_t qbase = qt * 256u + wave * (16u * NB);
+  float4_t bq[NB * KS];
+#pragma unroll
+  for (int f = 0; f < NB * KS; ++f) {
+    const int nb = f / KS, s = f % KS;
+    bq[f] = *reinterpret_cast<const float4_t*>(qhi + static_cast<uint64_t>(qbase + nb * 16 + x15) * DIM + 64 * s + 16 * g4);
+  }
+#pragma unroll
+  for (int f = 0; f < NB * KS; ++f) asm volatile("" ::"a"(bq[f]));
+  intx4_t bias0;
+#pragma unroll
+  for (int r = 0; r < 4; ++r) bias0[r] = I8_ACC_BIAS;
+  asm volatile("" : "+v"(bias0));
+  uint32_t qid[NB];
+  float t1q[NB];
+  const float lo_unit = __builtin_bit_cast(float, (127u - sa.lo_bits) << 23);
+#pragma unroll
+  for (int nb = 0; nb < NB; ++nb) {
+    qid[nb] = qbase + nb * 16 + x15;
+    const bool real = qid[nb] < nq;
+    const float T = real ? thr[qid[nb]] * qscale[qid[nb]] : __builtin_huge_valf();
+    t1q[nb] = real ? (T - (1.001f * qdelta[qid[nb]] + 2e-6f * fabsf(T) + 1e-5f)) * lo_unit : __builtin_huge_valf();
+    asm volatile("" ::"v"(t1q[nb]));
+  }
+  float g = 0.f, ngr = 0.f;
+  RowCredit rcv = rc;
+  if constexpr (CREDIT) asm volatile("" : "+v"(rcv.qn), "+v"(rcv.resid_max));
+  if constexpr (CREDIT) {
+    float gm = __builtin_huge_valf();
+#pragma unroll
+    for (int nb = 0; nb < NB; ++nb)
+      if (qid[nb] < nq) gm = fminf(gm, rc.qn[qid[nb]] * qscale[qid[nb]]);
+    g = (gm < 3.0e38f && gm > 0.f && rc.resid_max > 0.f) ? gm * lo_unit * 0.99999f : 0.f;
+    ngr = -(g * rc.resid_max);
+    const float adj = g > 0.f ? 0.51f * rc.scale_max : 0.f;
+#pragma unroll
+    for (int nb = 0; nb < NB; ++nb) { t1q[nb] -= adj; asm volatile("" ::"v"(t1q[nb])); }
+    asm volatile("" : "+v"(g), "+v"(ngr));
+  }
+  const bool wave_has_queries = qbase < nq;
+
+  uint32_t src_off[PPW];
+#pragma unroll
+  for (int i = 0; i < PPW; ++i) {
+    const uint32_t P = static_cast<uint32_t>((wave * PPW + i) * 64 + lane);
+    const uint32_t r = P / CHUNKS_PER_ROW, cpos = P % CHUNKS_PER_ROW;
+    src_off[i] = r * ROW_BYTES + (swz_chunk<ROW_BYTES>(cpos, r) << 4);
+  }
+  const uint32_t sc_off = (lane & (8 * MB - 1)) * 16;
+  const uint32_t a16 = static_cast<uint32_t>(x15) * ROW_BYTES + (swz_chunk<ROW_BYTES>(static_cast<uint32_t>(g4), static_cast<uint32_t>(x15)) << 4);
+
+  const char* gbase = reinterpret_cast<const char*>(rows);
+  const uint32_t lds_base = static_cast<uint32_t>(reinterpret_cast<uintptr_t>(NVDB_LPTR(smem)));
+  const uint32_t g_lo = row_lo / TROWS + t_lo;
+  auto tile_row0 = [&](uint32_t t_rel) -> uint32_t { return perm_tile(g_lo + (t_rel < NT ? t_rel : NT - 1), sa) * TROWS; };
+  auto issue_piece = [&](uint32_t row0, uint32_t buf, int i) {
+    glds16(src_off[i], gbase + static_cast<uint64_t>(row0) * ROW_BYTES, lds_base + buf * STAGE_BYTES + (wave * PPW + i) * 1024);
+  };
+  auto issue_scales = [&](uint32_t row0, uint32_t buf) {
+    if constexpr (CREDIT) {
+      if (lane < 16 * MB) glds16((lane & (16 * MB - 1)) * 16, reinterpret_cast<const char*>(rc.resid + static_cast<uint64_t>(row0) * 2), lds_base + buf * STAGE_BYTES + DATA_BYTES + wave * SLOT);
+    } else {
+      if (lane < 8 * MB) glds16(sc_off, reinterpret_cast<const char*>(scales + row0), lds_base + buf * STAGE_BYTES + DATA_BYTES + wave * 256);
+    }
+  };
+  auto loop_piece = [&](uint32_t row0, uint32_t buf, int i) { if constexpr (VAR != 3) issue_piece(row0, buf, i); };
+  auto loop_scales = [&](uint32_t row0, uint32_t buf) { if constexpr (VAR != 3) issue_scales(row0, buf); };
+#pragma unroll
+  for (int st = 0; st < NSTAGE - 1; ++st) {
+#pragma unroll
+    for (int i = 0; i < PPW; ++i) issue_piece(tile_row0(st), st, i);
+    issue_scales(tile_row0(st), st);
+  }
+
+  uint32_t wcnt = 0, n_stage1 = 0;
+  Hit* mylog = hitlog + static_cast<uint64_t>(wave_gid) * FILTER_LOGCAP;
+
+  intx4_t acc0[2][NB], acc1[2][NB];
+  float scv[2][8], scc[2][8];
+#pragma unroll
+  for (int i = 0; i < 8; ++i) { scv[0][i] = scv[1][i] = 0.f; scc[0][i] = scc[1][i] = 0.f; }
+#pragma unroll
+  for (int h = 0; h < 2; ++h)
+#pragma unroll
+    for (int nb = 0; nb < NB; ++nb) acc1[h][nb] = bias0;
+  float mx[NB][2];
+  float4_t ar[RING];
+
+  auto read_a = [&](const char* stage, int u, int mb) -> float4_t {
+    const int s = u >> 1, h = u & 1;
+    if constexpr (VAR == 4) { float4_t z = {0.f, 1.f, 2.f, 3.f}; asm volatile("" : "+v"(z)); return z; }
+    const uint32_t off = swz16<ROW_BYTES>() ? (a16 ^ ((s & 3) << 6)) + (s >> 2) * 256 : (a16 ^ ((s & 1) << 6)) + (s >> 1) * 128;
+    return *reinterpret_cast<const float4_t*>(stage + off + (2 * mb + h) * 16 * ROW_BYTES);
+  };
+  constexpr int SW0 = NSLOT >= 64 ? 8 : 4;
+  auto scale_step = [&](const char* stage, int mb, int set, int w) {
+    if constexpr (NOTEST) return;
+    if (w == 0) {
+      const float* sc_lds = reinterpret_cast<const float*>(stage + DATA_BYTES + wave * SLOT);
+#pragma unroll
+      for (int h = 0; h < 2; ++h) {
+        const float4 v = *reinterpret_cast<const float4*>(sc_lds + 32 * mb + 16 * h + 4 * g4);
+        scv[set][4 * h] = v.x; scv[set][4 * h + 1] = v.y; scv[set][4 * h + 2] = v.z; scv[set][4 * h + 3] = v.w;
+        if constexpr (CREDIT) {
+          const float4 r = *reinterpret_cast<const float4*>(sc_lds + 64 + 32 * mb + 16 * h + 4 * g4);
+          scc[set][4 * h] = r.x; scc[set][4 * h + 1] = r.y; scc[set][4 * h + 2] = r.z; scc[set][4 * h + 3] = r.w;
+        }
+      }
+    }
+    const int i = w - SW0;
+    if constexpr (CREDIT) {
+      if (i >= 0 && i < 8) scc[set][i] = __builtin_fmaf(scv[set][i], -8388608.f, __builtin_fmaf(g, scc[set][i], ngr));
+    } else {
+      if (i >= 0 && i < 8) scc[set][i] = scv[set][i] * -8388608.f;
+    }
+  };
+  float tm[NV];
+  constexpr int W0 = SW0 + 10;
+  constexpr int SPU = (NSLOT - W0 - 4) / NV >= 2 ? 2 : 1;
+  static_assert(W0 + NV * SPU + 2 <= NSLOT, "the test ends before the half's last MFMA");
+  auto test_step = [&](const intx4_t (&a)[2][NB], const float (&sc)[8], const float (&sccs)[8], int w) {
+    if constexpr (NOTEST) return;
+    const int rel = w - W0;
+    if (rel < 0 || rel % SPU != 0) return;
+    const int v = rel / SPU;
+    if (v < NV) {
+      const int nb = v >> 3, h = (v >> 2) & 1, j = v & 3;
+      const int b0 = a[h][nb][j];
+      tm[v] = __builtin_fmaf(__builtin_bit_cast(float, b0), sc[4 * h + j], sccs[4 * h + j]);
+    }
+    const int p = v - 1;
+    if (p >= 0 && p < NV && (p & 1)) mx[p >> 3][(p >> 2) & 1] = vmax3(mx[p >> 3][(p >> 2) & 1], tm[p - 1], tm[p]);
+  };
+  auto reset_max = [&]() {
+#pragma unroll
+    for (int nb = 0; nb < NB; ++nb) { mx[nb][0] = -__builtin_huge_valf(); mx[nb][1] = -__builtin_huge_valf(); }
+  };
+  float flagv = -1.f;
+  auto combine_flags = [&]() {
+    if constexpr (NOTEST) return;
+    float m[NB];
+#pragma unroll
+    for (int nb = 0; nb < NB; ++nb) m[nb] = vmax3(mx[nb][0], mx[nb][1], mx[nb][1]) - t1q[nb];
+    flagv = NB == 4 ? vmax3(vmax3(m[0], m[1], m[NB / 2]), m[NB - 1], m[NB - 1]) : vmax3(m[0], m[NB - 1], m[NB - 1]);
+  };
+  auto any_flag = [&]() -> bool { return __builtin_amdgcn_ballot_w64(flagv >= 0.f) != 0; };
+  auto rare_log = [&](const intx4_t (&a)[2][NB], const float (&sc)[8], const float (&sccs)[8], uint32_t row0, int mb) {
+    ++n_stage1;
+#pragma unroll
+    for (int nb = 0; nb < NB; ++nb)
+#pragma unroll
+      for (int h = 0; h < 2; ++h) {
+        if (!__builtin_amdgcn_ballot_w64(mx[nb][h] >= t1q[nb])) continue;
+#pragma unroll
+        for (int j = 0; j < 4; ++j) {
+          const int H = a[h][nb][j] - I8_ACC_BIAS;
+          bool hit;
+          if constexpr (CREDIT) hit = __builtin_fmaf(__builtin_bit_cast(float, a[h][nb][j]), sc[4 * h + j], sccs[4 * h + j]) >= t1q[nb];
+          else hit = static_cast<float>(H) * sc[4 * h + j] >= t1q[nb];
+          const unsigned long long m = __builtin_amdgcn_ballot_w64(hit);
+          if (m) {
+            const uint32_t idx = wcnt + static_cast<uint32_t>(__builtin_popcountll(m & ((1ull << lane) - 1ull)));
+            if (hit && idx < FILTER_LOGCAP)
+              mylog[idx] = Hit{sc[4 * h + j], row0 + 32u * mb + 16u * h + 4u * g4 + j, qid[nb], static_cast<uint32_t>(H)};
+            wcnt += static_cast<uint32_t>(__builtin_popcountll(m));
+          }
+        }
+      }
+  };
+
+  uint32_t sync_strikes = 0;
+  uint64_t stamp_c = 0, stamp_r = 0;
+  if constexpr (STAMP) { stamp_c = __builtin_amdgcn_s_memtime(); stamp_r = __builtin_amdgcn_s_memrealtime(); }
+  const uint32_t xw_t0 = static_cast<uint32_t>(__builtin_amdgcn_s_memrealtime());
+  constexpr int HP = PPW / 2, HP0 = HP < 3 ? HP : 3;
+  constexpr int D1 = (HP - HP0) > 0 ? (HP - HP0) : 1;
+  constexpr int EV1 = NFRAG / D1, EV2 = NFRAG / (PPW - HP);
+  static_assert((HP == HP0 || NFRAG % (HP - HP0) == 0) && NFRAG % (PPW - HP) == 0, "pieces spread evenly over the A fragments of both halves");
+  for (uint32_t t = 0; t < NT; ++t) {
+    if constexpr (SYNC) {
+      if (wave == 0 && (t & sync_mask) == 0) sibling_rendezvous(prog + static_cast<uint64_t>(stream) * 8, qt, t, sync_lead, sync_strikes, lane);
+    }
+    asm volatile("s_waitcnt vmcnt(%0)" ::"n"(VMT) : "memory");
+    __builtin_amdgcn_s_barrier();
+    const uint32_t next_row0 = tile_row0(t + 2), next_buf = (t + 2) % NSTAGE;
+    const char* stage = smem + (t % NSTAGE) * STAGE_BYTES;
+    if (!wave_has_queries) {
+#pragma unroll
+      for (int i = 0; i < PPW; ++i) issue_piece(next_row0, next_buf, i);
+      issue_scales(next_row0, next_buf);
+      continue;
+    }
+    reset_max();
+#pragma unroll
+    for (int u = 0; u < RING - 1; ++u) ar[u] = read_a(stage, u, 0);
+#pragma unroll
+    for (int i = 0; i < HP0; ++i) loop_piece(next_row0, next_buf, i);
+    __builtin_amdgcn_sched_barrier(0);
+#pragma unroll
+    for (int u = 0; u < NFRAG; ++u) {
+      if (u + RING - 1 < NFRAG) ar[(u + RING - 1) % RING] = read_a(stage, u + RING - 1, 0);
+      else ar[(u + RING - 1) % RING] = read_a(stage, u + RING - 1 - NFRAG, 1);
+      const float4_t av = ar[u % RING];
+      const int s = u >> 1, h = u & 1;
+#pragma unroll
+      for (int nb = 0; nb < NB; ++nb) {
+        if (s == 0) NVDB_MFMA_I8S_FROM(acc0[h][nb], av, bq[nb * KS], bias0);
+        else NVDB_MFMA_I8S_ACC(acc0[h][nb], av, bq[nb * KS + s]);
+        const int w = NB * u + nb;
+        scale_step(stage, 0, 0, w);
+        test_step(acc1, scv[1], scc[1], w);
+        if (w == NSLOT - 1) combine_flags();
+        __builtin_amdgcn_sched_barrier(0);
+      }
+      if constexpr (HP > HP0) {
+        if (u % EV1 == EV1 - 1) loop_piece(next_row0, next_buf, HP0 + u / EV1);
+        __builtin_amdgcn_sched_barrier(0);
+      }
+    }
+    if (VAR == 0 && t > 0 && any_flag()) rare_log(acc1, scv[1], scc[1], tile_row0(t - 1), 1);
+    if constexpr (VAR != 0) { asm volatile("" ::"v"(flagv)); }
+    reset_max();
+    constexpr int R0 = NFRAG % RING;
+#pragma unroll
+    for (int u = 0; u < NFRAG; ++u) {
+      if (u + RING - 1 < NFRAG) ar[(R0 + u + RING - 1) % RING] = read_a(stage, u + RING - 1, 1);
+      const float4_t av = ar[(R0 + u) % RING];
+      const int s = u >> 1, h = u & 1;
+#pragma unroll
+      for (int nb = 0; nb < NB; ++nb) {
+        if (s == 0) NVDB_MFMA_I8S_FROM(acc1[h][nb], av, bq[nb * KS], bias0);
+        else NVDB_MFMA_I8S_ACC(acc1[h][nb], av, bq[nb * KS + s]);
+        const int w = NB * u + nb;
+        scale_step(stage, 1, 1, w);
+        test_step(acc0, scv[0], scc[0], w);
+        if (w == NSLOT - 1) combine_flags();
+        __builtin_amdgcn_sched_barrier(0);
+      }
+      if (u % EV2 == EV2 - 1) loop_piece(next_row0, next_buf, HP + u / EV2);
+      if (u == 0) loop_scales(next_row0, next_buf);
+      __builtin_amdgcn_sched_barrier(0);
+    }
+    if (VAR == 0 && any_flag()) rare_log(acc0, scv[0], scc[0], tile_row0(t), 0);
+    if constexpr (VAR != 0) { asm volatile("" ::"v"(flagv)); }
+  }
+  if (wave_has_queries) {
+    asm volatile("s_nop 15\n\ts_nop 15" ::: "memory");
+    reset_max();
+#pragma unroll
+    for (int w = W0; w < W0 + (NV + 1) * SPU; ++w) test_step(acc1, scv[1], scc[1], w);
+    combine_flags();
+    if (VAR == 0 && any_flag()) rare_log(acc1, scv[1], scc[1], tile_row0(NT - 1), 1);
+  }
+  if constexpr (STAMP) {
+    const uint64_t dc = __builtin_amdgcn_s_memtime() - stamp_c, dr = __builtin_amdgcn_s_memrealtime() - stamp_r;
+    if (wave == 0 && lane == 0) {
+      uint64_t* out = reinterpret_cast<uint64_t*>(prog + static_cast<uint64_t>(gridDim.x) * 8) + static_cast<uint64_t>(blockIdx.x) * 2;
+      out[0] = dc; out[1] = dr;
+    }
+  }
+  if constexpr (SYNC) { if (wave == 0 && lane == 0) __hip_atomic_store(prog + static_cast<uint64_t>(stream) * 8 + qt, 0xFFFFFFFFu, __ATOMIC_RELAXED, __HIP_MEMORY_SCOPE_AGENT); }
+  if (stage_counts && lane == 0 && n_stage1) atomicAdd(stage_counts, n_stage1);
+  if (wave == 0 && lane == 0) record_xcd_speed(sa.xcdw, xcd_map, stream & 7u, NT, static_cast<uint32_t>(__builtin_amdgcn_s_memrealtime()) - xw_t0);
+  verify_and_scatter_i8<DIM, CREDIT>(mylog, wcnt, sa, lane, rows, qlo, thr, qscale, qinv, rcv);
diff --git a/nano-vectordb_amd/csrc/nvdb_corpus.cpp b/nano-vectordb_amd/csrc/nvdb_corpus.cpp
--- a/nano-vectordb_amd/csrc/nvdb_corpus.cpp
+++ b/nano-vectordb_amd/csrc/nvdb_corpus.cpp
@@ -13,6 +13,8 @@
   if (c->shadow16) { (void)hipFree(c->shadow16); c->shadow16 = nullptr; }
   if (c->shadow8) { (void)hipFree(c->shadow8); c->shadow8 = nullptr; }
   if (c->shadow8_scales) { (void)hipFree(c->shadow8_scales); c->shadow8_scales = nullptr; }
+  if (c->shadow_resid.p) { (void)hipFree(c->shadow_resid.p); c->shadow_resid = DevBuf{}; }
+  c->shadow_scale_max = 0.f;
   c->rows = nullptr; c->scales = nullptr; c->owned = false; c->n = 0; c->dim = 0; c->fdim = 0; c->dtype = 0; c->max_norm = 0.f;
   c->cap_hint = 0;
   c->q8shadow = false; c->resid_max = 0.f; c->filter_max_norm = 0.f;
@@ -63,14 +65,20 @@
     const size_t n_pad = (static_cast<size_t>(c->n) + PAD_ROWS - 1) / PAD_ROWS * PAD_ROWS + PAD_ROWS;
     HIPCHK(c, hipMemsetAsync(c->shadow8 + count, 0, pad, c->stream));
     HIPCHK(c, hipMemsetAsync(c->shadow8_scales, 0, n_pad * 4, c->stream));
-    HIPCHK(c, hipMemsetAsync(bits, 0, 8, c->stream));
-    if (c->dtype == NVDB_DTYPE_F32) shadow_q8_kernel<float><<<grid, 256, 0, c->stream>>>(static_cast<const float*>(c->rows), c->shadow8, c->shadow8_scales, c->n, c->dim, sdim, bits);
-    else shadow_q8_kernel<_Float16><<<grid, 256, 0, c->stream>>>(static_cast<const _Float16*>(c->rows), c->shadow8, c->shadow8_scales, c->n, c->dim, sdim, bits);
+    float* resid = nullptr;
+    if (hipMalloc(reinterpret_cast<void**>(&resid), n_pad * 8) != hipSuccess) { (void)hipGetLastError(); resid = nullptr; }
+    if (resid) { c->shadow_resid = DevBuf{resid, n_pad * 8}; HIPCHK(c, hipMemsetAsync(resid, 0, n_pad * 8, c->stream)); }
+    HIPCHK(c, hipMemsetAsync(bits, 0, 16, c->stream));
+    uint32_t hs[4] = {0, 0, 0, 0};
+    if (c->dtype == NVDB_DTYPE_F32) shadow_q8_kernel<float><<<grid, 256, 0, c->stream>>>(static_cast<const float*>(c->rows), c->shadow8, c->shadow8_scales, c->n, c->dim, sdim, bits, resid);
+    else shadow_q8_kernel<_Float16><<<grid, 256, 0, c->stream>>>(static_cast<const _Float16*>(c->rows), c->shadow8, c->shadow8_scales, c->n, c->dim, sdim, bits, resid);
     HIPCHK(c, hipGetLastError());
-    HIPCHK(c, hipMemcpyAsync(hb, bits, 8, hipMemcpyDeviceToHost, c->stream));
+    HIPCHK(c, hipMemcpyAsync(hs, bits, 16, hipMemcpyDeviceToHost, c->stream));
     HIPCHK(c, hipStreamSynchronize(c->stream));
+    hb[0] = hs[0]; hb[1] = hs[1];
     if (hb[1] == 0) {
       std::memcpy(&c->resid_max, &hb[0], 4);
+      std::memcpy(&c->shadow_scale_max, &hs[2], 4);
       HIPCHK(c, hipMemsetAsync(bits, 0, 8, c->stream));
       row_norm_max_kernel<DT_I8><<<grid, 256, 0, c->stream>>>(c->shadow8, c->shadow8_scales, c->n, sdim, bits);
       HIPCHK(c, hipGetLastError());
@@ -83,6 +91,7 @@
     }
     (void)hipFree(c->shadow8); c->shadow8 = nullptr;
     (void)hipFree(c->shadow8_scales); c->shadow8_scales = nullptr;
+    if (c->shadow_resid.p) { (void)hipFree(c->shadow_resid.p); c->shadow_resid = DevBuf{}; }
   }
   if (c->dtype != NVDB_DTYPE_I8 && c->dim <= F16_FILTER_MAX_DIM && !(c->dtype == NVDB_DTYPE_F16 && f16_filter_dim(c->dim)) && c->opt_f32_shadow) {
     uint32_t sdim = 128;
@@ -264,7 +273,7 @@
   parts_destroy(c);
   if (c->hostblock.p) c->misc.p = nullptr;
   for (DevBuf* b : {&c->q32, &c->q16, &c->qscale, &c->qinv, &c->ebound, &c->slack, &c->thr, &c->cnt, &c->overflow, &c->cand,
-                    &c->out_ids, &c->out_scores, &c->misc, &c->hostblock, &c->hitlog, &c->prog, &c->qdelta, &c->rq, &c->rcand, &c->rout_ids, &c->rout_dist, &c->rdbg, &c->lk_scores, &c->lk_sel, &c->lk_hist, &c->lk_state, &c->xcdw, &c->tickets,
+                    &c->out_ids, &c->out_scores, &c->misc, &c->hostblock, &c->hitlog, &c->prog, &c->qdelta, &c->qnorm, &c->rq, &c->rcand, &c->rout_ids, &c->rout_dist, &c->rdbg, &c->lk_scores, &c->lk_sel, &c->lk_hist, &c->lk_state, &c->xcdw, &c->tickets,
                     &c->rg_radius, &c->rg_kept, &c->rg_off, &c->rg_idx, &c->rg_q, &c->rg_desc, &c->rg_taken, &c->rg_slab, &c->rg_pcnt, &c->rg_maskof, &c->rg_ids, &c->rg_scores, &c->row_masks, &c->mask_rows})
     if (b->p) (void)hipFree(b->p);
   for (hipEvent_t e : c->ev_pool) (void)hipEventDestroy(e);
@@ -397,6 +406,7 @@
   else if (k == "fuse") { c->opt_fuse = value ? 1 : 0; }
   else if (k == "zero_copy") { c->opt_zero_copy = value ? 1 : 0; }
   else if (k == "shadow_exact_thr") { c->opt_shadow_exact_thr = value ? 1 : 0; }
+  else if (k == "shadow_row_credit") { c->opt_shadow_row_credit = value ? 1 : 0; }
   else if (k == "exact_mfma") { c->opt_exact_mfma = value ? 1 : 0; }
   else if (k == "exact_img") { c->opt_exact_img = value ? 1 : 0; }
   else if (k == "exact_prescan") { c->opt_exact_prescan = value ? 1 : 0; }
diff --git a/nano-vectordb_amd/csrc/nvdb_ctx.h b/nano-vectordb_amd/csrc/nvdb_ctx.h
--- a/nano-vectordb_amd/csrc/nvdb_ctx.h
+++ b/nano-vectordb_amd/csrc/nvdb_ctx.h
@@ -74,6 +74,10 @@
   int64_t opt_q8_auto_min_rows = 1 << 20;
   int64_t opt_q8_auto_max_mb = 16384;
   float* shadow8_scales = nullptr;
+  DevBuf shadow_resid;
+  float shadow_scale_max = 0.f;
+  DevBuf qnorm;
+  int64_t opt_shadow_row_credit = 1;
   _Float16* shadow16 = nullptr;
   uint32_t fdim = 0;
   DevBuf qdelta;
@@ -210,6 +214,9 @@
 inline bool filter_is_i8(const nvdb_hip_ctx* c) { return c->dtype == NVDB_DTYPE_I8 || (c->q8shadow && c->use_shadow); }
 inline bool f16_beside_shadow(const nvdb_hip_ctx* c) { return c->q8shadow && c->dtype == NVDB_DTYPE_F16 && f16_filter_dim(c->dim); }
 inline bool shadow_preferred(const nvdb_hip_ctx* c) { return c->q8shadow && !(f16_beside_shadow(c) && (c->opt_q8_shadow == 0 || c->shadow_demoted)); }
+inline bool shadow_row_credit(const nvdb_hip_ctx* c) {
+  return c->opt_shadow_row_credit && c->q8shadow && c->use_shadow && c->shadow_resid.p && c->resid_max > 0.f && c->resid_max < 1e30f && c->shadow_scale_max < 1e30f;
+}
 inline uint64_t q8_shadow_bytes(uint64_t n, uint32_t dim) { return n * (static_cast<uint64_t>(dim) + 4u); }
 inline bool q8_shadow_wanted(const nvdb_hip_ctx* c, uint64_t free_hbm) {
   if (c->opt_q8_shadow == 0 || c->dtype == NVDB_DTYPE_I8 || !i8_filter_dim(c->dim)) return false;
@@ -268,7 +275,7 @@
 nvdb_status launch_prep_q16(nvdb_hip_ctx* c, hipStream_t s, const float* dev_q, uint32_t nq, uint32_t nq_pad, const PrepInit& pinit);
 nvdb_status launch_prep_q8(nvdb_hip_ctx* c, hipStream_t s, const float* dev_q, uint32_t nq, uint32_t nq_pad, const PrepInit& pinit);
 nvdb_status launch_filter_f16(nvdb_hip_ctx* c, hipStream_t s, uint32_t row_lo, uint32_t row_hi, uint32_t nq, uint32_t QT, uint32_t cap);
-nvdb_status launch_filter_i8(nvdb_hip_ctx* c, hipStream_t s, uint32_t row_lo, uint32_t row_hi, uint32_t nq, uint32_t QT, uint32_t cap);
+nvdb_status launch_filter_i8(nvdb_hip_ctx* c, hipStream_t s, uint32_t row_lo, uint32_t row_hi, uint32_t nq, uint32_t QT, uint32_t cap, bool row_credit = false);
 nvdb_status launch_boot_f16(nvdb_hip_ctx* c, hipStream_t s, uint32_t n0, uint32_t nq, uint32_t QT, uint32_t cap, uint32_t nb);
 nvdb_status launch_boot_i8(nvdb_hip_ctx* c, hipStream_t s, uint32_t n0, uint32_t nq, uint32_t QT, uint32_t cap);
 nvdb_status corpus_alloc_padded(nvdb_hip_ctx* c, uint64_t n, uint32_t dim, uint32_t dtype, void** rows, float** scales);
@@ -306,7 +313,7 @@
   return next_prog_region(c, s, nwg, &out.prog);
 }
 
-struct FilterCall { hipStream_t s; uint32_t row_lo, row_hi, nq, QT, cap; const float* thr; };
+struct FilterCall { hipStream_t s; uint32_t row_lo, row_hi, nq, QT, cap; const float* thr; bool row_credit = false; };
 struct FilterGeom { uint32_t block; size_t lds; uint32_t log_waves; bool timed; };
 
 template <typename T> inline T launch_arg(T a) { return a; }
diff --git a/nano-vectordb_amd/csrc/nvdb_launch_i8.cpp b/nano-vectordb_amd/csrc/nvdb_launch_i8.cpp
--- a/nano-vectordb_amd/csrc/nvdb_launch_i8.cpp
+++ b/nano-vectordb_amd/csrc/nvdb_launch_i8.cpp
@@ -8,7 +8,8 @@
                                         static_cast<signed char*>(c->q16.p) + static_cast<size_t>(nq_pad) * c->fdim,
                                         static_cast<float*>(c->qscale.p), static_cast<float*>(c->qinv.p),
                                         static_cast<float*>(c->ebound.p), static_cast<float*>(c->slack.p), static_cast<float*>(c->qdelta.p),
-                                        static_cast<uint32_t*>(c->overflow.p), static_cast<uint32_t>(c->opt_i8_lo_bits), pinit);
+                                        static_cast<uint32_t*>(c->overflow.p), static_cast<uint32_t>(c->opt_i8_lo_bits), pinit,
+                                        c->qnorm.bytes >= static_cast<size_t>(nq_pad) * 4 ? static_cast<float*>(c->qnorm.p) : nullptr);
   HIPCHK(c, hipGetLastError());
   return NVDB_OK;
 }
@@ -63,6 +64,13 @@
     if constexpr (DIM == 768 || DIM == 512)
       if (w8 && DIM == 768) return launch(i8s_build<DIM, 8>(sync), 8, filter_i8s_lds_bytes<DIM, 8>());
 #endif
+    if constexpr (DIM >= 384 && NB == 2)
+      if (!w8 && f.row_credit && c->qnorm.bytes >= static_cast<size_t>(nq_pad) * 4) {
+        const RowCredit rc{static_cast<const float*>(c->shadow_resid.p), static_cast<const float*>(c->qnorm.p), c->resid_max, c->shadow_scale_max};
+        return launch_filter_i8_kernel(c, f, sync ? shadow_i8s_kernel<DIM, true> : shadow_i8s_kernel<DIM, false>, nwg, FilterGeom{256, filter_i8s_lds_bytes<DIM, 4, true>(), 8, true},
+                                       static_cast<size_t>(nq_pad) * DIM, static_cast<const float*>(c->qdelta.p), &c->hitlog, scatter_args(c, f.cap, TROWS), sy.prog, sy.mask, sy.lead,
+                                       static_cast<uint32_t*>(c->misc.p) + 4, rc);
+      }
     if constexpr (DIM >= 384)
       if (!w8) return launch(i8s_build<DIM, 4>(sync), 4, filter_i8s_lds_bytes<DIM, 4>());
   }
@@ -104,10 +112,10 @@
   return fail(c, NVDB_ERR_UNSUPPORTED, "int8 boot kernel: unsupported dim");
 }
 
-nvdb_status launch_filter_i8(nvdb_hip_ctx* c, hipStream_t s, uint32_t row_lo, uint32_t row_hi, uint32_t nq, uint32_t QT, uint32_t cap) {
+nvdb_status launch_filter_i8(nvdb_hip_ctx* c, hipStream_t s, uint32_t row_lo, uint32_t row_hi, uint32_t nq, uint32_t QT, uint32_t cap, bool row_credit) {
   const uint32_t nb = filter_nb(c, nq);
   const uint32_t nq_pad = QT * filter_qpb(c, nq);
-  const FilterCall f{s, row_lo, row_hi, nq, QT, cap, static_cast<const float*>(c->thr.p)};
+  const FilterCall f{s, row_lo, row_hi, nq, QT, cap, static_cast<const float*>(c->thr.p), row_credit};
   nvdb_status st;
   if (dispatch_dim(I8DimsBig{}, c->fdim, st, [&](auto D) { return launch_filter_i8w_big_dim<decltype(D)::value>(c, f, nq_pad); })) return st;
   if (i8_two_stage(c) && dispatch_dim(I8Dims{}, c->fdim, st, [&](auto D) {
diff --git a/nano-vectordb_amd/csrc/nvdb_search.cpp b/nano-vectordb_amd/csrc/nvdb_search.cpp
--- a/nano-vectordb_amd/csrc/nvdb_search.cpp
+++ b/nano-vectordb_amd/csrc/nvdb_search.cpp
@@ -58,7 +58,7 @@
 }
 
 nvdb_status launch_filter(nvdb_hip_ctx* c, hipStream_t s, uint32_t row_lo, uint32_t row_hi, uint32_t nq, uint32_t QT, uint32_t cap) {
-  return filter_is_i8(c) ? launch_filter_i8(c, s, row_lo, row_hi, nq, QT, cap) : launch_filter_f16(c, s, row_lo, row_hi, nq, QT, cap);
+  return filter_is_i8(c) ? launch_filter_i8(c, s, row_lo, row_hi, nq, QT, cap, shadow_row_credit(c)) : launch_filter_f16(c, s, row_lo, row_hi, nq, QT, cap);
 }
 
 nvdb_status search_core(nvdb_hip_ctx* c, hipStream_t s, const float* dev_q, uint32_t nq, uint32_t k, uint64_t* dev_out_ids,
@@ -75,7 +75,7 @@
       {c->thr, per_q, false}, {c->cnt, per_q, false}, {c->overflow, per_q, false}, {c->cand, static_cast<size_t>(nq) * cap * sizeof(Cand), false},
       {c->misc, 64, false}, {c->prog, static_cast<size_t>(p.prog_words) * 4, false}, {c->tickets, FUSE_TICKETS * 4, false},
       {c->q16, static_cast<size_t>(p.nq_pad) * c->fdim * 2, true}, {c->qscale, per_q, true}, {c->qinv, per_q, true},
-      {c->ebound, per_q, true}, {c->slack, per_q, true}, {c->qdelta, per_q, true}};
+      {c->ebound, per_q, true}, {c->slack, per_q, true}, {c->qdelta, per_q, true}, {c->qnorm, per_q, true}};
   for (const auto& w : workspace)
     if ((p.prep || !w.filter_flow) && (st = ensure(c, w.buf, w.bytes))) return st;
   c->stats = nvdb_hip_scan_stats{};
```

Result: slower. 146,200 (-5.4%).
